# DeepRank/Deeprank-GNN

Measured on AMD Instinct MI355X. Metric: interface-graphs/sec (fwd+bwd) GINet batch=64 per GPU, higher is better.
Workload: dtype f32; 1 GPU; GINet train step (topology + body fwd + FC head/MSE + bwd + grad all-reduce + Adam) on SYN graphs: 200 nodes, ~1000 directed edges, 32 node feats, 50->16 clusters (BASELINE.json configs[1]); graphs_per_gpu=64, global_batch=64, parallelism=dp1, mode=native, step_layout=auto

## Files before the change

### deeprank-gnn_amd/_lib.py

```python
import ctypes
import os

import torch

_HERE = os.path.dirname(os.path.abspath(__file__))
LIB_PATH = os.environ.get("DRGNN_LIB") or os.path.join(_HERE, "csrc", "libdrgnn.so")

GINET, SGAT, FOUT = 0, 1, 2
MAX_BRANCH = 2
LDS_LIMIT = 160 * 1024
HEAD_MAX_HIDDEN = 512

TI = {name: i for i, name in enumerate([
    "NPTR", "EPTR", "ROWPTR0", "COL0", "EID0", "COLPTR0", "ROWIDX0", "TSLOT0", "CL0", "NC0",
    "MPTR0", "MEM0", "ROWPTR1", "COL1", "NE1", "COLPTR1", "ROWIDX1", "TSLOT1", "CL1", "NC1",
    "MPTR1", "MEM1", "CPTR0", "E1PTR", "CPTR1", "ERR", "GSTAT", "HORD", "HMP0", "HSPLIT", "IHORD"])}
TI_COUNT = len(TI)
TF = {"W0": 0, "W1": 1}
TF_COUNT = 2

FAULT_EXCHANGE = 1
STATUS_BITS = {1: "edge endpoint outside its graph's node range",
               2: "batch vector / edge list not grouped by graph",
               4: "cluster ids of one graph span too large a range",
               8: "len(cluster1) != number of depth-0 clusters"}

_c_i64 = ctypes.c_int64
_c_i32 = ctypes.c_int32
_vp = ctypes.c_void_p


class ConvParams(ctypes.Structure):
    _fields_ = [("w_nbr", _vp), ("nbr_sk", _c_i64), ("nbr_sh", _c_i64),
                ("w_self", _vp), ("self_sk", _c_i64), ("self_sh", _c_i64),
                ("bias", _vp)]


class ConvGrads(ctypes.Structure):
    _fields_ = [("w_nbr", _vp), ("w_self", _vp), ("bias", _vp)]


class NetDesc(ctypes.Structure):
    _fields_ = [("kind", _c_i32), ("n_branch", _c_i32), ("n_feat", _c_i32), ("reserved", _c_i32),
                ("conv1", ConvParams * MAX_BRANCH), ("conv2", ConvParams * MAX_BRANCH)]


class EnsMember(ctypes.Structure):
    _fields_ = [("net", NetDesc), ("w1", _vp), ("b1", _vp), ("w2", _vp), ("b2", _vp)]


class CohortMember(ctypes.Structure):
    _fields_ = EnsMember._fields_ + [
                ("flat_param", _vp), ("flat_grad", _vp), ("exp_avg", _vp), ("exp_avg_sq", _vp),
                ("step2", _vp), ("pred", _vp), ("readout", _vp), ("head_partials", _vp), ("partials", _vp), ("loss", _vp),
                ("lr", ctypes.c_double), ("beta1", ctypes.c_double), ("beta2", ctypes.c_double), ("eps", ctypes.c_double),
                ("seed", ctypes.c_uint32), ("reserved", _c_i32)]


class TopologyRequest(ctypes.Structure):
    _fields_ = [("edge_index", _vp), ("edge_attr", _vp), ("batch", _vp), ("cluster0", _vp), ("cluster1", _vp),
                ("node_ptr", _vp), ("edge_ptr", _vp), ("c1_ptr", _vp),
                ("n_nodes", _c_i64), ("n_edges", _c_i64), ("len_cluster1", _c_i64), ("n_graphs", _c_i64),
                ("max_nodes", _c_i32), ("max_edges", _c_i32),
                ("ws_i32", _vp), ("ws_f32", _vp), ("scratch_i32", _vp),
                ("set", _vp), ("ids", _vp), ("x_out", _vp), ("y_out", _vp),
                ("flags", _c_i32), ("reserved", _c_i32),
                ("x", _vp), ("tiles", _vp), ("n_feat", _c_i32), ("reserved2", _c_i32)]


TOPO_HIER = 1
TOPO_LEAN = 2
TOPO_TILES = 4
METRICS_COUNTS, METRICS_REGRESSION, METRICS_RANKING = 1, 2, 4


class GraphSet(ctypes.Structure):
    _fields_ = [("n_graphs", _c_i64), ("n_nodes", _c_i64), ("n_edges", _c_i64), ("len_cluster1", _c_i64),
                ("n_feat", _c_i32), ("y_bytes", _c_i32),
                ("node_ptr", _vp), ("edge_ptr", _vp), ("c1_ptr", _vp),
                ("x", _vp), ("edge_index", _vp), ("edge_attr", _vp),
                ("cluster0", _vp), ("cluster1", _vp), ("y", _vp)]


class EpochPlan(ctypes.Structure):
    _fields_ = [("set", _vp), ("host_node_ptr", _vp), ("host_edge_ptr", _vp), ("host_c1_ptr", _vp),
                ("ids", _vp), ("host_ids", _vp), ("n_ids", _c_i64),
                ("batch_size", _c_i32), ("need_weights", _c_i32), ("inference", _c_i32), ("reserved", _c_i32),
                ("net", _vp), ("head", _vp), ("g_conv1", _vp), ("g_conv2", _vp),
                ("head_offset", _c_i64),
                ("flat_param", _vp), ("flat_grad", _vp), ("exp_avg", _vp), ("exp_avg_sq", _vp), ("n_param", _c_i64),
                ("step2", _vp),
                ("lr", ctypes.c_double), ("beta1", ctypes.c_double), ("beta2", ctypes.c_double), ("eps", ctypes.c_double),
                ("cache", _vp), ("exchange", _vp), ("exchange_user", _vp), ("step_overrides", _vp), ("last_loss", _vp)]


class Optim(ctypes.Structure):
    _fields_ = [("lr", ctypes.c_double), ("beta1", ctypes.c_double), ("beta2", ctypes.c_double), ("eps", ctypes.c_double),
                ("weight_decay", ctypes.c_double), ("max_grad_norm", ctypes.c_double),
                ("lr_table", _vp), ("norm_words", _vp), ("norm_out", _vp),
                ("lr_n", _c_i32), ("decoupled", _c_i32), ("clip", _c_i32), ("norm_cap", _c_i32),
                ("n_dead", _c_i32), ("reserved", _c_i32),
                ("dead_off", _c_i64 * 8), ("dead_len", _c_i64 * 8)]


class IfaceRequest(ctypes.Structure):
    _fields_ = [("xyz", _vp), ("atom_ptr", _vp), ("res_ptr", _vp), ("res_split", _vp), ("res_type", _vp),
                ("host_atom_ptr", _vp), ("host_res_ptr", _vp), ("host_res_split", _vp),
                ("n_atoms", _c_i64), ("n_residues", _c_i64), ("n_complexes", _c_i64),
                ("contact_distance", ctypes.c_double), ("internal_contact_distance", ctypes.c_double),
                ("tile_atoms", _c_i32), ("reserved", _c_i32),
                ("workspace", _vp), ("workspace_bytes", _c_i64),
                ("node_ptr", _vp), ("edge_ptr", _vp), ("iedge_ptr", _vp)]


class ScoreRequest(ctypes.Structure):
    _fields_ = [("xyz", _vp), ("zone_atom", _vp), ("zone_ref", _vp), ("pair_res", _vp), ("atom_ptr", _vp),
                ("host_zone_atom", _vp), ("host_zone_ptr", _vp), ("host_pair_res", _vp), ("host_atom_ptr", _vp),
                ("n_poses", _c_i64), ("n_atoms", _c_i64), ("n_residues", _c_i64), ("n_pairs", _c_i64),
                ("n_ref_pairs", _c_i64), ("fnat_cutoff", ctypes.c_double),
                ("scores", _vp), ("classes", _vp), ("n_preserved", _vp)]


class BsaRequest(ctypes.Structure):
    _fields_ = [("xyz", _vp), ("atom_ptr", _vp), ("res_ptr", _vp), ("res_split", _vp), ("rad_complex", _vp),
                ("rad_unbound", _vp), ("target_res", _vp), ("target_complex", _vp),
                ("host_atom_ptr", _vp), ("host_res_ptr", _vp), ("host_res_split", _vp), ("host_target_res", _vp),
                ("host_target_complex", _vp),
                ("n_atoms", _c_i64), ("n_residues", _c_i64), ("n_complexes", _c_i64), ("n_targets", _c_i64),
                ("n_radii", _c_i64), ("probe", ctypes.c_double), ("n_slices", _c_i32), ("reserved", _c_i32),
                ("out", _vp), ("status", _vp)]


class HseRequest(ctypes.Structure):
    _fields_ = [("xyz", _vp), ("atom_ptr", _vp), ("res_ptr", _vp), ("bb", _vp), ("target_res", _vp), ("target_complex", _vp),
                ("tile_ptr", _vp),
                ("host_atom_ptr", _vp), ("host_res_ptr", _vp), ("host_bb", _vp), ("host_target_res", _vp),
                ("host_target_complex", _vp), ("host_tile_ptr", _vp),
                ("n_atoms", _c_i64), ("n_residues", _c_i64), ("n_complexes", _c_i64), ("n_targets", _c_i64),
                ("n_tiles", _c_i64), ("n_rows", _c_i64), ("radius", ctypes.c_double), ("connect_cutoff", ctypes.c_double),
                ("offset", _c_i32), ("connect_a", _c_i32), ("connect_b", _c_i32), ("direction", _c_i32),
                ("out", _vp), ("status", _vp)]


class PackRequest(ctypes.Structure):
    _fields_ = [("node_ptr", _vp), ("edge_ptr", _vp), ("iedge_ptr", _vp), ("node_residue", _vp), ("chain", _vp), ("type", _vp),
                ("pos", _vp), ("edge_index", _vp), ("dist", _vp), ("internal_edge_index", _vp), ("bsa", _vp), ("hse", _vp),
                ("res_feat", _vp), ("type_table", _vp), ("cols", _vp), ("host_cols", _vp),
                ("n_complexes", _c_i64), ("n_nodes", _c_i64), ("n_edges", _c_i64), ("n_iedges", _c_i64),
                ("n_residues", _c_i64), ("n_rows", _c_i64),
                ("res_width", _c_i32), ("type_width", _c_i32), ("n_cols", _c_i32), ("edge_mode", _c_i32),
                ("x", _vp), ("edge_index_out", _vp), ("edge_attr", _vp), ("internal_edge_index_out", _vp), ("batch", _vp)]


PACK_TYPE, PACK_POS, PACK_CHAIN, PACK_BSA, PACK_HSE, PACK_RES = range(6)


EXCHANGE_FN = ctypes.CFUNCTYPE(ctypes.c_int, ctypes.c_void_p, ctypes.c_int64, ctypes.c_int64, ctypes.c_void_p)


class StepPlan(ctypes.Structure):
    _fields_ = [("kind", _c_i32), ("n_feat", _c_i32), ("max_nodes", _c_i32), ("max_edges", _c_i32), ("max_c0", _c_i32),
                ("R", _c_i32), ("H", _c_i32), ("O", _c_i32),
                ("n_graphs", _c_i64), ("co_built_graphs", _c_i64),
                ("train", _c_i32), ("topo_flags", _c_i32),
                ("force_wgs", _c_i32), ("no_class", _c_i32), ("no_aggregate", _c_i32), ("no_split", _c_i32),
                ("no_paired", _c_i32),
                ("family", _c_i32), ("wgs_per_graph", _c_i32), ("slabs_per_graph", _c_i32), ("width", _c_i32),
                ("cls", _c_i32), ("lean_ok", _c_i32), ("builder_wgs_per_graph", _c_i32),
                ("lds_bytes", _c_i64), ("xchg_words", _c_i64),
                ("from_memory", _c_i32), ("reserved", _c_i32)]

    OVERRIDES = ("force_wgs", "no_class", "no_aggregate", "no_split", "no_paired")


STEP_FAMILY_NONE, STEP_FAMILY_PRODUCT, STEP_FAMILY_AGGREGATE = 0, 1, 2


def _plan_inputs(kind, n_feat, max_nodes, max_edges, max_c0, R, H, O, n_graphs, topo_flags):
    p = StepPlan()
    p.kind, p.n_feat, p.max_nodes, p.max_edges, p.max_c0 = int(kind), int(n_feat), int(max_nodes), int(max_edges), int(max_c0)
    p.R, p.H, p.O, p.n_graphs, p.topo_flags = int(R), int(H), int(O), int(n_graphs), int(topo_flags)
    return p


class StepHints(ctypes.Structure):
    _fields_ = [("host_node_ptr", _vp), ("host_edge_ptr", _vp), ("set_node_ptr", _vp), ("set_edge_ptr", _vp),
                ("host_ids", _vp), ("topo_flags", _c_i32), ("reserved", _c_i32), ("tiles", _vp), ("plan", _vp),
                ("next_ids", _vp), ("n_next", _c_i64)]


class TopologyCacheDesc(ctypes.Structure):
    _fields_ = [("n_graphs", _c_i64), ("n_nodes", _c_i64), ("n_edges", _c_i64),
                ("ws_i32", _vp), ("ws_f32", _vp), ("x", _vp), ("y", _vp), ("y_bytes", _c_i32), ("flags", _c_i32),
                ("tiles", _vp)]


class HeadDesc(ctypes.Structure):
    _fields_ = [("R", _c_i32), ("H", _c_i32), ("O", _c_i32), ("task", _c_i32), ("train", _c_i32),
                ("p_drop", ctypes.c_float), ("seed", ctypes.c_uint32), ("transform_sigmoid", _c_i32),
                ("w1", _vp), ("b1", _vp), ("w2", _vp), ("b2", _vp), ("class_w", _vp), ("drop_mask", _vp)]


TASK_REG, TASK_CLASS, TASK_GRAD = 0, 1, 2
ZERO_RANGES = 8


def _ptr(t):
    return None if t is None else t.data_ptr()


class DrgnnError(RuntimeError):
    pass


def _check(rc, what):
    if rc != 0:
        kind = {-1: "bad argument", -2: "workspace/capacity", -3: "unsupported width"}.get(
            rc, "hipError_t %d" % rc if rc > 0 else "error %d" % rc)
        raise DrgnnError("%s failed: %s" % (what, kind))


class Api(object):

    def __init__(self, path):
        self.path = path
# ... 576 lines not shown
```

### deeprank-gnn_amd/csrc/drgnn_capi.hip

```cpp
#define DRGNN_KERNELS_MAIN
#include "drgnn_kernels.h"

#include <vector>
#include <algorithm>
#include <memory>
#include <string.h>
#include <stdlib.h>
#ifdef DRGNN_EMU
#define DRGNN_LDS_LIMIT (160 * 1024)
#else
#define DRGNN_LDS_LIMIT (160 * 1024)
#define HIP_TRY(expr)                                   \
    do {                                                \
        hipError_t e_ = (expr);                         \
        if (e_ != hipSuccess) return (int)e_;           \
    } while (0)
#endif



extern "C" {

int drgnn_abi_version(void) { return DRGNN_ABI_VERSION; }

#if defined(DRGNN_PHASE_TIMING) && !defined(DRGNN_EMU)
int drgnn_debug_set_phase_buffer(void* dev_buf) {
    unsigned long long* p = (unsigned long long*)dev_buf;
    return (int)hipMemcpyToSymbol(HIP_SYMBOL(g_phase_buf), &p, sizeof(p));
}
#endif

int drgnn_topology_layout(int64_t n_nodes, int64_t n_edges, int64_t n_graphs, int64_t* off_i32,
                          int64_t* off_f32) {
    if (n_nodes < 0 || n_edges < 0 || n_graphs < 0 || !off_i32 || !off_f32) return DRGNN_E_ARG;
    TopoLayout L;
    topo_layout(n_nodes, n_edges, n_graphs, &L);
    for (int k = 0; k <= DRGNN_TI_COUNT; ++k) off_i32[k] = L.i32[k];
    for (int k = 0; k <= DRGNN_TF_COUNT; ++k) off_f32[k] = L.f32[k];
    return 0;
}

int64_t drgnn_topology_scratch_elems(int64_t n_nodes, int64_t n_edges, int64_t n_graphs) {
    return topo_gscratch_base(n_nodes, n_edges, n_graphs) + TOPO_GSCRATCH_CONST;
}

static int64_t topo_lds_bytes(int capN, int capE, int tile_f = 0) {
    const int64_t capT = (capN > capE ? capN : capE) + 1;
    return 4 * (topo_scratch_ints(capN, capE, capT, (int64_t)capN + capE + 2) + (tile_f > 0 ? (int64_t)capN * (((tile_f + 3) & ~3) + 4) : 0));
}
static bool topo_tiles_shape_ok(int capN, int capE, int F) {
    const int TF = (F + 3) & ~3;
    if (capN <= 0 || F <= 0 || F > 256 || (int64_t)capN * TF > 16 * DRGNN_BCAP) return false;
    return topo_lds_bytes(capN, capE > 0 ? capE : 1, F) <= DRGNN_LDS_LIMIT;
}

int64_t drgnn_topology_lds_bytes(int32_t max_nodes, int32_t max_edges) {
    if (max_nodes <= 0) return 0;
    return topo_lds_bytes(max_nodes, max_edges > 0 ? max_edges : 1);
}

int64_t drgnn_topology_tiles_elems(int64_t n_nodes, int32_t n_feat) {
    if (n_nodes < 0 || n_feat <= 0) return 0;
    const int64_t TF = ((int64_t)n_feat + 3) & ~(int64_t)3;
    return (n_feat & 3) ? drgnn_tiles_x_off(n_nodes, TF) + n_nodes * TF : n_nodes * (TF + 2);
}
int32_t drgnn_topology_tiles_ok(int32_t max_nodes, int32_t max_edges, int32_t n_feat) {
    return topo_tiles_shape_ok(max_nodes, max_edges, n_feat) ? 1 : 0;
}

}

#ifndef DRGNN_TOPO_SPLIT_MAX_GRAPHS
#define DRGNN_TOPO_SPLIT_MAX_GRAPHS 160
#endif
static int topo_prepare(TopoLaunch& L, int64_t* lds_out, const int64_t* edge_index, const float* edge_attr,
                        const int64_t* batch, const int64_t* cluster0, const int64_t* cluster1,
                        const int32_t* node_ptr, const int32_t* edge_ptr, const int32_t* c1_ptr,
                        int64_t n_nodes, int64_t n_edges, int64_t len_cluster1, int64_t n_graphs,
                        int32_t max_nodes, int32_t max_edges, int32_t* ws_i32, float* ws_f32,
                        int32_t* scratch_i32, int32_t flags = DRGNN_TOPO_HIER, const float* x_in = nullptr,
                        float* tiles = nullptr, int32_t tile_f = 0) {
    if (n_nodes < 0 || n_edges < 0 || n_graphs < 0 || !ws_i32) return DRGNN_E_ARG;
    if (!batch && !(node_ptr && edge_ptr)) return DRGNN_E_ARG;
    if (!cluster0 && cluster1) return DRGNN_E_ARG;
    if (n_edges > 0 && !edge_index) return DRGNN_E_ARG;
    if (edge_attr && !ws_f32) return DRGNN_E_ARG;
    if (n_nodes + n_graphs >= INT32_MAX || n_edges >= INT32_MAX) return DRGNN_E_CAPACITY;
    TopoLayout lay;
    topo_layout(n_nodes, n_edges, n_graphs, &lay);
    L.tv = topo_view(ws_i32, ws_f32, lay);
    L.args.edge_index = edge_index;
    L.args.edge_attr = edge_attr;
    L.args.cluster0 = cluster0;
    L.args.cluster1 = cluster1;
    L.args.c1_ptr = c1_ptr;
    L.args.n_edges = n_edges;
    L.args.len_cluster1 = len_cluster1;
    L.args.n_graphs = (int)n_graphs;
    L.args.set_ids = nullptr; L.args.set_node_ptr = L.args.set_edge_ptr = L.args.set_c1_ptr = nullptr;
    L.args.set_x = nullptr; L.args.set_y = nullptr; L.args.x_out = nullptr; L.args.y_out = nullptr;
    L.args.n_set = 0; L.args.n_feat = 0; L.args.y_bytes = 0;
    L.args.flags = flags;
    L.args.x_in = nullptr; L.args.tiles = nullptr; L.args.tile_nodes = n_nodes; L.args.tile_f = 0;
    if (flags & DRGNN_TOPO_TILES) {
        if (!(flags & DRGNN_TOPO_HIER) || !tiles || (x_in && !(tile_f & 3) && (((uintptr_t)x_in) & 15)) || (((uintptr_t)tiles) & 15)) return DRGNN_E_ARG;
        if (!topo_tiles_shape_ok(max_nodes, max_edges, tile_f)) return DRGNN_E_CAPACITY;
        L.args.x_in = x_in; L.args.tiles = tiles; L.args.tile_f = tile_f;
    }
    L.gscratch = scratch_i32;
    L.level1_only = 0;
    L.roles = 1;
    L.pf_ids = nullptr; L.pf_n = 0; L.pf_graphs = 0;
    L.user_nptr = (node_ptr && edge_ptr) ? node_ptr : nullptr;
    L.user_eptr = (node_ptr && edge_ptr) ? edge_ptr : nullptr;
    int64_t lds = 0;
    L.capN = 0; L.capE = 0;
    if (max_nodes > 0) {
        lds = topo_lds_bytes(max_nodes, max_edges > 0 ? max_edges : 1, L.args.tile_f);
        if (lds <= DRGNN_LDS_LIMIT) { L.capN = max_nodes; L.capE = max_edges > 0 ? max_edges : 1; }
        else lds = 0;
    }
    if (L.args.tile_f > 0 && L.capN == 0) return DRGNN_E_CAPACITY;
    if (L.capN > 0 && cluster0 != nullptr && L.user_nptr != nullptr && !(cluster1 != nullptr && c1_ptr == nullptr) &&
        n_graphs <= DRGNN_TOPO_SPLIT_MAX_GRAPHS)
        L.roles = 2;
    *lds_out = lds;
    return 0;
}

static int topo_prepare_req(TopoLaunch& T, int64_t* tlds, const drgnn_topology_request* r) {
    const drgnn_graph_set* gs = r->set;
    if (!gs)
        return topo_prepare(T, tlds, r->edge_index, r->edge_attr, r->batch, r->cluster0, r->cluster1, r->node_ptr,
                            r->edge_ptr, r->c1_ptr, r->n_nodes, r->n_edges, r->len_cluster1, r->n_graphs, r->max_nodes,
                            r->max_edges, r->ws_i32, r->ws_f32, r->scratch_i32, r->flags, r->x, r->tiles, r->n_feat);
    if (!r->ids || !r->node_ptr || !r->edge_ptr || !gs->node_ptr || !gs->edge_ptr || !gs->cluster0) return DRGNN_E_ARG;
    if (gs->cluster1 && (!gs->c1_ptr || !r->c1_ptr)) return DRGNN_E_ARG;
    if (r->x_out && (!gs->x || gs->n_feat <= 0)) return DRGNN_E_ARG;
    if (r->y_out && (!gs->y || (gs->y_bytes != 4 && gs->y_bytes != 8))) return DRGNN_E_ARG;
    const float* attr = (r->ws_f32 && gs->edge_attr) ? gs->edge_attr : nullptr;
    if ((r->flags & DRGNN_TOPO_TILES) && (!gs->x || gs->n_feat <= 0 || (!(gs->n_feat & 3) && (((uintptr_t)gs->x) & 15)))) return DRGNN_E_ARG;
    const int rc = topo_prepare(T, tlds, gs->edge_index, attr, nullptr, gs->cluster0, gs->cluster1, r->node_ptr,
                                r->edge_ptr, r->c1_ptr, r->n_nodes, r->n_edges, r->len_cluster1, r->n_graphs,
                                r->max_nodes, r->max_edges, r->ws_i32, r->ws_f32, r->scratch_i32, r->flags, nullptr, r->tiles,
                                gs->n_feat);
    if (rc) return rc;
    TopoArgs& a = T.args;
    a.n_edges = gs->n_edges;
    a.set_ids = r->ids; a.set_node_ptr = gs->node_ptr; a.set_edge_ptr = gs->edge_ptr; a.set_c1_ptr = gs->c1_ptr;
    a.set_x = gs->x; a.set_y = gs->y; a.x_out = r->x_out; a.y_out = r->y_out;
    a.n_set = gs->n_graphs; a.n_feat = gs->n_feat; a.y_bytes = gs->y_bytes;
    return 0;
}

static int topology_build_impl(const int64_t* edge_index, const float* edge_attr, const int64_t* batch,
                         const int64_t* cluster0, const int64_t* cluster1, const int32_t* node_ptr,
                         const int32_t* edge_ptr, const int32_t* c1_ptr, int64_t n_nodes,
                         int64_t n_edges, int64_t len_cluster1, int64_t n_graphs, int32_t max_nodes,
                         int32_t max_edges, int32_t* ws_i32, float* ws_f32, int32_t* scratch_i32,
                         int32_t flags, void* stream_, const float* x_in = nullptr, float* tiles = nullptr,
                         int32_t tile_f = 0) {
    drgnn_stream_t stream = (drgnn_stream_t)stream_;
    TopoLaunch L;
    int64_t lds = 0;
    int rc0 = topo_prepare(L, &lds, edge_index, edge_attr, batch, cluster0, cluster1, node_ptr, edge_ptr, c1_ptr,
                           n_nodes, n_edges, len_cluster1, n_graphs, max_nodes, max_edges, ws_i32, ws_f32,
                           scratch_i32, flags, x_in, tiles, tile_f);
    if (rc0) return rc0;
    if (L.capN == 0 && !scratch_i32) return DRGNN_E_CAPACITY;
    if (n_graphs == 0) return 0;
    PtrArgs pa;
    pa.batch = batch; pa.edge_row = edge_index; pa.n_nodes = n_nodes; pa.n_edges = n_edges;
    pa.n_graphs = (int)n_graphs; pa.nptr = L.tv.p[DRGNN_TI_NPTR]; pa.eptr = L.tv.p[DRGNN_TI_EPTR];
    pa.err = L.tv.p[DRGNN_TI_ERR];
    const bool need_ptrs = !(node_ptr && edge_ptr);
    const int64_t span = n_nodes > n_edges ? n_nodes : n_edges;
#ifdef DRGNN_EMU
    if (need_ptrs) {
        for (int k = 0; k < 4; ++k) pa.err[k] = 0;
        for (int64_t i = 0; i < (span > 0 ? span : 1); ++i) ptr_item(pa, i);
    }
    std::vector<int> lds_buf((size_t)(lds / 4) + 16);
    for (int pass = 0; pass < 2; ++pass) {
        if (pass == 1) { if (!(cluster1 && !c1_ptr)) break; L.level1_only = 1; L.roles = 1; }
        for (int gph = 0; gph < n_graphs * (pass == 0 ? L.roles : 1); ++gph) {
            if (L.capN > 0) topo_block<true>(L, gph, lds_buf.data());
            else topo_block<false>(L, gph, lds_buf.data());
        }
    }
    (void)stream;
#else
    if (need_ptrs) {
        const int n = (int)n_graphs + 1;
        hipLaunchKernelGGL(k_topo_begin, dim3((unsigned)((n + 255) / 256)), dim3(256), 0, stream,
                           (const int32_t*)nullptr, (const int32_t*)nullptr, pa.nptr, pa.eptr, pa.err, n);
        const int64_t items = span > 0 ? span : 1;
        hipLaunchKernelGGL(k_ptrs, dim3((unsigned)((items + 255) / 256)), dim3(256), 0, stream, pa);
    }
    if (lds > 64 * 1024)
        HIP_TRY(hipFuncSetAttribute((const void*)k_topo<true>, hipFuncAttributeMaxDynamicSharedMemorySize, (int)lds));
    for (int pass = 0; pass < 2; ++pass) {
        if (pass == 1) { if (!(cluster1 && !c1_ptr)) break; L.level1_only = 1; L.roles = 1; }
        if (L.capN > 0) hipLaunchKernelGGL(k_topo<true>, dim3((unsigned)(n_graphs * L.roles)), dim3(DRGNN_NTHREADS), (size_t)lds, stream, L);
        else hipLaunchKernelGGL(k_topo<false>, dim3((unsigned)n_graphs), dim3(DRGNN_NTHREADS), 0, stream, L);
    }
    HIP_TRY(hipGetLastError());
#endif
    return 0;
}

extern "C" {

int drgnn_topology_build(const int64_t* edge_index, const float* edge_attr, const int64_t* batch,
                         const int64_t* cluster0, const int64_t* cluster1, const int32_t* node_ptr,
                         const int32_t* edge_ptr, const int32_t* c1_ptr, int64_t n_nodes,
                         int64_t n_edges, int64_t len_cluster1, int64_t n_graphs, int32_t max_nodes,
                         int32_t max_edges, int32_t* ws_i32, float* ws_f32, int32_t* scratch_i32,
                         void* stream_) {
    return topology_build_impl(edge_index, edge_attr, batch, cluster0, cluster1, node_ptr, edge_ptr, c1_ptr, n_nodes, n_edges,
                               len_cluster1, n_graphs, max_nodes, max_edges, ws_i32, ws_f32, scratch_i32, DRGNN_TOPO_HIER,
                               stream_);
}

int drgnn_topology_build_request(const drgnn_topology_request* r, void* stream_) {
    if (!r) return DRGNN_E_ARG;
    if (!r->set)
        return topology_build_impl(r->edge_index, r->edge_attr, r->batch, r->cluster0, r->cluster1, r->node_ptr,
                                   r->edge_ptr, r->c1_ptr, r->n_nodes, r->n_edges, r->len_cluster1, r->n_graphs,
                                   r->max_nodes, r->max_edges, r->ws_i32, r->ws_f32, r->scratch_i32, r->flags, stream_,
                                   r->x, r->tiles, r->n_feat);
    TopoLaunch L;
    int64_t lds = 0;
    const int rc = topo_prepare_req(L, &lds, r);
    if (rc) return rc;
    if (L.capN == 0 && !r->scratch_i32) return DRGNN_E_CAPACITY;
    if (r->n_graphs == 0) return 0;
#ifdef DRGNN_EMU
    std::vector<int> lds_buf((size_t)(lds / 4) + 16);
    for (int gph = 0; gph < r->n_graphs * L.roles; ++gph) {
        if (L.capN > 0) topo_block<true>(L, gph, lds_buf.data());
        else topo_block<false>(L, gph, lds_buf.data());
    }
    (void)stream_;
#else
    hipStream_t stream = (hipStream_t)stream_;
    if (lds > 64 * 1024)
        HIP_TRY(hipFuncSetAttribute((const void*)k_topo<true>, hipFuncAttributeMaxDynamicSharedMemorySize, (int)lds));
    if (L.capN > 0) hipLaunchKernelGGL(k_topo<true>, dim3((unsigned)(r->n_graphs * L.roles)), dim3(DRGNN_NTHREADS), (size_t)lds, stream, L);
    else hipLaunchKernelGGL(k_topo<false>, dim3((unsigned)r->n_graphs), dim3(DRGNN_NTHREADS), 0, stream, L);
    HIP_TRY(hipGetLastError());
#endif
    return 0;
}

int drgnn_topology_tiles(const int32_t* ws_i32, const float* ws_f32, int64_t n_nodes, int64_t n_edges, int64_t n_graphs,
                         const float* x, int32_t n_feat, int32_t use_weights, float* tiles, void* stream_) {
    if (!ws_i32 || !x || !tiles || n_nodes < 0 || n_edges < 0 || n_graphs < 0 || n_feat <= 0) return DRGNN_E_ARG;
    if (use_weights && !ws_f32) return DRGNN_E_ARG;
    if (n_graphs == 0) return 0;
    TopoLayout lay;
    topo_layout(n_nodes, n_edges, n_graphs, &lay);
    TilesArgs a;
    a.tv = topo_view(const_cast<int32_t*>(ws_i32), const_cast<float*>(ws_f32), lay);
    a.x = x; a.tiles = tiles; a.n_nodes = n_nodes; a.n_feat = n_feat; a.use_weights = use_weights ? 1 : 0;
#ifdef DRGNN_EMU
    for (int64_t g = 0; g < n_graphs; ++g) tiles_block(a, (int)g);
    (void)stream_;
#else
    hipLaunchKernelGGL(k_tiles, dim3((unsigned)n_graphs), dim3(DRGNN_NTHREADS), 0, (hipStream_t)stream_, a);
    HIP_TRY(hipGetLastError());
#endif
    return 0;
}

int drgnn_batch_offsets(const drgnn_graph_set* set, const int32_t* ids, int64_t n_ids, int32_t batch_size,
                        int32_t* ptrs, void* stream_) {
    if (!set || !ids || !ptrs || n_ids < 0 || batch_size < 1 || !set->node_ptr || !set->edge_ptr) return DRGNN_E_ARG;
    if (batch_size > 4096) return DRGNN_E_CAPACITY;
    if (n_ids == 0) return 0;
    OffsetsArgs a;
    a.set = *set; a.ids = ids; a.n_ids = n_ids; a.batch_size = batch_size; a.ptrs = ptrs;
    const int64_t nb = (n_ids + batch_size - 1) / batch_size;
    const size_t words = (size_t)DRGNN_NTHREADS + 4 + 3 * ((size_t)batch_size + 1);
#ifdef DRGNN_EMU
    std::vector<int> buf(words);
    for (int64_t k = 0; k < nb; ++k) batch_offsets_block(a, (int)k, buf.data() + DRGNN_NTHREADS + 4, buf.data());
    (void)stream_;
#else
    hipLaunchKernelGGL(k_batch_offsets, dim3((unsigned)nb), dim3(DRGNN_NTHREADS), words * 4, (hipStream_t)stream_, a);
    HIP_TRY(hipGetLastError());
#endif
    return 0;
}

int drgnn_topology_finalize(int32_t* ws_i32, int64_t n_nodes, int64_t n_edges, int64_t n_graphs,
                            void* stream_) {
    if (!ws_i32 || n_graphs < 0) return DRGNN_E_ARG;
    TopoLayout lay;
    topo_layout(n_nodes, n_edges, n_graphs, &lay);
    ScanArgs a;
    a.tv = topo_view(ws_i32, nullptr, lay);
    a.n_graphs = (int)n_graphs;
#ifdef DRGNN_EMU
    int part[DRGNN_NTHREADS + 4];
    finalize_block(a, part);
    (void)stream_;
#else
    hipLaunchKernelGGL(k_finalize, dim3(1), dim3(DRGNN_NTHREADS), 0, (hipStream_t)stream_, a);
    HIP_TRY(hipGetLastError());
#endif
    return 0;
}

int drgnn_topology_status(const int32_t* ws_i32, int64_t n_nodes, int64_t n_edges, int64_t n_graphs,
                          int32_t* status4, void* stream_) {
    if (!ws_i32 || !status4) return DRGNN_E_ARG;
    TopoLayout lay;
    topo_layout(n_nodes, n_edges, n_graphs, &lay);
    const int32_t* err = ws_i32 + lay.i32[DRGNN_TI_ERR];
    const int32_t* gst = ws_i32 + lay.i32[DRGNN_TI_GSTAT];
    std::vector<int32_t> host((size_t)(2 * n_graphs) + 4);
#ifdef DRGNN_EMU
    for (int k = 0; k < 4; ++k) host[k] = err[k];
    for (int64_t g = 0; g < 2 * n_graphs; ++g) host[4 + g] = gst[g];
    (void)stream_;
#else
    HIP_TRY(hipMemcpyAsync(host.data(), err, 4 * sizeof(int32_t), hipMemcpyDeviceToHost, (hipStream_t)stream_));
    if (n_graphs > 0)
        HIP_TRY(hipMemcpyAsync(host.data() + 4, gst, 2 * n_graphs * sizeof(int32_t), hipMemcpyDeviceToHost, (hipStream_t)stream_));
    HIP_TRY(hipStreamSynchronize((hipStream_t)stream_));
#endif
    status4[0] = host[0]; status4[1] = -1; status4[2] = 0; status4[3] = 0;
    for (int64_t g = 0; g < n_graphs; ++g) {
        host[4 + g] |= host[4 + n_graphs + g];
        if (host[4 + g]) {
            status4[0] |= host[4 + g];
            if (status4[1] < 0) status4[1] = (int32_t)g;
            status4[2] += 1;
        }
    }
    return 0;
}

struct StepCaps { int N, E, C; };
static StepCaps step_caps(int32_t max_nodes, int32_t max_edges, int32_t max_c0) {
    return StepCaps{max_nodes, max_edges > 0 ? max_edges : 1, (max_c0 > 0 && max_c0 < max_nodes) ? max_c0 : max_nodes};
}

int64_t drgnn_net_lds_bytes(int32_t kind, int32_t n_feat, int32_t max_nodes, int32_t max_edges,
                            int32_t max_c0, int32_t backward) {
    if (max_nodes <= 0) return 0;
    const StepCaps c = step_caps(max_nodes, max_edges, max_c0);
    return 4 * net_scratch_words(kind, n_feat, c.N, c.E, c.C, backward);
}

int64_t drgnn_net_partial_elems(int32_t kind, int32_t n_feat) { (void)kind; return net_partial_floats(n_feat); }

int64_t drgnn_net_scratch_elems(int32_t kind, int32_t n_feat, int64_t n_nodes, int64_t n_edges,
                                int64_t n_graphs) {
    const int nb = (kind == DRGNN_GINET) ? 2 : 1;
    const int64_t f = net_gscratch_base(kind, n_feat, n_nodes, n_edges, n_graphs, 0);
    const int64_t b = net_gscratch_base(kind, n_feat, n_nodes, n_edges, n_graphs, 1);
    return nb * (f > b ? f : b) + 64;
}

}

static int net_check(const drgnn_net_desc* net) {
    if (!net) return DRGNN_E_ARG;
    if (net->kind < DRGNN_GINET || net->kind > DRGNN_FOUT) return DRGNN_E_ARG;
    if (net->n_branch < 1 || net->n_branch > DRGNN_MAX_BRANCH) return DRGNN_E_ARG;
    if (net->n_feat < 1) return DRGNN_E_WIDTH;
    for (int b = 0; b < net->n_branch; ++b) {
        if (!net->conv1[b].w_nbr || !net->conv2[b].w_nbr) return DRGNN_E_ARG;
        if (net->kind != DRGNN_GINET &&
            (!net->conv1[b].w_self || !net->conv2[b].w_self || !net->conv1[b].bias || !net->conv2[b].bias))
            return DRGNN_E_ARG;
    }
    return 0;
}

template <bool BWD>
static int net_launch(NetLaunch& L, int32_t max_nodes, int32_t max_edges, int32_t max_c0, float* scratch,
// ... 2302 lines not shown
```

### deeprank-gnn_amd/csrc/drgnn_kernels.h

```cpp
#pragma once
#include "drgnn_head.h"
#include "drgnn_step.h"
#include "drgnn_step2.h"
#include "drgnn_step3.h"
#include "drgnn_layers.h"
#include "drgnn_mcl.h"
#include "drgnn_louvain.h"
#include "drgnn_iface.h"
#include "drgnn_score.h"
#include "drgnn_bsa.h"
#include "drgnn_hse.h"
#include "drgnn_pack.h"
#include "drgnn_metrics.h"
#include "drgnn_collate.h"
#include "drgnn_p2p.h"

struct PtrArgs {
    const int64_t* batch;
    const int64_t* edge_row;
    int64_t n_nodes, n_edges;
    int n_graphs;
    int32_t* nptr;
    int32_t* eptr;
    int32_t* err;
};

DEV void ptr_item(const PtrArgs& a, int64_t i) {
    const int B = a.n_graphs;
    if (i < a.n_nodes) {
        long long b = a.batch[i];
        long long prev = (i > 0) ? (long long)a.batch[i - 1] : -1;
        if (b < prev || b < 0 || b >= B) { ATOMIC_OR(&a.err[0], DRGNN_S_UNSORTED); a.err[1] = 0; b = prev < 0 ? 0 : prev; }
        for (long long gph = prev + 1; gph <= b && gph <= B; ++gph) a.nptr[gph] = (int32_t)i;
        if (i == a.n_nodes - 1)
            for (long long gph = b + 1; gph <= B; ++gph) a.nptr[gph] = (int32_t)a.n_nodes;
    }
    if (i < a.n_edges) {
        auto graph_of = [&](int64_t e) -> long long {
            const long long r = a.edge_row[e];
            if (r < 0 || r >= a.n_nodes) return -2;
            return (long long)a.batch[r];
        };
        long long b = graph_of(i);
        long long prev = (i > 0) ? graph_of(i - 1) : -1;
        if (b == -2 || prev == -2) { ATOMIC_OR(&a.err[0], DRGNN_S_EDGE_RANGE); a.err[1] = 0; if (b == -2) b = prev < 0 ? 0 : prev; if (prev == -2) prev = b; }
        if (b < prev || b >= B) { ATOMIC_OR(&a.err[0], DRGNN_S_UNSORTED); a.err[1] = 0; b = prev; }
        for (long long gph = prev + 1; gph <= b && gph <= B; ++gph) a.eptr[gph] = (int32_t)i;
        if (i == a.n_edges - 1)
            for (long long gph = b + 1; gph <= B; ++gph) a.eptr[gph] = (int32_t)a.n_edges;
    }
    if (i == 0) {
        if (a.n_nodes == 0) for (int gph = 0; gph <= B; ++gph) a.nptr[gph] = 0;
        if (a.n_edges == 0) for (int gph = 0; gph <= B; ++gph) a.eptr[gph] = 0;
    }
}

struct TopoLaunch {
    TopoView tv;
    TopoArgs args;
    const int32_t* user_nptr;
    const int32_t* user_eptr;
    int32_t* gscratch;
    int capN, capE;
    int level1_only;
    int roles;
    const int32_t* pf_ids; int pf_n; int pf_graphs;
    const float* pf_tiles; const float* pf_x; int pf_f; int pf_coef;
    long long pf_tile_nodes;
    const void* pf_y; int pf_y_bytes;
};

#ifdef DRGNN_EMU
DEV void prefetch_block(const TopoLaunch&, int) {}
#else
DEV void prefetch_block(const TopoLaunch& L, int g) {
    if (g >= L.pf_n) return;
    const int32_t* const* P = L.tv.p;
    const int id = __builtin_amdgcn_readfirstlane(L.pf_ids[g]);
    if (id < 0 || id >= L.pf_graphs) return;
    const int n0 = P[DRGNN_TI_NPTR][id], n1 = P[DRGNN_TI_NPTR][id + 1];
    const int e0 = P[DRGNN_TI_EPTR][id], e1 = P[DRGNN_TI_EPTR][id + 1];
    const int N = n1 - n0, E = e1 - e0, rowbase = n0 + id, t = threadIdx.x;
    int acc = P[DRGNN_TI_NC0][id] ^ P[DRGNN_TI_NE1][id] ^ P[DRGNN_TI_NC1][id] ^ P[DRGNN_TI_GSTAT][id] ^ P[DRGNN_TI_HSPLIT][4 * id];
    if (L.pf_y) acc ^= (L.pf_y_bytes == 8) ? (int)((const long long*)L.pf_y)[id] : ((const int*)L.pf_y)[id];
    drgnn_f4 f = {0.f, 0.f, 0.f, 0.f};
    const int n4 = (N * L.pf_f) >> 2;
    const drgnn_f4* s4 = (const drgnn_f4*)(L.pf_tiles + (long long)n0 * L.pf_f);
    const drgnn_f4* x4 = L.pf_x ? (const drgnn_f4*)(L.pf_x + (long long)n0 * L.pf_f) : nullptr;
    for (int q = t; q < n4; q += DRGNN_NTHREADS) {
        const drgnn_f4 v = s4[q];
        f[0] += v[0]; f[1] += v[1]; f[2] += v[2]; f[3] += v[3];
        if (x4) { const drgnn_f4 u = x4[q]; f[0] += u[0]; f[1] += u[1]; f[2] += u[2]; f[3] += u[3]; }
    }
    for (int i = t; i <= N; i += DRGNN_NTHREADS) {
        acc ^= P[DRGNN_TI_HMP0][rowbase + i] ^ P[DRGNN_TI_MPTR1][rowbase + i] ^ P[DRGNN_TI_ROWPTR1][rowbase + i] ^
               P[DRGNN_TI_COLPTR1][rowbase + i];
        if (i < N) {
            acc ^= P[DRGNN_TI_IHORD][n0 + i] ^ P[DRGNN_TI_MEM1][n0 + i];
            if (L.pf_coef) {
                const float* td = L.pf_tiles + L.pf_tile_nodes * L.pf_f + n0;
                f[0] += td[i] + td[L.pf_tile_nodes + i];
            }
        }
    }
    for (int e = t; e < E; e += DRGNN_NTHREADS) {
        acc ^= P[DRGNN_TI_COL1][e0 + e] ^ P[DRGNN_TI_ROWIDX1][e0 + e];
        if (L.pf_coef && L.tv.w1) { acc ^= P[DRGNN_TI_TSLOT1][e0 + e]; f[1] += L.tv.w1[e0 + e]; }
    }
    if (acc == 0x7fc12345 && f[0] + f[1] + f[2] + f[3] == 12345.678f) { const_cast<int32_t*>(P[DRGNN_TI_ERR])[1] = acc; }
}
#endif

template <bool LDS, int WEIGHTS = -1>
DEV void topo_block(const TopoLaunch& L, int blk, int* lds) {
    TopoScratch s;
    if (L.pf_ids != nullptr) { prefetch_block(L, blk); return; }
#ifdef DRGNN_TOPO_EXIT0
    return;
#endif
    int g = blk, role = TOPO_ROLE_ALL;
    if (L.roles == 2) {
        const int full = (L.args.n_graphs >> 3) << 4;
        if (blk < full) { g = ((blk >> 4) << 3) + (blk & 7); role = ((blk >> 3) & 1) ? TOPO_ROLE_MEMBERS : TOPO_ROLE_EDGES; }
        else { const int t = blk - full; g = (full >> 1) + (t >> 1); role = (t & 1) ? TOPO_ROLE_MEMBERS : TOPO_ROLE_EDGES; }
    }
    const int sidx = (role == TOPO_ROLE_MEMBERS) ? L.args.n_graphs + g : g;
    const int32_t* NP = L.user_nptr ? L.user_nptr : L.tv.p[DRGNN_TI_NPTR];
    const int32_t* EP = L.user_eptr ? L.user_eptr : L.tv.p[DRGNN_TI_EPTR];
    const int n0 = NP[g], n1 = NP[g + 1], N = n1 - n0;
    const int e0 = EP[g], e1 = EP[g + 1], E = e1 - e0;
    if (LDS) {
        const int capT = imax(L.capN, L.capE) + 1;
        s = topo_carve(lds, L.capN, L.capE, capT, L.capN + L.capE + 2);
        if (L.args.tile_f > 0 && L.args.tiles != nullptr)
            s.xs = (float*)(lds + topo_scratch_ints(L.capN, L.capE, capT, (int64_t)L.capN + L.capE + 2));
    } else {
        s = topo_carve(L.gscratch + topo_gscratch_base(n0, e0, g), N, E, N + E + 1, N + E + 2);
    }
    const bool fits = !LDS || (N <= L.capN && E <= L.capE);
    if (!L.level1_only) {
        FOR_TID(i, 1) {
            L.tv.p[DRGNN_TI_GSTAT][sidx] = 0;
            if (role == TOPO_ROLE_ALL) L.tv.p[DRGNN_TI_GSTAT][L.args.n_graphs + g] = 0;
            if (L.user_nptr && role != TOPO_ROLE_MEMBERS) {
                L.tv.p[DRGNN_TI_NPTR][g] = n0; L.tv.p[DRGNN_TI_NPTR][g + 1] = n1;
                L.tv.p[DRGNN_TI_EPTR][g] = e0; L.tv.p[DRGNN_TI_EPTR][g + 1] = e1;
                if (g == 0) L.tv.p[DRGNN_TI_ERR][0] = 0;
            }
        }
        if (fits && (L.args.flags & DRGNN_TOPO_LEAN)) topo_lean_preclear(N, s, role != TOPO_ROLE_EDGES, role != TOPO_ROLE_MEMBERS);
        BARRIER();
    }
    if (!fits) {
        FOR_TID(i, 1) { topo_flag(L.tv, DRGNN_S_EDGE_RANGE, sidx); }
        return;
    }
    if (!L.level1_only) {
        topo_graph<WEIGHTS>(L.tv, L.args, g, n0, n1, e0, e1, s, role);
    } else {
        FOR_TID(i, 1) { s.part[0] = 0; }
        BARRIER();
        FOR_TID(t, DRGNN_NTHREADS) {
            int acc = 0;
            for (int q = t; q < g; q += DRGNN_NTHREADS) acc += L.tv.p[DRGNN_TI_NC0][q];
            if (acc) ATOMIC_ADD(&s.part[0], acc);
        }
        BARRIER();
        const int begin = s.part[0];
        const int C0 = L.tv.p[DRGNN_TI_NC0][g];
        BARRIER();
        int len = C0;
        if (g == L.args.n_graphs - 1 && (int64_t)begin + C0 != L.args.len_cluster1) len = -1;
        if ((int64_t)begin + C0 > L.args.len_cluster1) len = -1;
        topo_graph_level1(L.tv, L.args, g, n0, C0, L.args.cluster1 + begin, len, s, g, false,
                          (L.args.flags & DRGNN_TOPO_HIER) ? L.tv.p[DRGNN_TI_CL0] + n0 : nullptr, N);
    }
}

struct TilesArgs { TopoView tv; const float* x; float* tiles; int64_t n_nodes; int n_feat, use_weights; };
DEV void tiles_block(const TilesArgs& a, int g) {
    const int n0 = a.tv.p[DRGNN_TI_NPTR][g], N = a.tv.p[DRGNN_TI_NPTR][g + 1] - n0;
    const int e0 = a.tv.p[DRGNN_TI_EPTR][g];
    const int32_t* rp = a.tv.p[DRGNN_TI_ROWPTR0] + n0 + g;
    const int32_t* col = a.tv.p[DRGNN_TI_COL0] + e0;
    const float* w = (a.use_weights && a.tv.w0) ? a.tv.w0 + e0 : nullptr;
    const int F = a.n_feat, TF = (F + 3) & ~3;
    const float* x = a.x + (long long)n0 * F;
    float* ts = a.tiles + (long long)n0 * TF;
    float* td = a.tiles + a.n_nodes * TF + n0;
    float* tc = td + a.n_nodes;
    float* tx = (F & 3) ? a.tiles + drgnn_tiles_x_off(a.n_nodes, TF) + (long long)n0 * TF : nullptr;
    FOR_TID(pad, N * (TF - F)) {
        const int i = pad / (TF - F), f = F + pad % (TF - F);
        ts[(long long)i * TF + f] = 0.0f;
        tx[(long long)i * TF + f] = 0.0f;
    }
    FOR_TID(item, N * F) {
        const int i = item / F, f = item - i * F;
        if (tx) tx[(long long)i * TF + f] = x[(long long)i * F + f];
        const int lo = rp[i], hi = rp[i + 1], deg = hi - lo;
        float acc = 0.0f, asum = 0.0f;
        if (w != nullptr) {
            for (int k = lo; k < hi; k += 4)
                for (int j = 0; j < 4; ++j) {
                    const int kk = (k + j < hi) ? k + j : hi - 1;
                    const float cf = ((k + j < hi) ? 1.0f : 0.0f) * w[kk];
                    asum += cf;
                    acc = fmaf(cf, x[(long long)col[kk] * F + f], acc);
                }
        } else {
            for (int k = lo; k < hi; ++k) acc += x[(long long)col[k] * F + f];
        }
        ts[(long long)i * TF + f] = acc;
        if (f == 0) {
            float d, sc;
            if (w != nullptr) { d = 1.0f / (float)(deg > 0 ? deg : 1); sc = asum * d; }
            else { d = deg > 0 ? 1.0f / (float)deg : 0.0f; sc = 1.0f; }
            td[i] = d; tc[i] = sc;
        }
    }
}

struct ScanArgs { TopoView tv; int n_graphs; };
DEV void finalize_block(const ScanArgs& a, int* part) {
    const int B = a.n_graphs;
    const int src[3] = {DRGNN_TI_NC0, DRGNN_TI_NE1, DRGNN_TI_NC1};
    const int dst[3] = {DRGNN_TI_CPTR0, DRGNN_TI_E1PTR, DRGNN_TI_CPTR1};
    for (int w = 0; w < 3; ++w) {
        int32_t* out = a.tv.p[dst[w]];
        const int32_t* in = a.tv.p[src[w]];
        FOR_TID(i, B + 1) { out[i] = (i < B) ? in[i] : 0; }
        BARRIER();
        wg_exscan(out, B + 1, part);
    }
}

struct ReduceArgs {
    const float* partials;
    int n_graphs, n_branch, n_feat, n_partial;
    int kind;
    drgnn_conv_params lay1[DRGNN_MAX_BRANCH], lay2[DRGNN_MAX_BRANCH];
    drgnn_conv_grads g1[DRGNN_MAX_BRANCH], g2[DRGNN_MAX_BRANCH];
    float* grad_x; int64_t n_nodes;
};

DEV float* reduce_dst(const ReduceArgs& a, int br, int p) {
    const int F = a.n_feat;
    const int o_w1s = F * DRGNN_H1, o_b1 = 2 * F * DRGNN_H1, o_w2n = o_b1 + DRGNN_H1;
    const int o_w2s = o_w2n + DRGNN_H1 * DRGNN_H2, o_b2 = o_w2s + DRGNN_H1 * DRGNN_H2;
    if (p < o_w1s)
        return a.g1[br].w_nbr ? a.g1[br].w_nbr + (int64_t)(p / DRGNN_H1) * a.lay1[br].nbr_sk + (int64_t)(p % DRGNN_H1) * a.lay1[br].nbr_sh : nullptr;
    if (p < o_b1) {
        const int q = p - o_w1s;
        return a.g1[br].w_self ? a.g1[br].w_self + (int64_t)(q / DRGNN_H1) * a.lay1[br].self_sk + (int64_t)(q % DRGNN_H1) * a.lay1[br].self_sh : nullptr;
    }
    if (p < o_w2n) return a.g1[br].bias ? a.g1[br].bias + (p - o_b1) : nullptr;
    if (p < o_w2s) {
        const int q = p - o_w2n;
        return a.g2[br].w_nbr ? a.g2[br].w_nbr + (int64_t)(q / DRGNN_H2) * a.lay2[br].nbr_sk + (int64_t)(q % DRGNN_H2) * a.lay2[br].nbr_sh : nullptr;
    }
    if (p < o_b2) {
        const int q = p - o_w2s;
        return a.g2[br].w_self ? a.g2[br].w_self + (int64_t)(q / DRGNN_H2) * a.lay2[br].self_sk + (int64_t)(q % DRGNN_H2) * a.lay2[br].self_sh : nullptr;
    }
    return a.g2[br].bias ? a.g2[br].bias + (p - o_b2) : nullptr;
}
DEV void reduce_write(const ReduceArgs& a, int br, int p, float acc) {
    float* d = reduce_dst(a, br, p);
    if (d) *d = acc;
}

DEV bool reduce_live(const ReduceArgs& a, int p) {
    if (a.kind != DRGNN_GINET) return true;
    const int F = a.n_feat;
    const int o_w1s = F * DRGNN_H1, o_w2n = 2 * F * DRGNN_H1 + DRGNN_H1, o_w2s = o_w2n + DRGNN_H1 * DRGNN_H2;
    return p < o_w1s || (p >= o_w2n && p < o_w2s);
}

DEV float reduce_sum(const ReduceArgs& a, int br, int p, int first, int stride) {
    const float* src = a.partials + (int64_t)br * a.n_partial + p;
    const int64_t step = (int64_t)a.n_branch * a.n_partial;
    float acc = 0.0f;
    float v[16];
    int g = first;
    for (; g + 15 * stride < a.n_graphs; g += 16 * stride) {
#pragma unroll
        for (int k = 0; k < 16; ++k) v[k] = src[(int64_t)(g + k * stride) * step];
#pragma unroll
        for (int k = 0; k < 16; ++k) acc += v[k];
    }
    for (; g < a.n_graphs; g += stride) acc += src[(int64_t)g * step];
    return acc;
}

DEV float reduce_sum_w(const ReduceArgs& a, int br, int p, int first, int stride, const float* w, int wshift) {
    const float* src = a.partials + (int64_t)br * a.n_partial + p;
    const int64_t step = (int64_t)a.n_branch * a.n_partial;
    float acc = 0.0f;
    float v[16], c[16];
    int g = first;
    for (; g + 15 * stride < a.n_graphs; g += 16 * stride) {
#pragma unroll
        for (int k = 0; k < 16; ++k) { v[k] = src[(int64_t)(g + k * stride) * step]; c[k] = w[(g + k * stride) >> wshift]; }
#pragma unroll
        for (int k = 0; k < 16; ++k) acc = fmaf(c[k], v[k], acc);
    }
    for (; g < a.n_graphs; g += stride) acc = fmaf(w[g >> wshift], src[(int64_t)g * step], acc);
    return acc;
}

DEV void reduce_grad_x(const ReduceArgs& a, int64_t item) {
    if (a.grad_x != nullptr && a.n_branch > 1 && item < a.n_nodes * a.n_feat) {
        float acc = a.grad_x[item];
        for (int br = 1; br < a.n_branch; ++br) acc += a.grad_x[(int64_t)br * a.n_nodes * a.n_feat + item];
        a.grad_x[item] = acc;
    }
}

struct NetLaunch {
    NetArgs a;
    float* gscratch;
    int capN, capE, capC;
    int64_t n_edges;
};

struct CoLaunch {
    NetLaunch net;
    TopoLaunch topo;
    int n_net;
};

HD int64_t net_gscratch_base(int kind, int F, int64_t n0, int64_t e0, int64_t g, int bwd) {
    const int64_t c0 = net_scratch_words(kind, F, 0, 0, 0, bwd);
    return net_scratch_words(kind, F, n0, e0, n0, bwd) - c0 + c0 * g;
}

template <int KIND, bool BWD, bool LDS>
DEV void net_block(const NetLaunch& L, int blk, float* lds) {
    const int nb = L.a.net.n_branch;
    const int g = blk / nb, br = blk % nb;
    float* scratch;
    int capN, capE, capC;
    if (LDS) {
        scratch = lds; capN = L.capN; capE = L.capE; capC = L.capC;
        const int n0 = L.a.tv.p[DRGNN_TI_NPTR][g], e0 = L.a.tv.p[DRGNN_TI_EPTR][g];
        if (L.a.tv.p[DRGNN_TI_NPTR][g + 1] - n0 > capN || L.a.tv.p[DRGNN_TI_EPTR][g + 1] - e0 > capE ||
            L.a.tv.p[DRGNN_TI_NC0][g] > capC) {
            if (!BWD) {
                FOR_TID(c, DRGNN_H2) { L.a.readout[(long)g * DRGNN_H2 * nb + br * DRGNN_H2 + c] = DRGNN_NAN; }
            }
            return;
        }
    } else {
        const int n0 = L.a.tv.p[DRGNN_TI_NPTR][g], e0 = L.a.tv.p[DRGNN_TI_EPTR][g];
        capN = L.a.tv.p[DRGNN_TI_NPTR][g + 1] - n0;
        capE = L.a.tv.p[DRGNN_TI_EPTR][g + 1] - e0;
        capC = capN;
        const int F = L.a.net.n_feat;
        const int64_t per_branch = net_gscratch_base(KIND, F, L.a.n_nodes, L.n_edges, L.a.n_graphs, BWD);
        scratch = L.gscratch + (int64_t)br * per_branch + net_gscratch_base(KIND, F, n0, e0, g, BWD);
    }
    if (BWD) net_backward_graph<KIND>(L.a, g, g, br, scratch, capN, capE, capC);
    else net_forward_graph<KIND>(L.a, g, g, br, scratch, capN, capE, capC);
}

#define DRGNN_STEP_DIMS_MAX 64
struct StepDims {
    int count;
    int32_t n0[DRGNN_STEP_DIMS_MAX], n[DRGNN_STEP_DIMS_MAX], e0[DRGNN_STEP_DIMS_MAX], e[DRGNN_STEP_DIMS_MAX];
    int32_t gi[DRGNN_STEP_DIMS_MAX];
};
struct StepLaunch {
    StepArgs a;
    int capN, capE, capC;
    int64_t words;
    StepDims dims;
};
struct StepCoLaunch {
    StepLaunch step;
    TopoLaunch topo;
    int n_net;
};

#ifndef DRGNN_EMU
template <int KIND, int XF, bool GATHER, int CLS, int SPLIT, bool TRAIN, int XG = 0>
DEV void step2_block(const StepLaunch& L, const StepArgs& A, int blk, float* lds) {
    int g, half;
    if (SPLIT == 2) { g = ((blk >> 4) << 3) + (blk & 7); half = (blk >> 3) & 1; }
    else { g = blk; half = 0; }
    if (g >= A.n_graphs) return;
    if (L.dims.count > 0) {
        const int gi = GATHER ? L.dims.gi[g] : g;
        GraphDims d;
        d.n0 = L.dims.n0[g]; d.N = L.dims.n[g]; d.e0 = L.dims.e0[g]; d.E = L.dims.e[g];
        d.rowbase = d.n0 + gi;
        d.C = 0; d.E1 = 0; d.C1 = 0;
        const int cnt_c = A.tv.p[DRGNN_TI_NC0][gi], cnt_e1 = A.tv.p[DRGNN_TI_NE1][gi], cnt_c1 = A.tv.p[DRGNN_TI_NC1][gi];
        const int32_t* hs = A.tv.p[DRGNN_TI_HSPLIT] + 4 * gi;
        const int hk = (SPLIT == 2) ? hs[0] : 0, hq = (SPLIT == 2) ? hs[1] : 0, hn = (SPLIT == 2) ? hs[2] : 0;
        net_step2_graph<KIND, XF, GATHER, CLS, SPLIT, TRAIN, XG>(A, d, g, gi, half, lds, L.capN, L.capE, L.capC, true, cnt_c, cnt_e1,
                                                             cnt_c1, hk, hq, hn);
        return;
    }
    const int gi = GATHER ? WG_UNIFORM(A.gather_ids[g]) : g;
    const GraphDims d = net_dims(A.tv, gi);
    const int32_t* hs = A.tv.p[DRGNN_TI_HSPLIT] + 4 * gi;
    const int hk = (SPLIT == 2) ? WG_UNIFORM(hs[0]) : 0, hq = (SPLIT == 2) ? WG_UNIFORM(hs[1]) : 0, hn = (SPLIT == 2) ? WG_UNIFORM(hs[2]) : 0;
    if (d.N > L.capN || d.E > L.capE || d.C > L.capC) {
        if (half == 0) {
            FOR_TID(c, A.hf.R) { const_cast<float*>(A.hf.readout)[(long)g * A.hf.R + c] = DRGNN_NAN; }
            if (TRAIN) {
                float* hp = A.hf.partials + (long)g * head_compact_floats(A.hf.R, A.hf.H, A.hf.O);
                FOR_TID(i, (int)head_compact_floats(A.hf.R, A.hf.H, A.hf.O)) { hp[i] = DRGNN_NAN; }
            }
            FOR_TID(o, A.hf.O) { A.hf.pred[(long)g * A.hf.O + o] = DRGNN_NAN; }
        }
        return;
    }
    net_step2_graph<KIND, XF, GATHER, CLS, SPLIT, TRAIN, XG>(A, d, g, gi, half, lds, L.capN, L.capE, L.capC, false, 0, 0, 0, hk, hq, hn);
}
#endif

#ifndef DRGNN_EMU
template <int XF, bool GATHER, int CLS, bool TRAIN>
DEV void step3_block(const StepLaunch& L, int blk, float* lds) {
    const int g = ((blk >> 4) << 3) + (blk & 7), br = (blk >> 3) & 1;
    if (g >= L.a.n_graphs) return;
    if (L.dims.count > 0) {
        const int gi = GATHER ? L.dims.gi[g] : g;
        GraphDims d;
        d.n0 = L.dims.n0[g]; d.N = L.dims.n[g]; d.e0 = L.dims.e0[g]; d.E = L.dims.e[g];
        d.rowbase = d.n0 + gi;
        d.C = 0; d.E1 = 0; d.C1 = 0;
        const int cnt_c = L.a.tv.p[DRGNN_TI_NC0][gi], cnt_e1 = L.a.tv.p[DRGNN_TI_NE1][gi], cnt_c1 = L.a.tv.p[DRGNN_TI_NC1][gi];
        net_step3_graph<XF, GATHER, CLS, TRAIN>(L.a, d, g, gi, br, lds, L.capN, L.capE, L.capC, true, cnt_c, cnt_e1, cnt_c1);
        return;
    }
    const int gi = GATHER ? WG_UNIFORM(L.a.gather_ids[g]) : g;
    const GraphDims d = net_dims(L.a.tv, gi);
    if (d.N > L.capN || d.E > L.capE || d.C > L.capC) {
        const uint32_t tag = (uint32_t)L.a.step2[0] + 1u;
        FOR_TID(c, DRGNN_H2) { const_cast<float*>(L.a.hf.readout)[(long)g * L.a.hf.R + br * DRGNN_H2 + c] = DRGNN_NAN; }
        FOR_TID(h, L.a.hf.H) { xchg_publish(L.a.xchg + ((long)g * 2 + br) * L.a.hf.H + h, tag, DRGNN_NAN); }
        if (br == 0) {
            if (TRAIN) {
                float* hp = L.a.hf.partials + (long)g * head_compact_floats(L.a.hf.R, L.a.hf.H, L.a.hf.O);
                FOR_TID(i, (int)head_compact_floats(L.a.hf.R, L.a.hf.H, L.a.hf.O)) { hp[i] = DRGNN_NAN; }
            }
            FOR_TID(o, L.a.hf.O) { L.a.hf.pred[(long)g * L.a.hf.O + o] = DRGNN_NAN; }
        }
        return;
    }
    net_step3_graph<XF, GATHER, CLS, TRAIN>(L.a, d, g, gi, br, lds, L.capN, L.capE, L.capC, false, 0, 0, 0);
}
#endif

#ifndef DRGNN_EMU
template <int XF, bool GATHER, int CLS, bool TRAIN, bool SG = false>
DEV void step3b_block(const StepLaunch& L, const StepArgs& A, int g, float* lds) {
    constexpr bool DUAL = !SG && STEP3B_DUAL(XF, CLS, TRAIN);
    if (g >= A.n_graphs) return;
    if (L.dims.count > 0) {
        const int gi = GATHER ? L.dims.gi[g] : g;
        GraphDims d;
        d.n0 = L.dims.n0[g]; d.N = L.dims.n[g]; d.e0 = L.dims.e0[g]; d.E = L.dims.e[g];
        d.rowbase = d.n0 + gi;
        d.C = 0; d.E1 = 0; d.C1 = 0;
        const int cnt_c = A.tv.p[DRGNN_TI_NC0][gi], cnt_e1 = A.tv.p[DRGNN_TI_NE1][gi], cnt_c1 = A.tv.p[DRGNN_TI_NC1][gi];
        net_step3_graph_both<XF, GATHER, CLS, TRAIN, DUAL, SG>(A, d, g, gi, lds, L.capN, L.capE, L.capC, true, cnt_c, cnt_e1, cnt_c1);
        return;
    }
    const int gi = GATHER ? WG_UNIFORM(A.gather_ids[g]) : g;
    const GraphDims d = net_dims(A.tv, gi);
    if (d.N > L.capN || d.E > L.capE || d.C > L.capC) {
        FOR_TID(c, A.hf.R) { const_cast<float*>(A.hf.readout)[(long)g * A.hf.R + c] = DRGNN_NAN; }
        if (TRAIN) {
            float* hp = A.hf.partials + (long)g * head_compact_floats(A.hf.R, A.hf.H, A.hf.O);
            FOR_TID(i, (int)head_compact_floats(A.hf.R, A.hf.H, A.hf.O)) { hp[i] = DRGNN_NAN; }
        }
        FOR_TID(o, A.hf.O) { A.hf.pred[(long)g * A.hf.O + o] = DRGNN_NAN; }
        return;
    }
    net_step3_graph_both<XF, GATHER, CLS, TRAIN, DUAL, SG>(A, d, g, gi, lds, L.capN, L.capE, L.capC, false, 0, 0, 0);
}
#endif

struct UpdateArgs {
    ReduceArgs r;
    HeadReduceArgs h;
    AdamArgs ad;
    int conv_blocks;
    int blocks_per_branch;
    int apply_adam;
    const float* readout;
    int hR, hH;
    int32_t* step2;
    float* loss2;
};

DEV void update_store(const UpdateArgs& u, float* dst, float g) {
    *dst = g;
    if (u.apply_adam) adam_item(u.ad, (int64_t)(dst - u.ad.grad));
}

DEV int update_head_items(const UpdateArgs& u) { return (u.readout ? u.hH * u.hR : 0) + u.h.P - 1; }
DEV float update_head_sum(const UpdateArgs& u, int item, int first, int stride) {
    float acc = 0.0f;
    if (u.readout) {
        const int HR = u.hH * u.hR;
        if (item < HR) {
            const int h = item / u.hR, r = item - h * u.hR;
            const float* dh = u.h.partials + h;
            const float* xr = u.readout + r;
            float va[16], vb[16];
            int w = first;
            for (; w + 15 * stride < u.h.n_wg; w += 16 * stride) {
#pragma unroll
                for (int k = 0; k < 16; ++k) { va[k] = dh[(long)(w + k * stride) * u.h.P]; vb[k] = xr[(long)(w + k * stride) * u.hR]; }
#pragma unroll
                for (int k = 0; k < 16; ++k) acc = fmaf(va[k], vb[k], acc);
            }
            for (; w < u.h.n_wg; w += stride) acc = fmaf(dh[(long)w * u.h.P], xr[(long)w * u.hR], acc);
            return acc;
        }
        item -= HR;
    }
    const float* src = u.h.partials + item;
    float v[16];
    int w = first;
    for (; w + 15 * stride < u.h.n_wg; w += 16 * stride) {
#pragma unroll
        for (int k = 0; k < 16; ++k) v[k] = src[(long)(w + k * stride) * u.h.P];
#pragma unroll
        for (int k = 0; k < 16; ++k) acc += v[k];
    }
    for (; w < u.h.n_wg; w += stride) acc += src[(long)w * u.h.P];
    return acc;
}
DEV float update_head_sum_w(const UpdateArgs& u, int item, int first, int stride, const float* gw) {
    float acc = 0.0f;
    if (u.readout) {
        const int HR = u.hH * u.hR;
        if (item < HR) {
            const int h = item / u.hR, r = item - h * u.hR;
            const float* dh = u.h.partials + h;
            const float* xr = u.readout + r;
            float va[16], vb[16], vc[16];
            int w = first;
            for (; w + 15 * stride < u.h.n_wg; w += 16 * stride) {
#pragma unroll
                for (int k = 0; k < 16; ++k) {
                    va[k] = dh[(long)(w + k * stride) * u.h.P]; vb[k] = xr[(long)(w + k * stride) * u.hR]; vc[k] = gw[w + k * stride];
                }
#pragma unroll
                for (int k = 0; k < 16; ++k) acc = fmaf(vc[k] * va[k], vb[k], acc);
            }
            for (; w < u.h.n_wg; w += stride) acc = fmaf(gw[w] * dh[(long)w * u.h.P], xr[(long)w * u.hR], acc);
            return acc;
        }
        item -= HR;
    }
    const float* src = u.h.partials + item;
    float v[16], c[16];
    int w = first;
    for (; w + 15 * stride < u.h.n_wg; w += 16 * stride) {
#pragma unroll
        for (int k = 0; k < 16; ++k) { v[k] = src[(long)(w + k * stride) * u.h.P]; c[k] = gw[w + k * stride]; }
#pragma unroll
        for (int k = 0; k < 16; ++k) acc = fmaf(c[k], v[k], acc);
    }
    for (; w < u.h.n_wg; w += stride) acc = fmaf(gw[w], src[(long)w * u.h.P], acc);
    return acc;
}
struct GradArgs {
    UpdateArgs u;
    const float* graph_weight;
    int wshift;
    int n_zero;
    float* zero_ptr[DRGNN_ZERO_RANGES];
    int64_t zero_len[DRGNN_ZERO_RANGES];
};
DEV void update_head_store(const UpdateArgs& u, int item, float acc) {
    const int n_grad = update_head_items(u) - 1;
    if (item < n_grad) update_store(u, u.h.grad + item, acc);
    else if (item == n_grad && u.h.loss) { u.h.loss[0] = acc; if (u.loss2) u.loss2[0] = acc; }
}

struct CohortStep {
    const drgnn_cohort_member* members;
    const int32_t* ids;
    const int32_t* counts;
    int K;
    int64_t stride;
};
#ifndef DRGNN_EMU
#ifdef DRGNN_KERNELS_MAIN
__global__ void __launch_bounds__(256) k_ptrs(PtrArgs a) {
    const int64_t i = (int64_t)blockIdx.x * blockDim.x + threadIdx.x;
    ptr_item(a, i);
}
#endif
template <int N>
DEV void kernarg_touch_lines(int off0) {
    static_assert(N >= 1 && N <= 12, "lines per call");
    const char* base = (const char*)__builtin_amdgcn_kernarg_segment_ptr() + (off0 & ~63);
    int t;
#define DRGNN_KA_OFF(k) "i"(64 * ((k) < N ? (k) : N - 1))
    asm volatile("s_load_dword %0, %1, %2\n s_load_dword %0, %1, %3\n s_load_dword %0, %1, %4\n s_load_dword %0, %1, %5\n"
                 "s_load_dword %0, %1, %6\n s_load_dword %0, %1, %7\n s_load_dword %0, %1, %8\n s_load_dword %0, %1, %9\n"
                 "s_load_dword %0, %1, %10\n s_load_dword %0, %1, %11\n s_load_dword %0, %1, %12\n s_load_dword %0, %1, %13\n"
                 "s_waitcnt lgkmcnt(0)"
                 : "=&s"(t)
                 : "s"(base), DRGNN_KA_OFF(0), DRGNN_KA_OFF(1), DRGNN_KA_OFF(2), DRGNN_KA_OFF(3), DRGNN_KA_OFF(4), DRGNN_KA_OFF(5),
                   DRGNN_KA_OFF(6), DRGNN_KA_OFF(7), DRGNN_KA_OFF(8), DRGNN_KA_OFF(9), DRGNN_KA_OFF(10), DRGNN_KA_OFF(11)
                 : "memory");
#undef DRGNN_KA_OFF
}
#define DRGNN_KA_LINES(first_byte, end_byte) ((((end_byte) - 1) >> 6) - ((first_byte) >> 6) + 1)
template <bool LDS>
__global__ void __launch_bounds__(DRGNN_NTHREADS) k_topo(TopoLaunch L) {
    extern __shared__ __attribute__((aligned(16))) int smem_i[];
    PHASE_BEGIN();
    kernarg_touch_lines<DRGNN_KA_LINES(0, (int)sizeof(TopoLaunch))>(0);
    topo_block<LDS>(L, blockIdx.x, smem_i);
}
#ifdef DRGNN_KERNELS_MAIN
__global__ void __launch_bounds__(DRGNN_NTHREADS) k_tiles(TilesArgs a) { tiles_block(a, blockIdx.x); }
__global__ void __launch_bounds__(DRGNN_NTHREADS) k_finalize(ScanArgs a) {
    __shared__ int part[DRGNN_NTHREADS + 4];
    finalize_block(a, part);
}
__global__ void __launch_bounds__(256) k_reduce(ReduceArgs a, int64_t n_items) {
    __shared__ float quarter[4][64];
    const int lane = threadIdx.x & 63, q = threadIdx.x >> 6;
    const int bpb = (a.n_partial + 63) / 64;
    int br = 0, blk = (int)blockIdx.x;
    while (blk >= bpb && br + 1 < a.n_branch) { blk -= bpb; ++br; }
    const int p_raw = blk * 64 + lane;
    const bool live = p_raw < a.n_partial && reduce_live(a, p_raw);
    const int p = live ? p_raw : 0;
    quarter[q][lane] = live ? reduce_sum(a, br, p, q, 4) : 0.0f;
    __syncthreads();
    if (q == 0) {
        if (live) reduce_write(a, br, p, (quarter[0][lane] + quarter[1][lane]) + (quarter[2][lane] + quarter[3][lane]));
    } else {
        for (int64_t e = (int64_t)blockIdx.x * 192 + (threadIdx.x - 64); e < a.n_nodes * a.n_feat && a.grad_x; e += (int64_t)gridDim.x * 192)
            reduce_grad_x(a, e);
    }
}
#endif
template <int KIND, bool BWD, bool LDS>
__global__ void __launch_bounds__(DRGNN_NTHREADS) k_net(NetLaunch L) {
    extern __shared__ __attribute__((aligned(16))) float smem_f[];
    PHASE_BEGIN();
    net_block<KIND, BWD, LDS>(L, blockIdx.x, smem_f);
}
template <int KIND, bool BWD>
__global__ void __launch_bounds__(DRGNN_NTHREADS) k_net_co_topo(CoLaunch C) {
    extern __shared__ __attribute__((aligned(16))) float smem_c[];
    PHASE_BEGIN();
    if ((int)blockIdx.x < C.n_net) net_block<KIND, BWD, true>(C.net, blockIdx.x, smem_c);
    else topo_block<true>(C.topo, (int)blockIdx.x - C.n_net, (int*)smem_c);
}
DEV const StepCoLaunch& step_kernarg() {
    return *reinterpret_cast<const StepCoLaunch*>((const char*)__builtin_amdgcn_kernarg_segment_ptr());
}
DEV void co_kernarg_touch() {
    constexpr int first = (int)offsetof(StepCoLaunch, topo), end = (int)sizeof(StepCoLaunch);
    constexpr int N0 = 13, N1 = DRGNN_KA_LINES(first, end);
    static_assert(offsetof(StepLaunch, dims) + sizeof(int) >= 0x2c0 && sizeof(StepLaunch) >= 0x340, "the touched lines lie inside the step arguments");
    static_assert(N1 >= 1 && N1 <= 13, "one asm statement covers 13 lines per part");
    const char* b0 = (const char*)__builtin_amdgcn_kernarg_segment_ptr();
    const char* b1 = b0 + (first & ~63);
    int t;
#define DRGNN_KA_OFF(k, N) "i"(64 * ((k) < N ? (k) : N - 1))
#define DRGNN_KA_13(b) "s_load_dword %0, " b ", %3\n s_load_dword %0, " b ", %4\n s_load_dword %0, " b ", %5\n s_load_dword %0, " b ", %6\n" \
                       "s_load_dword %0, " b ", %7\n s_load_dword %0, " b ", %8\n s_load_dword %0, " b ", %9\n s_load_dword %0, " b ", %10\n" \
                       "s_load_dword %0, " b ", %11\n s_load_dword %0, " b ", %12\n s_load_dword %0, " b ", %13\n s_load_dword %0, " b ", %14\n" \
                       "s_load_dword %0, " b ", %15\n"
    asm volatile(DRGNN_KA_13("%1")
                 "s_load_dword %0, %2, %16\n s_load_dword %0, %2, %17\n s_load_dword %0, %2, %18\n s_load_dword %0, %2, %19\n"
                 "s_load_dword %0, %2, %20\n s_load_dword %0, %2, %21\n s_load_dword %0, %2, %22\n s_load_dword %0, %2, %23\n"
                 "s_load_dword %0, %2, %24\n s_load_dword %0, %2, %25\n s_load_dword %0, %2, %26\n s_load_dword %0, %2, %27\n"
                 "s_load_dword %0, %2, %28\n s_waitcnt lgkmcnt(0)"
                 : "=&s"(t)
                 : "s"(b0), "s"(b1),
                   DRGNN_KA_OFF(0, N0), DRGNN_KA_OFF(1, N0), DRGNN_KA_OFF(2, N0), DRGNN_KA_OFF(3, N0), DRGNN_KA_OFF(4, N0), DRGNN_KA_OFF(5, N0),
                   DRGNN_KA_OFF(6, N0), DRGNN_KA_OFF(7, N0), DRGNN_KA_OFF(8, N0), DRGNN_KA_OFF(9, N0), DRGNN_KA_OFF(10, N0), DRGNN_KA_OFF(11, N0),
                   DRGNN_KA_OFF(12, N0),
                   DRGNN_KA_OFF(0, N1), DRGNN_KA_OFF(1, N1), DRGNN_KA_OFF(2, N1), DRGNN_KA_OFF(3, N1), DRGNN_KA_OFF(4, N1), DRGNN_KA_OFF(5, N1),
                   DRGNN_KA_OFF(6, N1), DRGNN_KA_OFF(7, N1), DRGNN_KA_OFF(8, N1), DRGNN_KA_OFF(9, N1), DRGNN_KA_OFF(10, N1), DRGNN_KA_OFF(11, N1),
                   DRGNN_KA_OFF(12, N1)
                 : "memory");
#undef DRGNN_KA_13
#undef DRGNN_KA_OFF
}
#ifdef DRGNN_TOPO_FIRST
#define STEP_CO_ROLES(C)                                                       \
    const int co_extra_ = (int)gridDim.x - (C).n_net;                          \
    const bool co_is_step_ = (int)blockIdx.x >= co_extra_;                     \
    const int co_step_blk_ = (int)blockIdx.x - co_extra_, co_topo_blk_ = (int)blockIdx.x
#else
#define STEP_CO_ROLES(C)                                                       \
    const bool co_is_step_ = (int)blockIdx.x < (C).n_net;                      \
    const int co_step_blk_ = (int)blockIdx.x, co_topo_blk_ = (int)blockIdx.x - (C).n_net
#endif
template <int KIND, int XF, bool GATHER, int CLS, int SPLIT, bool TRAIN, int XG = 0>
__global__ void __launch_bounds__(DRGNN_NTHREADS) k_step2_co_topo(StepCoLaunch C_by_value) {
    extern __shared__ __attribute__((aligned(16))) float smem_s2[];
    PHASE_BEGIN();
    const StepCoLaunch& C = step_kernarg();
    co_kernarg_touch();
    STEP_CO_ROLES(C);
    if (co_is_step_) step2_block<KIND, XF, GATHER, CLS, SPLIT, TRAIN, XG>(C.step, C.step.a, co_step_blk_, smem_s2);
    else topo_block<true, (KIND == DRGNN_SGAT) ? -1 : 0>(C.topo, co_topo_blk_, (int*)smem_s2);
}
template <int XF, bool GATHER, int CLS, bool TRAIN>
__global__ void __launch_bounds__(DRGNN_NTHREADS) k_step3_co_topo(StepCoLaunch C_by_value) {
    extern __shared__ __attribute__((aligned(16))) float smem_s3[];
    PHASE_BEGIN();
    const StepCoLaunch& C = step_kernarg();
    co_kernarg_touch();
    STEP_CO_ROLES(C);
    if (co_is_step_) step3_block<XF, GATHER, CLS, TRAIN>(C.step, co_step_blk_, smem_s3);
    else topo_block<true, 0>(C.topo, co_topo_blk_, (int*)smem_s3);
}
template <int XF, bool GATHER, int CLS, bool TRAIN, bool SG = false>
__global__ void __launch_bounds__(DRGNN_NTHREADS) k_step3b_co_topo(StepCoLaunch C_by_value) {
    extern __shared__ __attribute__((aligned(16))) float smem_s3b[];
    PHASE_BEGIN();
    const StepCoLaunch& C = step_kernarg();
    co_kernarg_touch();
    STEP_CO_ROLES(C);
    if (co_is_step_) step3b_block<XF, GATHER, CLS, TRAIN, SG>(C.step, C.step.a, co_step_blk_, smem_s3b);
    else topo_block<true, 0>(C.topo, co_topo_blk_, (int*)smem_s3b);
}
DEV bool ens_slot(int blk, int K, int n_graphs, int& g, int& m) {
    const int q = blk >> 3;
    m = q % K;
    g = (q / K) * 8 + (blk & 7);
    return g < n_graphs;
}
DEV void ens_args(StepArgs& a, const drgnn_ens_member* models, int m) {
    const drgnn_ens_member& mm = models[m];
    a.net = mm.net;
    a.hf.w1 = mm.w1; a.hf.b1 = mm.b1; a.hf.w2 = mm.w2; a.hf.b2 = mm.b2;
    a.hf.pred = a.hf.pred + (long)m * a.hf.B * a.hf.O;
    a.hf.readout = a.hf.readout + (long)m * a.hf.B * a.hf.R;
}
typedef void (*drgnn_ens_kernel_t)(StepCoLaunch, const drgnn_ens_member*, int);
template <int XF, int CLS, bool SG>
__global__ void __launch_bounds__(DRGNN_NTHREADS) k_step3b_ens(StepCoLaunch C_by_value, const drgnn_ens_member* models, int K) {
    extern __shared__ __attribute__((aligned(16))) float smem_e3[];
    PHASE_BEGIN();
    const StepCoLaunch& C = step_kernarg();
    co_kernarg_touch();
    int g, m;
    if (!ens_slot((int)blockIdx.x, K, C.step.a.n_graphs, g, m)) return;
    StepArgs a = C.step.a;
    ens_args(a, models, m);
    step3b_block<XF, true, CLS, false, SG>(C.step, a, g, smem_e3);
}
template <int KIND, int XF, int CLS, int XG>
__global__ void __launch_bounds__(DRGNN_NTHREADS) k_step2_ens(StepCoLaunch C_by_value, const drgnn_ens_member* models, int K) {
    extern __shared__ __attribute__((aligned(16))) float smem_e2[];
    PHASE_BEGIN();
    const StepCoLaunch& C = step_kernarg();
    co_kernarg_touch();
    int g, m;
    if (!ens_slot((int)blockIdx.x, K, C.step.a.n_graphs, g, m)) return;
    StepArgs a = C.step.a;
    ens_args(a, models, m);
    step2_block<KIND, XF, true, CLS, 1, false, XG>(C.step, a, g, smem_e2);
}
template <class T> DEV T wg_uniform_words(const T& v) {
    static_assert(sizeof(T) % 4 == 0, "whole words");
    union { T t; int w[sizeof(T) / 4]; } in, out;
    in.t = v;
#pragma unroll
    for (int i = 0; i < (int)(sizeof(T) / 4); ++i) out.w[i] = __builtin_amdgcn_readfirstlane(in.w[i]);
    return out.t;
}
DEV bool cohort_args(StepArgs& a, const CohortStep& c, int m, int g) {
    const int B = WG_UNIFORM(c.counts[m]);
    if (g >= B) return false;
    const drgnn_cohort_member mm = wg_uniform_words(c.members[m]);
    a.net = mm.net;
    a.n_graphs = B;
    a.gather_ids = c.ids + (int64_t)m * c.stride;
    a.partials = mm.partials;
    a.step2 = mm.step2;
    a.hf.B = B; a.hf.seed = mm.seed; a.hf.step = mm.step2;
    a.hf.w1 = mm.w1; a.hf.b1 = mm.b1; a.hf.w2 = mm.w2; a.hf.b2 = mm.b2;
    a.hf.pred = mm.pred; a.hf.readout = mm.readout; a.hf.partials = mm.head_partials;
    return true;
}
typedef void (*drgnn_cohort_kernel_t)(StepCoLaunch, CohortStep);
template <int XF, int CLS, bool SG>
__global__ void __launch_bounds__(DRGNN_NTHREADS) k_step3b_cohort(StepCoLaunch C_by_value, CohortStep coh) {
    extern __shared__ __attribute__((aligned(16))) float smem_c3[];
    PHASE_BEGIN();
    const StepCoLaunch& C = step_kernarg();
    co_kernarg_touch();
    int g, m;
    if (!ens_slot((int)blockIdx.x, coh.K, C.step.a.n_graphs, g, m)) return;
    StepArgs a = C.step.a;
    if (!cohort_args(a, coh, m, g)) return;
    step3b_block<XF, true, CLS, true, SG>(C.step, a, g, smem_c3);
}
template <int KIND, int XF, int CLS, int XG>
__global__ void __launch_bounds__(DRGNN_NTHREADS) k_step2_cohort(StepCoLaunch C_by_value, CohortStep coh) {
    extern __shared__ __attribute__((aligned(16))) float smem_c2[];
    PHASE_BEGIN();
    const StepCoLaunch& C = step_kernarg();
    co_kernarg_touch();
    int g, m;
    if (!ens_slot((int)blockIdx.x, coh.K, C.step.a.n_graphs, g, m)) return;
    StepArgs a = C.step.a;
    if (!cohort_args(a, coh, m, g)) return;
    step2_block<KIND, XF, true, CLS, 1, true, XG>(C.step, a, g, smem_c2);
}
#ifdef DRGNN_KERNELS_MAIN
__global__ void __launch_bounds__(DRGNN_NTHREADS) k_conv_gemm(ConvLayerArgs a) { conv_gemm_block(a, blockIdx.x); }
__global__ void __launch_bounds__(256) k_conv_aggregate(ConvLayerArgs a) {
    conv_aggregate_item(a, (int64_t)blockIdx.x * blockDim.x + threadIdx.x);
}
__global__ void __launch_bounds__(256) k_conv_bwd_du(ConvLayerArgs a) {
    conv_bwd_du_item(a, (int64_t)blockIdx.x * blockDim.x + threadIdx.x);
}
__global__ void __launch_bounds__(DRGNN_NTHREADS) k_conv_bwd_dw(ConvLayerArgs a) { conv_bwd_dw_block(a, blockIdx.x); }
__global__ void __launch_bounds__(256) k_conv_reduce(ConvReduceArgs a) {
    conv_reduce_item(a, blockIdx.x * blockDim.x + threadIdx.x);
}
__global__ void __launch_bounds__(256) k_conv_bwd_dx(ConvLayerArgs a) {
    conv_bwd_dx_item(a, (int64_t)blockIdx.x * blockDim.x + threadIdx.x);
}
__global__ void __launch_bounds__(DRGNN_NTHREADS) k_segpool_fwd(SegPoolArgs a) { segpool_fwd_block(a, blockIdx.x); }
__global__ void __launch_bounds__(256) k_segmax_bwd(SegPoolArgs a, int64_t n_items, int64_t n_nodes) {
    segmax_bwd_item(a, (int64_t)blockIdx.x * blockDim.x + threadIdx.x, n_items, n_nodes);
}
__global__ void __launch_bounds__(DRGNN_NTHREADS) k_edge_export(EdgeExportArgs a) { edge_export_block(a, blockIdx.x); }
__global__ void __launch_bounds__(DRGNN_NTHREADS) k_cluster_max(ClusterOffsetArgs a) {
    __shared__ long long mm[2];
    cluster_max_block(a, blockIdx.x, mm);
}
__global__ void k_cluster_scan(ClusterOffsetArgs a) { cluster_scan_single(a); }
__global__ void __launch_bounds__(DRGNN_NTHREADS) k_cluster_add(ClusterOffsetArgs a) { cluster_add_block(a, blockIdx.x); }
__global__ void __launch_bounds__(DRGNN_NTHREADS) k_mcl(MclArgs a) {
// ... 331 lines not shown
```

### deeprank-gnn_amd/csrc/drgnn_topology.h

```cpp
#pragma once
#include "drgnn_rt.h"
#include "../../include/drgnn.h"

HD long long drgnn_tiles_x_off(long long n, int TF) { return n * TF + ((2 * n + 3) & ~3LL); }

#ifdef DRGNN_EMU
#define LAMBDA_DEV
#else
#define LAMBDA_DEV __device__
#endif

struct TopoLayout {
    int64_t i32[DRGNN_TI_COUNT + 1];
    int64_t f32[DRGNN_TF_COUNT + 1];
};

static inline void topo_layout(int64_t N, int64_t E, int64_t B, TopoLayout* L) {
    int64_t o = 0;
    auto take = [&](int which, int64_t n) { L->i32[which] = o; o += (n + 3) & ~(int64_t)3; };
    take(DRGNN_TI_NPTR, B + 1);
    take(DRGNN_TI_EPTR, B + 1);
    take(DRGNN_TI_ROWPTR0, N + B);
    take(DRGNN_TI_COL0, E);
    take(DRGNN_TI_EID0, E);
// ... 211 lines not shown
#else
    long long lo = LLONG_MAX, hi = LLONG_MIN;
    for (int i = threadIdx.x; i < n; i += DRGNN_NTHREADS) {
        const long long v = (long long)ids[i];
        lo = v < lo ? v : lo;
        hi = v > hi ? v : hi;
        low[i] = (int)(unsigned int)((unsigned long long)v & 0xffffffffull);
    }
    if ((int)(threadIdx.x & ~(DRGNN_WAVE - 1)) < n) {
        wave_minmax_i64(lo, hi);
        if ((threadIdx.x & (DRGNN_WAVE - 1)) == 0) {
            slots[2 * (threadIdx.x / DRGNN_WAVE)] = lo;
            slots[2 * (threadIdx.x / DRGNN_WAVE) + 1] = hi;
        }
    }
#endif
}
DEV void wg_rank_prepare(const int64_t* ids, int n, TopoScratch& s) { wg_rank_prepare_to(ids, n, s.pp, s.mm + 2); }
#ifndef DRGNN_EMU
DEV void wg_rank_prepare_val(long long v, int n, int* low, long long* slots) {
    long long lo = LLONG_MAX, hi = LLONG_MIN;
    if ((int)threadIdx.x < n) {
        lo = v; hi = v;
        low[threadIdx.x] = (int)(unsigned int)((unsigned long long)v & 0xffffffffull);
    }
    if ((int)(threadIdx.x & ~(DRGNN_WAVE - 1)) < n) {
        wave_minmax_i64(lo, hi);
        if ((threadIdx.x & (DRGNN_WAVE - 1)) == 0) {
            slots[2 * (threadIdx.x / DRGNN_WAVE)] = lo;
            slots[2 * (threadIdx.x / DRGNN_WAVE) + 1] = hi;
        }
    }
}
#endif
DEV void wg_prepared_minmax(const long long* slots, int n, long long& mn, long long& mx) {
    mn = LLONG_MAX; mx = LLONG_MIN;
    const int nw = imin(DRGNN_NTHREADS / DRGNN_WAVE, (n + DRGNN_WAVE - 1) / DRGNN_WAVE);
    if (nw == 1) { mn = slots[0]; mx = slots[1]; return; }
    for (int w = 0; w < nw; ++w) {
        const long long l = slots[2 * w], h = slots[2 * w + 1];
        mn = l < mn ? l : mn;
        mx = h > mx ? h : mx;
    }
}

DEV int wg_cluster_rank(const TopoView& tv, int graph, const int64_t* ids, int n, TopoScratch& s,
                        bool prepared = false, bool with_members = true, int* inv = nullptr) {
    long long mn, mx;
    if (prepared) {
        mn = LLONG_MAX; mx = LLONG_MIN;
        const int nw = imin(DRGNN_NTHREADS / DRGNN_WAVE, (n + DRGNN_WAVE - 1) / DRGNN_WAVE);
        for (int w = 0; w < nw; ++w) {
            const long long l = s.mm[2 + 2 * w], h = s.mm[3 + 2 * w];
            mn = l < mn ? l : mn;
            mx = h > mx ? h : mx;
        }
    } else {
        wg_minmax64(ids, n, s.mm, false);
        mn = s.mm[0]; mx = s.mm[1];
    }
    const long long span = (n > 0) ? (mx - mn + 1) : 0;
    int C;
    if (span >= 0 && span <= (long long)(s.capF - 1)) {
        const int range = (int)span;
        if (!prepared) {
            FOR_TID(v, range + 1) { s.fl[v] = 0; }
            BARRIER();
        }
        const unsigned int mn_lo = (unsigned int)((unsigned long long)mn & 0xffffffffull);
        if (prepared) { FOR_TID(i, n) { s.fl[(int)((unsigned int)s.pp[i] - mn_lo)] = 1; } }
        else { FOR_TID(i, n) { s.fl[(int)((long long)ids[i] - mn)] = 1; } }
        BARRIER();
        C = wg_exscan(s.fl, range + 1, s.part);
        if (prepared) { FOR_TID(i, n) { s.cl[i] = s.fl[(int)((unsigned int)s.pp[i] - mn_lo)]; } }
        else { FOR_TID(i, n) { s.cl[i] = s.fl[(int)((long long)ids[i] - mn)]; } }
        FOR_TID(b, n + 1) { s.mp[b] = 0; s.cur[b] = 0; }
        BARRIER();
    } else {
        FOR_TID(i, n) {
            const long long me = (long long)ids[i];
            int r = 0;
            for (int j = 0; j < n; ++j) {
                const long long o = (long long)ids[j];
                r += (o < me || (o == me && j < i)) ? 1 : 0;
            }
            s.t1[r] = i;
        }
        BARRIER();
        FOR_TID(p, n + 1) {
            int head = 0;
            if (p < n) head = (p == 0 || ids[s.t1[p]] != ids[s.t1[p - 1]]) ? 1 : 0;
            s.t2[p] = head;
        }
        BARRIER();
        C = wg_exscan(s.t2, n + 1, s.part);
        FOR_TID(p, n) {
            const bool head = (p == 0 || ids[s.t1[p]] != ids[s.t1[p - 1]]);
            s.cl[s.t1[p]] = s.t2[p] - (head ? 0 : 1);
        }
        FOR_TID(b, n + 1) { s.mp[b] = 0; s.cur[b] = 0; }
        BARRIER();
    }
    if (with_members) {
        const int* cl = s.cl;
        wg_bucket_sort(n, C, [cl] LAMBDA_DEV(int i) { return cl[i]; }, s.mp, s.cur, s.t1, s.t2, s.mem,
                       s.part, true, inv);
    }
    return C;
}

DEV void wg_csc_build(int n, int m, const int* col, const int* slot_row, TopoScratch& s,
                      int32_t* g_colptr, int32_t* g_rowidx, int32_t* g_tslot, bool prezeroed = false) {
    wg_bucket_sort(m, n, [col] LAMBDA_DEV(int k) { return col[k]; }, s.cp, s.cur, s.t1, s.t2, s.t3,
                   s.part, prezeroed);
    FOR_TID(j, m) {
        const int k = s.t3[j];
        g_tslot[j] = k;
        g_rowidx[j] = slot_row[k];
    }
    FOR_TID(i, n + 1) { g_colptr[i] = s.cp[i]; }
    BARRIER();
}

struct TopoArgs {
    const int64_t* edge_index;
    const float* edge_attr;
    const int64_t* cluster0;
    const int64_t* cluster1;
    const int32_t* c1_ptr;
    int64_t n_edges;
    int64_t len_cluster1;
    int n_graphs;
    const int32_t* set_ids;
    const int64_t* set_node_ptr;
    const int64_t* set_edge_ptr;
    const int64_t* set_c1_ptr;
    const float* set_x;
    const void* set_y;
    float* x_out;
    void* y_out;
    int64_t n_set;
    int n_feat, y_bytes;
    int flags;
    const float* x_in;
    float* tiles;
    int64_t tile_nodes;
    int tile_f;
};

struct TopoSrc {
    const int64_t* row; const int64_t* col; const float* attr; const int64_t* cl0; const int64_t* cl1;
    long long shift; long long x_row;
};
DEV TopoSrc topo_src(const TopoArgs& a, int g, int n0, int e0) {
    TopoSrc t;
    if (a.set_ids == nullptr) {
        t.row = a.edge_index + e0;
        t.col = a.edge_index + a.n_edges + e0;
        t.attr = a.edge_attr ? a.edge_attr + e0 : nullptr;
        t.cl0 = a.cluster0 ? a.cluster0 + n0 : nullptr;
        t.cl1 = (a.cluster1 && a.c1_ptr) ? a.cluster1 + a.c1_ptr[g] : nullptr;
        t.shift = n0;
        t.x_row = n0;
    } else {
        long long id = a.set_ids[g];
        if (id < 0 || id >= a.n_set) id = 0;
        const long long se = a.set_edge_ptr[id], sn = a.set_node_ptr[id];
        t.row = a.edge_index + se;
        t.col = a.edge_index + a.n_edges + se;
        t.attr = a.edge_attr ? a.edge_attr + se : nullptr;
        t.cl0 = a.cluster0 ? a.cluster0 + sn : nullptr;
        t.cl1 = (a.cluster1 && a.set_c1_ptr) ? a.cluster1 + a.set_c1_ptr[id] : nullptr;
        t.shift = 0;
        t.x_row = sn;
    }
    return t;
}
DEV void topo_gather_rows(const TopoArgs& a, const TopoSrc& src, int g, int n0, int N) {
    if (a.set_ids == nullptr || a.x_out == nullptr) return;
    const int F = a.n_feat;
    const float* xs = a.set_x + src.x_row * F;
    float* xd = a.x_out + (long long)n0 * F;
#ifndef DRGNN_EMU
    if ((F & 3) == 0) {
        const drgnn_f4* xs4 = (const drgnn_f4*)xs;
        drgnn_f4* xd4 = (drgnn_f4*)xd;
        FOR_TID(i, N * (F >> 2)) { xd4[i] = xs4[i]; }
    } else
#endif
    {
        FOR_TID(i, N * F) { xd[i] = xs[i]; }
    }
    if (a.y_out && a.set_y) {
        long long id = a.set_ids[g];
        if (id < 0 || id >= a.n_set) id = 0;
        FOR_TID(i, 1) {
            if (a.y_bytes == 8) ((int64_t*)a.y_out)[g] = ((const int64_t*)a.set_y)[id];
            else ((int32_t*)a.y_out)[g] = ((const int32_t*)a.set_y)[id];
        }
    }
}

DEV void topo_hier_init(int C, TopoScratch& s) {
    FOR_TID(c, C + 1) { s.t4[c] = (C > 0) ? C - 1 : 0; s.rp1[c] = 0; s.nb[c] = 0; }
}
DEV void topo_hier(const TopoView& tv, int g, int n0, int N, int C, int C1, const int* cl0, TopoScratch& s) {
    const int rowbase = n0 + g;
    const int* qpos = s.t4;
    int* ptr = s.rp1;
    int* cur = s.nb;
    int* tmp = s.t1;
    int* slot_bucket = s.t2;
    long long* best = (long long*)s.fl;
    FOR_TID(i, N) { ATOMIC_ADD(&ptr[qpos[cl0[i]]], 1); }
    FOR_TID(i, 1) { best[0] = LLONG_MAX; }
    BARRIER();
    wg_exscan(ptr, C + 1, s.part);
    int32_t* g_hord = tv.p[DRGNN_TI_HORD] + n0;
    int32_t* g_ihord = tv.p[DRGNN_TI_IHORD] + n0;
    int32_t* g_hmp = tv.p[DRGNN_TI_HMP0] + rowbase;
    FOR_TID(i, N) {
        const int b = qpos[cl0[i]];
        const int pos = ptr[b] + ATOMIC_ADD(&cur[b], 1);
        tmp[pos] = i;
        slot_bucket[pos] = b;
    }
    FOR_TID(q, C + 1) { g_hmp[q] = ptr[q]; }
    FOR_TID(k, C1 + 1) {
        const int pos = ptr[imin(s.mp[k], C)];
        int d = 2 * pos - N;
        d = d < 0 ? -d : d;
        ATOMIC_MIN64(&best[0], ((long long)d << 32) | (long long)k);
    }
    BARRIER();
    FOR_TID(p, N) {
        const int b = slot_bucket[p];
        const int me = tmp[p];
        const int lo = ptr[b], hi = ptr[b + 1];
        int rank = 0;
        for (int q = lo; q < hi; ++q) rank += (tmp[q] < me) ? 1 : 0;
        g_hord[lo + rank] = me;
        g_ihord[me] = lo + rank;
    }
    FOR_TID(i, 1) {
        const int k = (int)(best[0] & 0xffffffffLL);
        const int q = imin(s.mp[k], C);
        int32_t* hs = tv.p[DRGNN_TI_HSPLIT] + 4 * g;
        hs[0] = k; hs[1] = q; hs[2] = ptr[q]; hs[3] = C1;
    }
}

DEV void topo_graph_level1(const TopoView& tv, const TopoArgs& a, int g, int n0, int C0, const int64_t* ids1,
                           int c1_len, TopoScratch& s, int sidx, bool prepared = false, const int* cl0 = nullptr,
                           int N = 0, bool hier_ready = false) {
    const int rowbase = n0 + g;
    if (c1_len != C0) {
        FOR_TID(i, 1) { topo_flag(tv, DRGNN_S_CLUSTER1_LEN, sidx); }
    }
    const int n = imin(C0, imax(c1_len, 0));
    if (cl0 != nullptr && !hier_ready) { topo_hier_init(C0, s); BARRIER(); }
    const int C1 = wg_cluster_rank(tv, sidx, ids1, n, s, prepared, true, cl0 != nullptr ? s.t4 : nullptr);
    int32_t* g_cl1 = tv.p[DRGNN_TI_CL1] + n0;
    int32_t* g_mptr1 = tv.p[DRGNN_TI_MPTR1] + rowbase;
    int32_t* g_mem1 = tv.p[DRGNN_TI_MEM1] + n0;
    FOR_TID(i, n) { g_cl1[i] = s.cl[i]; g_mem1[i] = s.mem[i]; }
    FOR_TID(c, C1 + 1) { g_mptr1[c] = s.mp[c]; }
    FOR_TID(i, 1) { tv.p[DRGNN_TI_NC1][g] = C1; }
    BARRIER();
    if (cl0 != nullptr) topo_hier(tv, g, n0, N, C0, C1, cl0, s);
}

#define TOPO_ROLE_ALL 0
#define TOPO_ROLE_EDGES 1
#define TOPO_ROLE_MEMBERS 2

DEV void topo_stage_edges(const TopoView& tv, const TopoSrc& src, int g, int N, int E, bool has_w, TopoScratch& s) {
    const int64_t* src_row = src.row;
    const int64_t* src_col = src.col;
    const long long shift = src.shift;
    const int Nm1 = N - 1;
    FOR_TID(e, E) {
        long long r = (long long)src_row[e] - shift, c = (long long)src_col[e] - shift;
        if (r < 0 || r > Nm1 || c < 0 || c > Nm1) {
            topo_flag(tv, DRGNN_S_EDGE_RANGE, g);
            r = (r < 0 || r > Nm1) ? 0 : r;
            c = (c < 0 || c > Nm1) ? 0 : c;
        }
        s.er[e] = (int)r;
        s.ec[e] = (int)c;
        if (has_w) s.w0[e] = src.attr[e];
    }
}

DEV void topo_csr0(const TopoView& tv, int g, int n0, int e0, int N, int E, bool has_w, TopoScratch& s) {
    const int rowbase = n0 + g;
    int32_t* g_rowptr0 = tv.p[DRGNN_TI_ROWPTR0] + rowbase;
    int32_t* g_col0 = tv.p[DRGNN_TI_COL0] + e0;
    int32_t* g_eid0 = tv.p[DRGNN_TI_EID0] + e0;
    float* g_w0 = tv.w0 ? tv.w0 + e0 : nullptr;
    int* rp = s.rp;
    int* cp = s.rp + (N + 1);
    int* cur_r = s.cur;
    int* cur_c = s.nb;
    FOR_TID(e, E) {
        ATOMIC_ADD(&rp[s.er[e]], 1);
        ATOMIC_ADD(&cp[s.ec[e]], 1);
    }
    BARRIER();
    wg_exscan(rp, 2 * N + 2, s.part);
    FOR_TID(e, E) {
        const int r = s.er[e], c = s.ec[e];
        s.t1[rp[r] + ATOMIC_ADD(&cur_r[r], 1)] = e;
        s.t2[cp[c] - E + ATOMIC_ADD(&cur_c[c], 1)] = e;
    }
    BARRIER();
    FOR_TID(p, E) {
        {
            const int e = s.t1[p];
            const int lo = rp[s.er[e]], hi = rp[s.er[e] + 1];
            int rank = 0;
            for (int q = lo; q < hi; ++q) rank += (s.t1[q] < e) ? 1 : 0;
            s.t3[lo + rank] = e;
        }
        {
            const int e = s.t2[p];
            const int lo = cp[s.ec[e]] - E, hi = cp[s.ec[e] + 1] - E;
            int rank = 0;
            for (int q = lo; q < hi; ++q) rank += (s.t2[q] < e) ? 1 : 0;
            s.t4[lo + rank] = e;
        }
    }
    BARRIER();
    FOR_TID(k, E) {
        const int e = s.t3[k];
        s.t5[e] = k;
        s.col[k] = s.ec[e];
        if (has_w) ((float*)s.seg)[k] = s.w0[e];
        g_col0[k] = s.ec[e];
        g_eid0[k] = e;
        if (has_w) g_w0[k] = s.w0[e];
    }
    {
        int32_t* g_colptr0 = tv.p[DRGNN_TI_COLPTR0] + rowbase;
        FOR_TID(i, N + 1) { g_rowptr0[i] = rp[i]; g_colptr0[i] = cp[i] - E; }
    }
    BARRIER();
    {
        int32_t* g_rowidx0 = tv.p[DRGNN_TI_ROWIDX0] + e0;
        int32_t* g_tslot0 = tv.p[DRGNN_TI_TSLOT0] + e0;
        FOR_TID(j, E) {
            const int e = s.t4[j];
            g_rowidx0[j] = s.er[e];
            g_tslot0[j] = s.t5[e];
        }
    }
    BARRIER();
}

DEV void topo_pool(const TopoView& tv, int g, int n0, int e0, int E, int C, bool has_w, TopoScratch& s) {
    const int rowbase = n0 + g;
    float* g_w1 = tv.w1 ? tv.w1 + e0 : nullptr;
    const int BW = (C + 31) >> 5;
    const bool bitmap = !has_w && (long)C * BW + 1 <= (long)s.capT;
    int E1;
    int32_t* g_rowptr1 = tv.p[DRGNN_TI_ROWPTR1] + rowbase;
    int32_t* g_col1 = tv.p[DRGNN_TI_COL1] + e0;
    if (bitmap) {
        int* bm = s.t1;
        int* pre = s.t2;
        FOR_TID(q, C * BW) { bm[q] = 0; }
        BARRIER();
        FOR_TID(e, E) {
            const int r = s.cl[s.er[e]], cc = s.cl[s.ec[e]];
            if (cc != r) ATOMIC_OR(&bm[r * BW + (cc >> 5)], (int)(1u << (cc & 31)));
        }
        BARRIER();
        FOR_TID(q, C * BW + 1) { pre[q] = (q < C * BW) ? __builtin_popcount((unsigned)bm[q]) : 0; }
        BARRIER();
        E1 = wg_exscan(pre, C * BW + 1, s.part);
        FOR_TID(q, C * BW) {
            unsigned bits = (unsigned)bm[q];
            const int r = q / BW, base_col = (q - r * BW) << 5;
            int slot = pre[q];
            while (bits) {
                const int b = __builtin_ctz(bits);
                bits &= bits - 1;
                s.col1[slot] = base_col + b;
                s.seg[slot] = r;
                g_col1[slot] = base_col + b;
                ++slot;
            }
        }
        FOR_TID(r, C + 1) {
            const int v = pre[r * BW];
            s.rp1[r] = v;
            g_rowptr1[r] = v;
            s.cp[r] = 0;
            s.cur[r] = 0;
        }
        FOR_TID(i, 1) { tv.p[DRGNN_TI_NE1][g] = E1; }
        BARRIER();
    } else {
        FOR_TID(r, C + 1) { s.pp[r] = 0; s.cur[r] = 0; }
        FOR_TID(i, 1) { TOPO_WMAX(s)[0] = 0; }
        BARRIER();
        {
            int mine = 0;
            FOR_TID(e, E) {
                ATOMIC_ADD(&s.pp[s.cl[s.er[e]]], 1);
                if (has_w) { const int b = topo_f2i(fabsf(s.w0[e])) & 0x7fffffff; mine = b > mine ? b : mine; }
            }
#ifdef DRGNN_EMU
            if (has_w) ATOMIC_MAX(TOPO_WMAX(s), mine);
#else
            if (has_w && (int)(threadIdx.x & ~(DRGNN_WAVE - 1)) < E) {
#pragma unroll
                for (int m = 1; m < DRGNN_WAVE; m <<= 1) { const int o = __shfl_xor(mine, m, DRGNN_WAVE); mine = o > mine ? o : mine; }
                if ((threadIdx.x & (DRGNN_WAVE - 1)) == 0) ATOMIC_MAX(TOPO_WMAX(s), mine);
            }
#endif
        }
        BARRIER();
        wg_exscan(s.pp, C + 1, s.part);
        constexpr int DROPPED = 0x7FFF;
        const bool packed = (E <= 0x10000) && (C <= DROPPED);
        FOR_TID(e, E) {
            const int r = s.cl[s.er[e]];
            const int cc = s.cl[s.ec[e]];
            const int j = s.pp[r] + ATOMIC_ADD(&s.cur[r], 1);
            if (packed) {
                s.t1[j] = (((cc == r) ? DROPPED : cc) << 16) | e;
            } else {
                s.t1[j] = (cc == r) ? INT_MAX : cc;
                s.t2[j] = e;
            }
            s.t3[j] = r;
        }
        BARRIER();
        FOR_TID(j, E) {
            const int r = s.t3[j];
            const int mine = s.t1[j];
            const int lo = s.pp[r], hi = s.pp[r + 1];
            if (packed) {
                const int rank = rank_below(s.t1, lo, hi, mine);
                const int key = mine >> 16;
                s.t4[lo + rank] = (key == DROPPED) ? INT_MAX : key;
                s.t5[lo + rank] = mine & 0xFFFF;
            } else {
                const int id = s.t2[j];
                int rank = 0;
                for (int q = lo; q < hi; ++q) {
                    const int kq = s.t1[q];
                    rank += (kq < mine || (kq == mine && s.t2[q] < id)) ? 1 : 0;
                }
                s.t4[lo + rank] = mine;
                s.t5[lo + rank] = id;
            }
        }
        BARRIER();
        float* const wv = reinterpret_cast<float*>(s.t2);
        FOR_TID(j, E + 1) {
            int head = 0;
            if (j < E) {
                const int key = s.t4[j];
                head = (key != INT_MAX && (j == s.pp[s.t3[j]] || s.t4[j - 1] != key)) ? 1 : 0;
                if (has_w) wv[j] = s.w0[s.t5[j]];
            }
            s.t1[j] = head;
        }
        BARRIER();
        E1 = wg_exscan(s.t1, E + 1, s.part);
        double winv = 1.0;
        const double wsc = has_w ? topo_wscale(TOPO_WMAX(s)[0], &winv) : 1.0;
        FOR_TID(j, E) {
            const int key = s.t4[j];
            const int r = s.t3[j];
            if (key != INT_MAX && (j == s.pp[r] || s.t4[j - 1] != key)) {
                const int slot = s.t1[j];
                s.col1[slot] = key;
                s.seg[slot] = r;
                g_col1[slot] = key;
                if (has_w) {
                    const int hi = s.pp[r + 1];
                    long long w = 0;
                    int q = j;
                    for (; q + 3 < hi; q += 4) {
                        const int k0 = s.t4[q], k1 = s.t4[q + 1], k2 = s.t4[q + 2], k3 = s.t4[q + 3];
                        const float v0 = wv[q], v1 = wv[q + 1], v2 = wv[q + 2], v3 = wv[q + 3];
                        const bool e0 = k0 == key, e1 = e0 && k1 == key, e2 = e1 && k2 == key, e3 = e2 && k3 == key;
                        if (e0) w += topo_wfix(v0, wsc);
                        if (e1) w += topo_wfix(v1, wsc);
                        if (e2) w += topo_wfix(v2, wsc);
                        if (e3) w += topo_wfix(v3, wsc);
                        if (!e3) { q = hi; break; }
                    }
                    for (; q < hi && s.t4[q] == key; ++q) w += topo_wfix(wv[q], wsc);
                    g_w1[slot] = (float)((double)w * winv);
                }
            }
        }
        FOR_TID(r, C + 1) {
            const int v = s.t1[s.pp[r]];
            s.rp1[r] = v;
            g_rowptr1[r] = v;
            s.cp[r] = 0;
            s.cur[r] = 0;
        }
        FOR_TID(i, 1) { tv.p[DRGNN_TI_NE1][g] = E1; }
        BARRIER();
    }
    wg_csc_build(C, E1, s.col1, s.seg, s, tv.p[DRGNN_TI_COLPTR1] + rowbase,
                 tv.p[DRGNN_TI_ROWIDX1] + e0, tv.p[DRGNN_TI_TSLOT1] + e0, true);
}

DEV int topo_clusters0(const TopoView& tv, int g, int n0, int N, const TopoSrc& src, TopoScratch& s, int sidx,
                       bool with_members, bool ranks_out = false) {
    const int rowbase = n0 + g;
    const int C = wg_cluster_rank(tv, sidx, src.cl0, N, s, true, with_members);
    if (!with_members && ranks_out) {
        int32_t* g_cl0 = tv.p[DRGNN_TI_CL0] + n0;
        FOR_TID(i, N) { g_cl0[i] = s.cl[i]; }
        FOR_TID(i, 1) { tv.p[DRGNN_TI_NC0][g] = C; }
    }
    if (with_members) {
        int32_t* g_cl0 = tv.p[DRGNN_TI_CL0] + n0;
        int32_t* g_mptr0 = tv.p[DRGNN_TI_MPTR0] + rowbase;
        int32_t* g_mem0 = tv.p[DRGNN_TI_MEM0] + n0;
        FOR_TID(i, N) { g_cl0[i] = s.cl[i]; g_mem0[i] = s.mem[i]; }
        FOR_TID(c, C + 1) { g_mptr0[c] = s.mp[c]; }
        FOR_TID(i, 1) { tv.p[DRGNN_TI_NC0][g] = C; }
    }
    return C;
}
DEV void topo_clusters1(const TopoView& tv, const TopoArgs& a, int g, int n0, int N, int C, const TopoSrc& src, TopoScratch& s,
                        int sidx) {
    if (a.cluster1 == nullptr || a.c1_ptr == nullptr) return;
    const bool hier = (a.flags & DRGNN_TOPO_HIER) != 0;
    FOR_TID(v, s.capF) { s.fl[v] = 0; }
    if (hier) {
        FOR_TID(i, N) { s.t5[i] = s.cl[i]; }
        topo_hier_init(C, s);
    }
    const int b = a.c1_ptr[g];
    const int c1_len = a.c1_ptr[g + 1] - b;
    wg_rank_prepare(src.cl1, imin(C, imax(c1_len, 0)), s);
    BARRIER();
    topo_graph_level1(tv, a, g, n0, C, src.cl1, c1_len, s, sidx, true, hier ? s.t5 : nullptr, N, true);
}

struct TopoTile { const float* x; float* ts; float* td; float* tc; float* tx; float* xs; int F, TF; };
#ifdef DRGNN_EMU
struct TopoTouch { int dummy; };
DEV void topo_touch_load(TopoTouch&, const float*, int) {}
DEV void topo_touch_done(const TopoTouch&) {}
#else
struct TopoTouch { drgnn_f4 v[4]; };
DEV void topo_touch_load(TopoTouch& t, const float* p, int words) {
#ifdef DRGNN_NO_TOUCH
    const int n4 = 0;
#else
    const int n4 = p ? (words >> 2) : 0;
#endif
#pragma unroll
    for (int j = 0; j < 4; ++j) {
        const int q = threadIdx.x + j * DRGNN_NTHREADS;
        t.v[j] = drgnn_f4{0.f, 0.f, 0.f, 0.f};
        if (q < n4) t.v[j] = ((const drgnn_f4*)p)[q];
    }
}
DEV void topo_touch_done(const TopoTouch& t) {
#pragma unroll
    for (int j = 0; j < 4; ++j) asm volatile("" :: "v"(t.v[j]));
}
#endif
DEV TopoTile topo_tile_of(const TopoArgs& a, const TopoSrc& src, int n0, float* xs) {
    TopoTile t;
    t.F = (a.tiles != nullptr) ? a.tile_f : 0;
    const float* xsrc = a.set_ids ? a.set_x : a.x_in;
    if (xsrc == nullptr || xs == nullptr) t.F = 0;
    t.x = (t.F > 0) ? xsrc + src.x_row * t.F : nullptr;
    t.TF = (t.F + 3) & ~3;
    t.ts = (t.F > 0) ? a.tiles + (long long)n0 * t.TF : nullptr;
    t.td = (t.F > 0) ? a.tiles + a.tile_nodes * t.TF + n0 : nullptr;
    t.tc = (t.F > 0) ? t.td + a.tile_nodes : nullptr;
    t.tx = (t.F > 0 && (t.F & 3)) ? a.tiles + drgnn_tiles_x_off(a.tile_nodes, t.TF) + (long long)n0 * t.TF : nullptr;
    t.xs = xs;
    return t;
}
#ifdef DRGNN_EMU
struct TopoTileRegs { int dummy; };
DEV void topo_tile_load(TopoTileRegs&, const TopoTile&, int) {}
DEV void topo_tile_store(const TopoTileRegs&, const TopoTile& t, int N) {
    for (int i = 0; i < N && t.F > 0; ++i)
        for (int f = 0; f < t.TF; ++f) t.xs[i * (t.TF + 4) + f] = (f < t.F) ? t.x[(long long)i * t.F + f] : 0.0f;
}
#else
struct TopoTileRegs { BurstX<4> bx; };
DEV void topo_tile_load(TopoTileRegs& r, const TopoTile& t, int N) { if (t.F > 0 && !(t.F & 3)) burst_load_x(r.bx, t.x, N, t.F); }
DEV void topo_tile_store(const TopoTileRegs& r, const TopoTile& t, int N) {
    if (t.F <= 0) return;
    if (!(t.F & 3)) { burst_store_x4(r.bx, t.xs, t.F + 4); return; }
    const FastDiv fd = fastdiv_make(t.TF);
    FOR_TID(e, N * t.TF) {
        const int i = fastdiv(fd, e), f = fastmod(fd, e, i);
        t.xs[i * (t.TF + 4) + f] = (f < t.F) ? t.x[(long long)i * t.F + f] : 0.0f;
    }
}
#endif
DEV void topo_tiles_rows(const TopoTile& t, int N, const int* rp, const int* col_s, const float* w_s) {
    if (t.F <= 0) return;
    const int F = t.TF, G4 = F >> 2, XLD = F + 4;
    const FastDiv fd = fastdiv_make(G4);
    FOR_TID(item, N * G4) {
        const int i = fastdiv(fd, item), c = fastmod(fd, item, i) * 4;
        const int lo = rp[i], hi = rp[i + 1], deg = hi - lo;
        float a0 = 0.f, a1 = 0.f, a2 = 0.f, a3 = 0.f, asum = 0.f;
        if (w_s != nullptr) {
            for (int k = lo; k < hi; k += 4) {
                int kk[4];
                float cf[4];
                for (int j = 0; j < 4; ++j) { kk[j] = (k + j < hi) ? k + j : hi - 1; cf[j] = (k + j < hi) ? 1.0f : 0.0f; }
                for (int j = 0; j < 4; ++j) { cf[j] *= w_s[kk[j]]; asum += cf[j]; }
                const float* xj[4];
                for (int j = 0; j < 4; ++j) xj[j] = t.xs + ROW24(col_s[kk[j]], XLD) + c;
                for (int j = 0; j < 4; ++j) {
                    a0 = fmaf(cf[j], xj[j][0], a0); a1 = fmaf(cf[j], xj[j][1], a1);
                    a2 = fmaf(cf[j], xj[j][2], a2); a3 = fmaf(cf[j], xj[j][3], a3);
                }
            }
        } else {
#ifndef DRGNN_EMU
#pragma unroll 4
#endif
            for (int k = lo; k < hi; ++k) {
                const float* xj = t.xs + ROW24(col_s[k], XLD) + c;
                a0 += xj[0]; a1 += xj[1]; a2 += xj[2]; a3 += xj[3];
            }
        }
        out_store16(t.ts, i * F + c, N * F, a0, a1, a2, a3);
        if (t.tx != nullptr) {
            const float* xi = t.xs + ROW24(i, XLD) + c;
            out_store16(t.tx, i * F + c, N * F, xi[0], xi[1], xi[2], xi[3]);
        }
        if (c == 0) {
            float d, sc;
            if (w_s != nullptr) { d = 1.0f / (float)(deg > 0 ? deg : 1); sc = asum * d; }
            else { d = deg > 0 ? 1.0f / (float)deg : 0.0f; sc = 1.0f; }
            out_store(&t.td[i], d); out_store(&t.tc[i], sc);
        }
    }
}

#ifdef DRGNN_EMU
#define TOPO_LANES(G) 1
template <int G> DEV int topo_group_sum(int v) { return v; }
#else
#define TOPO_LANES(G) (G)
template <int CTRL> DEV int dpp_take_int(int v) { return __builtin_amdgcn_update_dpp(0, v, CTRL, 0xF, 0xF, false); }
template <int G> DEV int topo_group_sum(int v) {
    if (G >= 2) v += dpp_take_int<0xB1>(v);
    if (G >= 4) v += dpp_take_int<0x4E>(v);
    if (G >= 8) v += dpp_take_int<0x141>(v);
    if (G >= 16) v += dpp_take_int<0x140>(v);
    return v;
}
#endif
template <int G> DEV int topo_count_below(const int* keys, int n, int me, int sub) {
    constexpr int L = TOPO_LANES(G);
    int cnt = 0;
    for (int j = sub; j < n; j += 4 * L) {
        const int j1 = j + L, j2 = j + 2 * L, j3 = j + 3 * L;
        const int k0 = keys[j], k1 = keys[j1 < n ? j1 : j], k2 = keys[j2 < n ? j2 : j], k3 = keys[j3 < n ? j3 : j];
        cnt += ((k0 < me) ? 1 : 0) + ((j1 < n && k1 < me) ? 1 : 0) + ((j2 < n && k2 < me) ? 1 : 0) + ((j3 < n && k3 < me) ? 1 : 0);
    }
    return topo_group_sum<L>(cnt);
}

DEV void topo_lean_preclear(int N, TopoScratch& s, bool rows, bool clusters) {
    if (rows) { FOR_TID(i, N + 1) { s.rp[i] = 0; s.cur[i] = 0; } }
    if (clusters) {
        FOR_TID(v, imin(2 * N + 2, s.capF)) { s.fl[v] = 0; }
        FOR_TID(i, 1) { TOPO_OVF(s)[0] = (2 * N + 2 > s.capF) ? 1 : 0; TOPO_WMAX(s)[0] = 0; }
    }
}
DEV void topo_lean_flag(long long v, int i, int* Z, int N, int* key, TopoScratch& s) {
    if ((unsigned long long)v < (unsigned long long)N) { Z[(int)v] = 1; key[i] = (int)v; }
    else { TOPO_OVF(s)[0] = 1; key[i] = 0; }
}
DEV void topo_lean_prepare(const TopoSrc& src, int N, int E, int n1, bool rows, bool clusters, TopoScratch& s, bool pre = false,
                           long long v0 = 0, long long v1 = 0) {
    if (rows) { FOR_TID(e, E) { ATOMIC_ADD(&s.rp[s.er[e]], 1); } }
    if (clusters && 2 * N + 2 <= s.capF) {
        const int R = N + 1;
        FOR_TID(i, N + 1) { s.cp[i] = 0; }
#ifndef DRGNN_EMU
        if (pre) {
            if ((int)threadIdx.x < N) topo_lean_flag(v0, threadIdx.x, s.fl, N, s.pp, s);
// ... 137 lines not shown
        constexpr int G = TOPO_LANES(8);
        FOR_TID(item, (C + 1) * G) {
            const int q = item / G, sub = item % G;
            int acc = 0;
            for (int c = sub; c < C; c += G) acc += (qpos[c] < q) ? csize[c] : 0;
            acc = topo_group_sum<G>(acc);
            if (sub == 0) { hmp[q] = acc; out_store(&g_hmp[q], acc); }
        }
    }
    if (rows && tile.F > 0) topo_tiles_rows(tile, N, s.rp, s.col, has_w ? (const float*)s.wr : nullptr);
    auto emit_pooled = [&](const int* Y, const int E1) {
        int32_t* g_col1 = tv.p[DRGNN_TI_COL1] + e0;
        int32_t* g_rowidx1 = tv.p[DRGNN_TI_ROWIDX1] + e0;
        int32_t* g_tslot1 = tv.p[DRGNN_TI_TSLOT1] + e0;
        FOR_TID_FROM(q, 2 * CB, 512) {
            const bool tr = q >= CB;
            const int qq = tr ? q - CB : q;
            unsigned bits = (unsigned)(tr ? bmT[qq] : bm[qq]);
            const int r = qq / BW, base = (qq - r * BW) << 5;
            int slot = Y[q] - (tr ? E1 : 0);
            int32_t* dst = tr ? g_rowidx1 : g_col1;
            while (bits) {
                const int b = __builtin_ctz(bits);
                bits &= bits - 1;
                out_store(&dst[slot], base + b);
                if (tr && has_w) {
                    const int row = base + b, w_ = row * BW + (r >> 5);
                    out_store(&g_tslot1[slot], Y[w_] + __builtin_popcount((unsigned)bm[w_] & ((1u << (r & 31)) - 1u)));
                }
                ++slot;
            }
        }
        if (has_w) {
            double inv_unused;
            const double scale = topo_wscale(wmax_bits[0], &inv_unused);
            long long* acc = (long long*)s.seg;
            FOR_TID(e, E) {
                const int r = s.cl[s.er[e]], cc = s.cl[s.ec[e]];
                if (cc != r) {
                    const int w_ = r * BW + (cc >> 5);
                    const int slot = Y[w_] + __builtin_popcount((unsigned)bm[w_] & ((1u << (cc & 31)) - 1u));
                    ATOMIC_ADD64(&acc[slot], topo_wfix(s.w0[e], scale));
                }
            }
        }
        int32_t* g_rowptr1 = tv.p[DRGNN_TI_ROWPTR1] + rowbase;
        int32_t* g_colptr1 = tv.p[DRGNN_TI_COLPTR1] + rowbase;
        FOR_TID(r, C + 1) { out_store(&g_rowptr1[r], Y[r * BW]); out_store(&g_colptr1[r], Y[CB + r * BW] - E1); }
        FOR_TID(i, 1) { out_store(&tv.p[DRGNN_TI_NE1][g], E1); }
    };
    auto node_claim = [&]() {
    FOR_TID_FROM(i, N, 768) {
        const int c = s.cl[i], b = qpos[c];
        const int pos = hmp[b] + ATOMIC_ADD(&s.cur[c], 1);
        s.t5[pos] = i;
        s.nb[pos] = b;
    }
    };
    auto hier_tail = [&]() {
    {
        int32_t* g_hord = tv.p[DRGNN_TI_HORD] + n0;
        int32_t* g_ihord = tv.p[DRGNN_TI_IHORD] + n0;
        FOR_TID(p, N) {
            const int me = s.t5[p], b = s.nb[p];
            const int lo = hmp[b], hi = hmp[b + 1];
            int rank = 0;
            for (int q = lo; q < hi; ++q) rank += (s.t5[q] < me) ? 1 : 0;
            out_store(&g_hord[lo + rank], me);
            out_store(&g_ihord[me], lo + rank);
        }
    }
    {
        int32_t* hs = tv.p[DRGNN_TI_HSPLIT] + 4 * g;
#ifdef DRGNN_EMU
        long long best = LLONG_MAX;
        for (int k = 0; k <= C1; ++k) {
            int d = 2 * hmp[imin(mp1[k], C)] - N;
            d = d < 0 ? -d : d;
            const long long v = ((long long)d << 32) | (long long)k;
            best = v < best ? v : best;
        }
        const int kb = (int)(best & 0xffffffffLL);
        const int qb = imin(mp1[kb], C);
        out_store(&hs[0], kb); out_store(&hs[1], qb); out_store(&hs[2], hmp[qb]); out_store(&hs[3], C1);
#else
        if (threadIdx.x < DRGNN_WAVE) {
            long long best = LLONG_MAX, other = LLONG_MIN;
            for (int k = threadIdx.x; k <= C1; k += DRGNN_WAVE) {
                int d = 2 * hmp[imin(mp1[k], C)] - N;
                d = d < 0 ? -d : d;
                const long long v = ((long long)d << 32) | (long long)k;
                best = v < best ? v : best;
            }
            wave_minmax_i64(best, other);
            if (threadIdx.x == 0) {
                const int kb = (int)(best & 0xffffffffLL);
                const int qb = imin(mp1[kb], C);
                out_store(&hs[0], kb); out_store(&hs[1], qb); out_store(&hs[2], hmp[qb]); out_store(&hs[3], C1);
            }
        }
#endif
    }
    };
#ifndef DRGNN_EMU
    if (with_pool && !has_w && 2 * CB + 1 <= DRGNN_NTHREADS) {
        int* Y = s.t4;
        const int t = threadIdx.x, ny = 2 * CB + 1;
        const int lane = t & (DRGNN_WAVE - 1), wave = t >> 6, nw = (ny + DRGNN_WAVE - 1) / DRGNN_WAVE;
        int v = 0, inc = 0;
        if (wave < nw) {
            v = (t < CB) ? __builtin_popcount((unsigned)bm[t]) : (t < 2 * CB) ? __builtin_popcount((unsigned)bmT[t - CB]) : 0;
            inc = wave_incl_scan(v);
            if (lane == DRGNN_WAVE - 1) s.part[wave] = inc;
        }
        BARRIER();
        int base = 0, total = 0;
        for (int w = 0; w < nw; ++w) {
            const int tw = s.part[w];
            base += (w < wave) ? tw : 0;
            total += tw;
        }
        if (t < ny) Y[t] = base + inc - v;
        node_claim();
        BARRIER();
        emit_pooled(Y, total >> 1);
        hier_tail();
        return 0;
    }
#endif
    if (with_pool) {
        int* Y = s.t4;
        FOR_TID(q, 2 * CB + 1) { Y[q] = (q < CB) ? __builtin_popcount((unsigned)bm[q]) : (q < 2 * CB) ? __builtin_popcount((unsigned)bmT[q - CB]) : 0; }
        if (2 * CB + 1 > DRGNN_NTHREADS) BARRIER();
        const int E1 = wg_exscan(Y, 2 * CB + 1, s.part) >> 1;
        emit_pooled(Y, E1);
    } else {
        BARRIER();
    }
    node_claim();
    BARRIER();
    if (with_pool && has_w) {
        double inv;
        (void)topo_wscale(wmax_bits[0], &inv);
        const long long* acc = (const long long*)s.seg;
        float* g_w1 = tv.w1 + e0;
        const int E1 = s.t4[CB];
        FOR_TID(q, E1) { out_store(&g_w1[q], (float)((double)acc[q] * inv)); }
    }
    hier_tail();
    return 0;
}

template <int WEIGHTS = -1>
DEV void topo_graph(const TopoView& tv, const TopoArgs& a, int g, int n0, int n1, int e0, int e1,
                    TopoScratch& s, int role = TOPO_ROLE_ALL) {
    const int N = n1 - n0;
    int E = e1 - e0;
    const int sidx = (role == TOPO_ROLE_MEMBERS) ? a.n_graphs + g : g;
    if (N <= 0 && E > 0) {
        FOR_TID(i, 1) { topo_flag(tv, DRGNN_S_EDGE_RANGE, sidx); }
        E = 0;
    }
    PHASE_MARK();
    const TopoSrc src = topo_src(a, g, n0, e0);
    const bool has_w = (WEIGHTS != 0) && (a.edge_attr != nullptr) && (tv.w0 != nullptr);
    const bool structure = (role != TOPO_ROLE_EDGES);
    const bool pool = (role != TOPO_ROLE_MEMBERS);
    if (structure) topo_gather_rows(a, src, g, n0, N);

    const bool lean = (a.flags & DRGNN_TOPO_LEAN) != 0 && (a.flags & DRGNN_TOPO_HIER) != 0 && a.cluster0 != nullptr &&
                      a.cluster1 != nullptr && a.c1_ptr != nullptr;
    const int c1_len = lean ? a.c1_ptr[g + 1] - a.c1_ptr[g] : 0;
    const int nc1 = imin(N, imax(c1_len, 0));
    const bool run_rows = lean && structure;
    const bool run_clusters = lean && pool;
    const TopoTile tile = topo_tile_of(a, src, n0, structure ? s.xs : nullptr);
    TopoTileRegs treg;
    topo_tile_load(treg, tile, N);
    TopoTouch touch;
    topo_touch_load(touch, (run_rows || (structure && !lean)) ? tile.ts : nullptr, N * tile.TF);
    long long pre0 = 0, pre1 = 0;
    bool pre = false;
#ifndef DRGNN_EMU
    if (run_clusters && N <= DRGNN_NTHREADS) {
        pre = true;
        if ((int)threadIdx.x < N) pre0 = (long long)src.cl0[threadIdx.x];
        if ((int)threadIdx.x < nc1) pre1 = (long long)src.cl1[threadIdx.x];
    }
#endif
    topo_stage_edges(tv, src, sidx, N, E, has_w, s);
    topo_tile_store(treg, tile, N);
    topo_touch_done(touch);
    bool rows_done = false, need_c1 = false;
    if (run_rows || run_clusters) {
        topo_lean_prepare(src, N, E, nc1, run_rows, run_clusters, s, pre, pre0, pre1);
        BARRIER();
        if (run_rows && !run_clusters) {
            topo_lean_rows(tv, g, n0, e0, N, E, has_w, s, tile);
            return;
        }
        const int rc = topo_lean_clusters(tv, g, n0, e0, N, E, c1_len, true, has_w, s, sidx, run_rows, tile);
        if (rc == 0) return;
        if (run_rows) {
            if (rc == 1) topo_lean_rows(tv, g, n0, e0, N, E, has_w, s, tile);
            else topo_lean_rows_tail(tv, g, n0, e0, N, E, has_w, s, tile);
            rows_done = true;
        }
        need_c1 = true;
        BARRIER();
    }
    if (structure && !rows_done) {
        FOR_TID(i, 2 * N + 2) { s.rp[i] = 0; }
        FOR_TID(i, N + 1) { s.cur[i] = 0; }
        FOR_TID(i, N) { s.nb[i] = 0; }
    }
    FOR_TID(v, s.capF) { s.fl[v] = 0; }
    if (a.cluster0 != nullptr) wg_rank_prepare(src.cl0, N, s);
    BARRIER();

    if (structure && !rows_done) {
        topo_csr0(tv, g, n0, e0, N, E, has_w, s);
        topo_tiles_rows(tile, N, s.rp, s.col, has_w ? (const float*)s.seg : nullptr);
    }
    if (a.cluster0 == nullptr) {
        FOR_TID(i, 1) { tv.p[DRGNN_TI_NC0][g] = 0; tv.p[DRGNN_TI_NE1][g] = 0; tv.p[DRGNN_TI_NC1][g] = 0; }
        BARRIER();
        return;
    }
    if (role == TOPO_ROLE_MEMBERS) {
        const int C = topo_clusters0(tv, g, n0, N, src, s, sidx, false);
        topo_clusters1(tv, a, g, n0, N, C, src, s, sidx);
        return;
    }
    const bool members0 = !(lean && role == TOPO_ROLE_EDGES);
    const int C = topo_clusters0(tv, g, n0, N, src, s, sidx, members0, true);
    BARRIER();
    topo_pool(tv, g, n0, e0, E, C, has_w, s);
    if (role == TOPO_ROLE_ALL || need_c1) topo_clusters1(tv, a, g, n0, N, C, src, s, sidx);
}
```

### deeprank-gnn_amd/data.py

```python
import copy

import torch

__all__ = ["Data", "Batch", "DataLoader"]


def _is_index_key(key):
    return ("index" in key) or ("face" in key)


class Data(object):

    def __init__(self, x=None, edge_index=None, edge_attr=None, y=None, pos=None, **extra):
        store = self.__dict__
        store["x"] = x
        store["edge_index"] = edge_index
        store["edge_attr"] = edge_attr
        store["y"] = y
        store["pos"] = pos
        store.update(extra)

    def keys(self):
        return [k for k, v in self.__dict__.items() if v is not None and not k.startswith("_")]

    def __getitem__(self, key):
        return self.__dict__.get(key)

    def __setitem__(self, key, value):
        self.__dict__[key] = value

    def __contains__(self, key):
        return self.__dict__.get(key) is not None

    def __iter__(self):
        for k in self.keys():
            yield k, self.__dict__[k]

    @property
    def num_nodes(self):
        for key in ("x", "pos", "batch", "cluster0"):
            v = self.__dict__.get(key)
            if torch.is_tensor(v):
                return v.size(0)
        ei = self.__dict__.get("edge_index")
        if torch.is_tensor(ei) and ei.numel():
            return int(ei.max()) + 1
        return 0

    @property
    def num_edges(self):
        ei = self.__dict__.get("edge_index")
        return 0 if ei is None else ei.size(-1)

    @property
    def num_features(self):
        x = self.__dict__.get("x")
        if x is None:
            return 0
        return 1 if x.dim() == 1 else x.size(1)

    num_node_features = num_features

    def apply(self, fn):
        for k, v in self.__dict__.items():
            if torch.is_tensor(v):
                self.__dict__[k] = fn(v)
        return self

    def to(self, device, non_blocking=False):
        return self.apply(lambda t: t.to(device, non_blocking=non_blocking))

    def cpu(self):
        return self.to("cpu")

    def cuda(self, device=None):
        return self.to("cuda" if device is None else device)

    def clone(self):
        twin = self.__class__.__new__(self.__class__)
        for k, v in self.__dict__.items():
            twin.__dict__[k] = v.clone() if torch.is_tensor(v) else copy.deepcopy(v)
        return twin

    def __repr__(self):
        parts = []
        for k, v in self:
            parts.append("%s=%s" % (k, list(v.shape) if torch.is_tensor(v) else type(v).__name__))
        return "%s(%s)" % (self.__class__.__name__, ", ".join(parts))


class Batch(Data):

    def __init__(self, batch=None, **kw):
        super().__init__(**kw)
        self.__dict__["batch"] = batch

    @property
    def num_graphs(self):
        ng = self.__dict__.get("_num_graphs")
        if ng is None:
            b = self.__dict__.get("batch")
            ng = 0 if b is None or b.numel() == 0 else int(b.max()) + 1
            self.__dict__["_num_graphs"] = ng
        return ng

    @classmethod
    def from_data_list(cls, graphs):
        if len(graphs) == 0:
            raise ValueError("cannot batch an empty list of graphs")
        names = list(graphs[0].keys())
        pieces = {k: [] for k in names}
        owner = []
        shift = 0
        for gid, g in enumerate(graphs):
            n = g.num_nodes
            for k in names:
                v = g[k]
                if torch.is_tensor(v) and _is_index_key(k) and shift:
                    v = v + shift
                pieces[k].append(v)
            owner.append(torch.full((n,), gid, dtype=torch.long))
            shift += n
        out = cls()
        for k in names:
            first = pieces[k][0]
            if torch.is_tensor(first):
                vals = [v.reshape(1) if v.dim() == 0 else v for v in pieces[k]]
                out[k] = torch.cat(vals, dim=-1 if _is_index_key(k) else 0)
            elif isinstance(first, (int, float, bool)):
                out[k] = torch.tensor(pieces[k])
            else:
                out[k] = pieces[k]
        out["batch"] = torch.cat(owner, dim=0)
        out.__dict__["_num_graphs"] = len(graphs)
        out._record_layout(graphs)
        return out

    def _record_layout(self, graphs):
        nodes = [g.num_nodes for g in graphs]
        edges = [g.num_edges for g in graphs]

        def ptr(counts):
            t = torch.zeros(len(counts) + 1, dtype=torch.int32)
            if counts:
                t[1:] = torch.tensor(counts, dtype=torch.int64).cumsum(0).to(torch.int32)
            return t
        d = self.__dict__
        d["_node_ptr"] = ptr(nodes)
        d["_edge_ptr"] = ptr(edges)
        d["_host_node_ptr"] = d["_node_ptr"].numpy().copy()
        d["_host_edge_ptr"] = d["_edge_ptr"].numpy().copy()
        d["_max_nodes"] = max(nodes) if nodes else 0
        d["_max_edges"] = max(edges) if edges else 0
        c1 = [g["cluster1"] for g in graphs]
        if all(torch.is_tensor(c) for c in c1):
            lens = [int(c.numel()) for c in c1]
            d["_c1_ptr"] = ptr(lens)
            d["_max_c0"] = max(lens) if lens else 0


class DataLoader(torch.utils.data.DataLoader):

    def __init__(self, dataset, batch_size=1, shuffle=False, **kw):
        kw.pop("collate_fn", None)
        super().__init__(dataset, batch_size=batch_size, shuffle=shuffle,
                         collate_fn=Batch.from_data_list, **kw)
```

### deeprank-gnn_amd/topology.py

```python
import torch

from . import _lib

__all__ = ["Topology"]


def _contig(t, dtype):
    if t is None:
        return None
    if t.dtype != dtype:
        t = t.to(dtype)
    return t.contiguous()


class Topology(object):
    def __init__(self, api, n_nodes, n_edges, n_graphs, device, has_weights):
        self.api = api
        self.n_nodes, self.n_edges, self.n_graphs = int(n_nodes), int(n_edges), int(n_graphs)
        self.off_i32, self.off_f32 = api.topology_layout(self.n_nodes, self.n_edges, self.n_graphs)
        self.ws_i32 = torch.empty(max(self.off_i32[-1], 4), dtype=torch.int32, device=device)
        self.ws_f32 = (torch.empty(max(self.off_f32[-1], 4), dtype=torch.float32, device=device)
                       if has_weights else None)
        self.max_nodes = 0
        self.max_edges = 0
        self.max_c0 = 0
        self.host_node_ptr = self.host_edge_ptr = None
        self.has_level1 = False
        self.flags = _lib.TOPO_HIER
        self.x = None
        self.tiles = None
        self._tiles_x_version = None
        self.n_feat = 0
        self._finalized = False

    @classmethod
    def from_batch(cls, data, api=None, with_level1=True, check=False, need_weights=True, graph_only=False,
                   build=True, flags=None, with_tiles=True, host_tables=True):
        api = api or _lib.get()
        edge_index = _contig(data.edge_index, torch.int64)
        batch = _contig(data.batch, torch.int64)
        if api is _lib._API:
            _lib.require_device(edge_index, batch)
        device = batch.device
        n_nodes = batch.numel()
        n_edges = edge_index.size(1) if edge_index.dim() == 2 else 0
        edge_attr = getattr(data, "edge_attr", None) if need_weights else None
        if edge_attr is not None:
            if edge_attr.dim() == 2 and edge_attr.size(1) != 1:
                raise ValueError("only one edge feature is supported (the reference's layers "
                                 "broadcast edge_attr [E,1] over the channels, sGAT.py:76)")
            edge_attr = _contig(edge_attr.reshape(-1), torch.float32)
        cluster0 = _contig(getattr(data, "cluster0", None), torch.int64)
        if cluster0 is None and not graph_only:
            raise ValueError("the batch has no cluster0 (pre-computed communities, DataSet.py:342-357)")
        if graph_only:
            cluster0 = None
            with_level1 = False
        cluster1 = _contig(getattr(data, "cluster1", None), torch.int64) if with_level1 else None
        d = getattr(data, "__dict__", {})
        n_graphs = d.get("_num_graphs")
        if n_graphs is None:
            n_graphs = getattr(data, "num_graphs", None)
        if n_graphs is None:
            n_graphs = int(batch.max()) + 1 if n_nodes else 0
        node_ptr = _contig(d.get("_node_ptr"), torch.int32)
        edge_ptr = _contig(d.get("_edge_ptr"), torch.int32)
        c1_ptr = _contig(d.get("_c1_ptr"), torch.int32) if cluster1 is not None else None
        for t in (node_ptr, edge_ptr, c1_ptr):
            if t is not None and t.device != device:
                node_ptr = edge_ptr = c1_ptr = None
                break
        topo = cls(api, n_nodes, n_edges, n_graphs, device, edge_attr is not None)
        max_nodes = int(d.get("_max_nodes", 0))
        max_edges = int(d.get("_max_edges", 0))
        max_c0 = int(d.get("_max_c0", 0))
        if max_nodes == 0 and n_nodes and n_graphs:
            cn = torch.bincount(batch, minlength=n_graphs)
            be = batch[edge_index[0]] if n_edges else None
            ce = torch.bincount(be, minlength=n_graphs) if n_edges else torch.zeros_like(cn)
            cc = torch.zeros_like(cn)
            if cluster0 is not None:
                lo = cluster0.min()
                span = cluster0.max() - lo + 1
                keys = torch.unique(batch * span + (cluster0 - lo))
                cc = torch.bincount(torch.div(keys, span, rounding_mode="floor"), minlength=n_graphs)
            grouped = (batch[1:] >= batch[:-1]).all() if n_nodes > 1 else torch.ones((), dtype=torch.bool, device=device)
            if n_edges > 1:
                grouped = grouped & (be[1:] >= be[:-1]).all()
            flag = grouped.to(cn.dtype).reshape(1).expand(n_graphs)
            counts = torch.stack([cn[:n_graphs], ce[:n_graphs], cc[:n_graphs], flag]).cpu()
            max_nodes, max_edges = int(counts[0].max()), int(counts[1].max())
            if cluster0 is not None:
                max_c0 = int(counts[2].max())
            if host_tables and node_ptr is None and bool(counts[3, 0]) and int(counts[0].sum()) == n_nodes and \
                    int(counts[1].sum()) == n_edges and cn.numel() == n_graphs:
                ptr = torch.zeros((3, n_graphs + 1), dtype=torch.int32)
                ptr[:, 1:] = torch.cumsum(counts[:3], dim=1).to(torch.int32)
                dev_ptr = ptr.to(device)
                node_ptr, edge_ptr = dev_ptr[0], dev_ptr[1]
                if cluster1 is not None and int(counts[2].sum()) == cluster1.numel():
                    c1_ptr = dev_ptr[2]
                topo.host_node_ptr, topo.host_edge_ptr = ptr[0].numpy(), ptr[1].numpy()
        topo.max_nodes, topo.max_edges = max_nodes, max_edges
        topo.max_c0 = max_c0
        scratch = None
        lds_limit = 160 * 1024
        need = api.topology_lds_bytes(max_nodes, max_edges)
        if max_nodes == 0 or need > lds_limit:
            scratch = torch.empty(api.topology_scratch_elems(n_nodes, n_edges, n_graphs),
                                  dtype=torch.int32, device=device)
        topo.has_level1 = cluster1 is not None
        topo._inputs = (edge_index, edge_attr, batch, cluster0, cluster1, node_ptr, edge_ptr, c1_ptr, scratch)
        x = getattr(data, "x", None) if (with_tiles and cluster1 is not None) else None
        if x is not None and x.dim() == 2 and x.dtype == torch.float32 and x.device == device and scratch is None:
            x = x.contiguous()
            F = int(x.shape[1])
            if x.shape[0] == n_nodes and F > 0 and (F % 4 != 0 or x.data_ptr() % 16 == 0) and \
                    (api.topology_tiles_ok(max_nodes, max_edges, F) or (F <= 64 and max_nodes < 1024 and max_edges <= 2048)):
                topo.x, topo.n_feat = x, F
                topo.tiles = torch.empty(max(api.topology_tiles_elems(n_nodes, F), 4), dtype=torch.float32, device=device)
                topo._tiles_separately = not api.topology_tiles_ok(max_nodes, max_edges, F)
        if build:
            topo.rebuild(flags)
            if check:
                topo.check()
        return topo

    def request(self, flags=None):
        edge_index, edge_attr, batch, cluster0, cluster1, node_ptr, edge_ptr, c1_ptr, scratch = self._inputs
        r = _lib.TopologyRequest()
        p = _lib._ptr
        r.edge_index, r.edge_attr, r.batch, r.cluster0, r.cluster1 = p(edge_index), p(edge_attr), p(batch), p(cluster0), p(cluster1)
        r.node_ptr, r.edge_ptr, r.c1_ptr = p(node_ptr), p(edge_ptr), p(c1_ptr)
        r.n_nodes, r.n_edges, r.n_graphs = self.n_nodes, self.n_edges, self.n_graphs
        r.len_cluster1 = 0 if cluster1 is None else cluster1.numel()
        r.max_nodes, r.max_edges = self.max_nodes, self.max_edges
        r.ws_i32, r.ws_f32, r.scratch_i32 = p(self.ws_i32), p(self.ws_f32), p(scratch)
        r.flags = self.full_flags() if flags is None else int(flags)
        self._tiles_pending = False
        if (r.flags & _lib.TOPO_TILES) and getattr(self, "_tiles_separately", False):
            r.flags &= ~_lib.TOPO_TILES
            self._tiles_pending = True
        if r.flags & _lib.TOPO_TILES:
            if self.tiles is None:
                raise ValueError("this topology has no aggregation tiles (no float32 x the builder's LDS holds a tile of)")
            r.x, r.tiles, r.n_feat = p(self.x), p(self.tiles), self.n_feat
            self._tiles_x_version = self.x._version
        self.flags = int(r.flags)
        self._finalized = False
        return r

    def full_flags(self):
        own = self.tiles is not None and not getattr(self, "_tiles_separately", False)
        return _lib.TOPO_HIER | (_lib.TOPO_TILES if own else 0)

    def rebuild(self, flags=None):
        edge_index, edge_attr, batch, cluster0, cluster1, node_ptr, edge_ptr, c1_ptr, scratch = self._inputs
        if flags is None:
            flags = self.full_flags()
        if int(flags) != _lib.TOPO_HIER:
            stream = _lib.current_stream(batch)
            self.api.topology_build_request(self.request(flags), stream)
            if getattr(self, "_tiles_pending", False):
                self.api.topology_tiles(self.ws_i32, self.ws_f32, self.n_nodes, self.n_edges, self.n_graphs, self.x, self.n_feat,
                                        self.ws_f32 is not None, self.tiles, stream)
                self._tiles_x_version = self.x._version
                self.flags |= _lib.TOPO_TILES
                self._tiles_pending = False
            return self
        self.flags = _lib.TOPO_HIER
        self.api.topology_build(edge_index, edge_attr, batch, cluster0, cluster1, node_ptr, edge_ptr, c1_ptr,
                                self.n_nodes, self.n_edges, 0 if cluster1 is None else cluster1.numel(),
                                self.n_graphs, self.max_nodes, self.max_edges, self.ws_i32, self.ws_f32,
                                scratch, _lib.current_stream(batch))
        self._finalized = False
        return self

    @classmethod
    def single_graph(cls, edge_index, edge_attr, n_nodes, api=None, cluster=None):
        import types
        dev = edge_index.device if edge_index is not None else cluster.device
        if edge_index is None:
            edge_index = torch.zeros((2, 0), dtype=torch.int64, device=dev)
        shadow = types.SimpleNamespace(
            edge_index=edge_index, edge_attr=edge_attr,
            batch=torch.zeros(n_nodes, dtype=torch.int64, device=dev), cluster0=cluster, cluster1=None)
        shadow.__dict__["_num_graphs"] = 1 if n_nodes > 0 else 0
        shadow.__dict__["_node_ptr"] = torch.tensor([0, n_nodes], dtype=torch.int32, device=dev)
        shadow.__dict__["_edge_ptr"] = torch.tensor([0, edge_index.size(1)], dtype=torch.int32, device=dev)
        shadow.__dict__["_max_nodes"] = n_nodes
        shadow.__dict__["_max_edges"] = int(edge_index.size(1))
        return cls.from_batch(shadow, api=api, with_level1=False, graph_only=cluster is None)

    def totals(self):
        self.finalize()
        B = self.n_graphs
        vals = torch.stack([self.array("CPTR0")[B], self.array("E1PTR")[B], self.array("CPTR1")[B]]).tolist()
        return int(vals[0]), int(vals[1]), int(vals[2])

    def array(self, name):
        k = _lib.TI[name]
        return self.ws_i32[self.off_i32[k]:self.off_i32[k + 1]]

    def tile_arrays(self):
        n, F = self.n_nodes, self.n_feat
        TF = (F + 3) // 4 * 4
        t = self.tiles
        return t[:n * TF].view(n, TF)[:, :F], t[n * TF:n * TF + n], t[n * TF + n:n * TF + 2 * n]

    def weights(self, name):
        k = _lib.TF[name]
        return self.ws_f32[self.off_f32[k]:self.off_f32[k + 1]]

    def status(self):
        return self.api.topology_status(self.ws_i32, self.n_nodes, self.n_edges, self.n_graphs,
                                        _lib.current_stream(self.ws_i32))

    def check(self):
        st = self.status()
        if st[0]:
            msgs = [m for bit, m in _lib.STATUS_BITS.items() if st[0] & bit]
            raise _lib.DrgnnError("malformed batch (graph %d): %s" % (st[1], "; ".join(msgs)))

    def finalize(self):
        if not self._finalized:
            self.api.topology_finalize(self.ws_i32, self.n_nodes, self.n_edges, self.n_graphs,
                                       _lib.current_stream(self.ws_i32))
            self._finalized = True
        return self
```

### include/drgnn.h

```cpp
#ifndef DRGNN_H
#define DRGNN_H

#include <stdint.h>

#ifdef __cplusplus
extern "C" {
#endif

#define DRGNN_ABI_VERSION 5

#define DRGNN_E_ARG      (-1)
#define DRGNN_E_CAPACITY (-2)
#define DRGNN_E_WIDTH    (-3)

#define DRGNN_S_EDGE_RANGE    1
#define DRGNN_S_UNSORTED      2
#define DRGNN_S_CLUSTER_RANGE 4
#define DRGNN_S_CLUSTER1_LEN  8
#define DRGNN_FAULT_EXCHANGE  1
#define DRGNN_FAULT_SPLIT     2

#define DRGNN_GINET 0
#define DRGNN_SGAT  1
#define DRGNN_FOUT  2
// ... 11 lines not shown
    DRGNN_TI_NC0,
    DRGNN_TI_MPTR0,
    DRGNN_TI_MEM0,
    DRGNN_TI_ROWPTR1,
    DRGNN_TI_COL1,
    DRGNN_TI_NE1,
    DRGNN_TI_COLPTR1,
    DRGNN_TI_ROWIDX1,
    DRGNN_TI_TSLOT1,
    DRGNN_TI_CL1,
    DRGNN_TI_NC1,
    DRGNN_TI_MPTR1,
    DRGNN_TI_MEM1,
    DRGNN_TI_CPTR0,
    DRGNN_TI_E1PTR,
    DRGNN_TI_CPTR1,
    DRGNN_TI_ERR,
    DRGNN_TI_GSTAT,
    DRGNN_TI_HORD,
    DRGNN_TI_HMP0,
    DRGNN_TI_HSPLIT,
    DRGNN_TI_IHORD,
    DRGNN_TI_COUNT
};
enum drgnn_topo_f32 {
    DRGNN_TF_W0 = 0,
    DRGNN_TF_W1,
    DRGNN_TF_COUNT
};

int drgnn_topology_layout(int64_t n_nodes, int64_t n_edges, int64_t n_graphs,
                          int64_t* off_i32, int64_t* off_f32);

int64_t drgnn_topology_scratch_elems(int64_t n_nodes, int64_t n_edges, int64_t n_graphs);
int64_t drgnn_topology_lds_bytes(int32_t max_nodes, int32_t max_edges);
int drgnn_topology_build(const int64_t* edge_index, const float* edge_attr,
                         const int64_t* batch, const int64_t* cluster0, const int64_t* cluster1,
                         const int32_t* node_ptr, const int32_t* edge_ptr, const int32_t* c1_ptr,
                         int64_t n_nodes, int64_t n_edges, int64_t len_cluster1, int64_t n_graphs,
                         int32_t max_nodes, int32_t max_edges,
                         int32_t* ws_i32, float* ws_f32, int32_t* scratch_i32, void* stream);

int drgnn_topology_finalize(int32_t* ws_i32, int64_t n_nodes, int64_t n_edges,
                            int64_t n_graphs, void* stream);

int drgnn_topology_status(const int32_t* ws_i32, int64_t n_nodes, int64_t n_edges,
                          int64_t n_graphs, int32_t* status4, void* stream);

typedef struct drgnn_conv_params {
    const float* w_nbr;  int64_t nbr_sk, nbr_sh;
    const float* w_self; int64_t self_sk, self_sh;
    const float* bias;
} drgnn_conv_params;

typedef struct drgnn_conv_grads {
    float* w_nbr;
    float* w_self;
    float* bias;
} drgnn_conv_grads;

#define DRGNN_MAX_BRANCH 2

typedef struct drgnn_net_desc {
    int32_t kind;
    int32_t n_branch;
    int32_t n_feat;
    int32_t reserved;
    drgnn_conv_params conv1[DRGNN_MAX_BRANCH];
    drgnn_conv_params conv2[DRGNN_MAX_BRANCH];
} drgnn_net_desc;

int64_t drgnn_net_lds_bytes(int32_t kind, int32_t n_feat, int32_t max_nodes, int32_t max_edges,
                            int32_t max_c0, int32_t backward);

int drgnn_net_forward(const drgnn_net_desc* net, const float* x,
                      const int32_t* ws_i32, const float* ws_f32,
                      int64_t n_nodes, int64_t n_edges, int64_t n_graphs,
                      int32_t max_nodes, int32_t max_edges, int32_t max_c0,
                      float* xp, int32_t* arg0, int32_t* arg1, float* readout,
                      float* scratch_f32, int32_t* step_inc ,
                      void* stream);

int64_t drgnn_net_partial_elems(int32_t kind, int32_t n_feat);
int64_t drgnn_net_scratch_elems(int32_t kind, int32_t n_feat, int64_t n_nodes, int64_t n_edges,
                                int64_t n_graphs);
int drgnn_net_backward(const drgnn_net_desc* net, const float* x, const float* grad_readout,
                       const int32_t* ws_i32, const float* ws_f32,
                       int64_t n_nodes, int64_t n_edges, int64_t n_graphs,
                       int32_t max_nodes, int32_t max_edges, int32_t max_c0,
                       const float* xp, const int32_t* arg0, const int32_t* arg1,
                       float* grad_x, float* partials, float* scratch_f32,
                       int32_t* step_inc , void* stream);

int drgnn_net_reduce_grads(const drgnn_net_desc* net, const float* partials, int64_t n_nodes,
                           int64_t n_graphs, drgnn_conv_grads* g_conv1, drgnn_conv_grads* g_conv2,
                           float* grad_x, void* stream);

int64_t drgnn_conv_layer_slabs(int64_t n_nodes);
int64_t drgnn_conv_layer_partial_elems(int32_t kind, int32_t F, int32_t H);
int drgnn_conv_layer_forward(int32_t kind, const float* x, int64_t n_nodes, int32_t F, int32_t H,
                             const drgnn_conv_params* p, const int32_t* ws_i32, const float* ws_f32,
                             int64_t n_edges, float* u, float* out, void* stream);
int drgnn_conv_layer_backward(int32_t kind, const float* x, int64_t n_nodes, int32_t F, int32_t H,
                              const drgnn_conv_params* p, const int32_t* ws_i32, const float* ws_f32,
                              int64_t n_edges, const float* grad_out, float* du, float* partials,
                              const drgnn_conv_grads* g, float* grad_x, void* stream);
int drgnn_segpool_forward(const int32_t* ws_i32, int64_t n_nodes, int64_t n_edges, int64_t n_graphs,
                          const float* x, int32_t H, int32_t op, float* out, int64_t* arg, void* stream);
int drgnn_segmax_backward(const float* grad_out, const int64_t* arg, int64_t n_clusters, int32_t H,
                          int64_t n_nodes, float* grad_x , void* stream);
int drgnn_pooled_edges_export(const int32_t* ws_i32, const float* ws_f32, int64_t n_nodes, int64_t n_edges,
                              int64_t n_graphs, int64_t e1_total, int64_t* edge_index, float* edge_attr,
                              void* stream);
int drgnn_cluster_offset(int64_t* cluster, const int32_t* node_ptr, int64_t n_graphs, int64_t* scratch,
                         void* stream);

#define DRGNN_TASK_REG   0
#define DRGNN_TASK_CLASS 1
#define DRGNN_TASK_GRAD  2
typedef struct drgnn_head_desc {
    int32_t R, H, O;
    int32_t task;
    int32_t train;
    float   p_drop;
    uint32_t seed;
    int32_t transform_sigmoid;
    const float* w1; const float* b1; const float* w2; const float* b2;
    const float* class_w;
    const float* drop_mask;
} drgnn_head_desc;

typedef struct drgnn_graph_set {
    int64_t n_graphs, n_nodes, n_edges, len_cluster1;
    int32_t n_feat, y_bytes;
    const int64_t* node_ptr; const int64_t* edge_ptr; const int64_t* c1_ptr;
    const float* x; const int64_t* edge_index; const float* edge_attr;
    const int64_t* cluster0; const int64_t* cluster1; const void* y;
} drgnn_graph_set;
typedef struct drgnn_topology_request {
    const int64_t* edge_index; const float* edge_attr; const int64_t* batch;
    const int64_t* cluster0; const int64_t* cluster1;
    const int32_t* node_ptr; const int32_t* edge_ptr; const int32_t* c1_ptr;
    int64_t n_nodes, n_edges, len_cluster1, n_graphs;
    int32_t max_nodes, max_edges;
    int32_t* ws_i32; float* ws_f32; int32_t* scratch_i32;
    const drgnn_graph_set* set; const int32_t* ids; float* x_out; void* y_out;
    int32_t flags, reserved;
    const float* x; float* tiles;
    int32_t n_feat, reserved2;
} drgnn_topology_request;
#define DRGNN_TOPO_HIER 1
#define DRGNN_TOPO_LEAN 2
#define DRGNN_TOPO_TILES 4
int64_t drgnn_topology_tiles_elems(int64_t n_nodes, int32_t n_feat);
int32_t drgnn_topology_tiles_ok(int32_t max_nodes, int32_t max_edges, int32_t n_feat);
int drgnn_topology_tiles(const int32_t* ws_i32, const float* ws_f32, int64_t n_nodes, int64_t n_edges, int64_t n_graphs,
                         const float* x, int32_t n_feat, int32_t use_weights, float* tiles, void* stream);
int drgnn_topology_build_request(const drgnn_topology_request* request, void* stream);
int drgnn_batch_offsets(const drgnn_graph_set* set, const int32_t* ids, int64_t n_ids, int32_t batch_size,
                        int32_t* ptrs, void* stream);

int64_t drgnn_net_head_stage_bytes(int32_t R, int32_t H, int32_t O);
int drgnn_net_backward_fused_head(const drgnn_net_desc* net, const drgnn_head_desc* head, const float* x,
                                  const float* readout, const void* target, const int32_t* step,
                                  const int32_t* ws_i32, const float* ws_f32, int64_t n_nodes,
                                  int64_t n_edges, int64_t n_graphs, int32_t max_nodes, int32_t max_edges,
                                  int32_t max_c0, const float* xp, const int32_t* arg0, const int32_t* arg1,
                                  float* pred, float* head_partials, float* grad_x, float* partials,
                                  float* scratch_f32,
                                  const drgnn_topology_request* next_topology ,
                                  void* stream);

int64_t drgnn_head_partial_elems(int32_t R, int32_t H, int32_t O);
int64_t drgnn_head_num_slabs(int64_t n_graphs);
int32_t drgnn_head_pass_units(int32_t R, int32_t H, int32_t O, int64_t n_graphs);
int drgnn_head_step(const drgnn_head_desc* head, const float* readout, const void* target,
                    int64_t n_graphs, const int32_t* step, float* pred, float* grad_readout,
                    float* partials, void* stream);
int drgnn_head_reduce(const float* partials, int64_t n_graphs, int32_t R, int32_t H, int32_t O,
                      float* grad_block, float* loss, int32_t* step, void* stream);
int drgnn_adam_step(float* param, const float* grad, float* exp_avg, float* exp_avg_sq,
                    const int32_t* step, int64_t n, double lr, double beta1, double beta2, double eps,
                    double weight_decay, void* stream);

int drgnn_train_update(const drgnn_net_desc* net, const float* conv_partials, int64_t n_graphs,
                       drgnn_conv_grads* g_conv1, drgnn_conv_grads* g_conv2,
                       const float* head_partials, int64_t head_slabs ,
                       int32_t R, int32_t H, int32_t O, int64_t head_offset, float* flat_param, float* flat_grad, float* exp_avg,
                       float* exp_avg_sq, int64_t n_param, const int32_t* step, float* loss,
                       double lr, double beta1, double beta2, double eps, int32_t apply_adam, void* stream);

#define DRGNN_STEP_FAMILY_NONE 0
#define DRGNN_STEP_FAMILY_PRODUCT 1
#define DRGNN_STEP_FAMILY_AGGREGATE 2
typedef struct drgnn_step_plan {
    int32_t kind, n_feat, max_nodes, max_edges, max_c0, R, H, O;
    int64_t n_graphs;
    int64_t co_built_graphs;
    int32_t train;
    int32_t topo_flags;
    int32_t force_wgs, no_class, no_aggregate, no_split, no_paired;
    int32_t family, wgs_per_graph, slabs_per_graph, width, cls, lean_ok, builder_wgs_per_graph;
    int64_t lds_bytes, xchg_words;
    int32_t from_memory, reserved;
} drgnn_step_plan;
int32_t drgnn_net_step_plan(drgnn_step_plan* plan);

typedef struct drgnn_step_hints {
    const int32_t* host_node_ptr; const int32_t* host_edge_ptr;
    const int64_t* set_node_ptr; const int64_t* set_edge_ptr; const int32_t* host_ids;
    int32_t topo_flags, reserved;
    const float* tiles;
    const drgnn_step_plan* plan;
    const int32_t* next_ids; int64_t n_next;
} drgnn_step_hints;
int64_t drgnn_net_step_xchg_elems(int32_t kind, int32_t max_nodes, int32_t max_c0, int32_t H);
int64_t drgnn_net_step_lds_bytes(int32_t kind, int32_t n_feat, int32_t max_nodes, int32_t max_edges,
                                 int32_t max_c0, int32_t R, int32_t H, int32_t O);
int64_t drgnn_head_compact_elems(int32_t R, int32_t H, int32_t O);
int32_t drgnn_net_step_variant(int32_t kind, const float* x, int32_t n_feat, int32_t max_nodes, int32_t max_edges,
                               int32_t max_c0, int32_t H, int32_t O);
int drgnn_net_train_step(const drgnn_net_desc* net, const drgnn_head_desc* head, const float* x,
                         const void* target, int32_t* step2, const int32_t* ws_i32, const float* ws_f32,
                         int64_t n_nodes, int64_t n_edges, int64_t n_graphs, int32_t max_nodes,
                         int32_t max_edges, int32_t max_c0, float* pred, float* readout,
                         float* head_partials, float* partials, uint64_t* xchg,
                         const drgnn_topology_request* next_topology ,
                         const drgnn_step_hints* hints , void* stream);
int drgnn_step_update(const drgnn_net_desc* net, const float* conv_partials, int64_t n_graphs,
                      drgnn_conv_grads* g_conv1, drgnn_conv_grads* g_conv2, const float* head_partials,
                      const float* readout, int32_t R, int32_t H, int32_t O, int64_t head_offset,
                      float* flat_param, float* flat_grad, float* exp_avg, float* exp_avg_sq, int64_t n_param,
                      int32_t* step2, float* loss, double lr, double beta1, double beta2, double eps,
                      int32_t apply_adam, int32_t slabs_per_graph, void* stream);

#define DRGNN_ZERO_RANGES 8
int drgnn_step_gradients(const drgnn_net_desc* net, const float* conv_partials, int64_t n_graphs,
                         drgnn_conv_grads* g_conv1, drgnn_conv_grads* g_conv2, const float* head_partials,
                         const float* readout, int32_t R, int32_t H, int32_t O, float* head_grad,
                         const float* graph_weight, float* const* zero_ptr, const int64_t* zero_len, int32_t n_zero,
                         int32_t* step2, int32_t slabs_per_graph, void* stream);

int drgnn_graclus(const int32_t* ws_i32, int64_t n_nodes, int64_t n_edges, int64_t n_graphs, int32_t max_nodes,
                  int32_t max_edges, const float* weight, const int64_t* perm, int64_t* cluster, void* stream);

int drgnn_mcl(const int64_t* edge_index, int64_t n_edges, const int32_t* node_ptr, const int32_t* edge_ptr,
              const int64_t* mat_ptr, int64_t n_graphs, double* mat_scratch, int32_t* int_scratch,
              int64_t* labels, int32_t* info, void* stream);

int drgnn_louvain(const int64_t* edge_index, int64_t n_edges, const int32_t* node_ptr, const int32_t* edge_ptr,
                  int64_t n_graphs, int32_t max_nodes, int32_t max_edges, int64_t* labels, int32_t* info,
                  double* modularity, void* stream);

#define DRGNN_METRICS_COUNTS     1
#define DRGNN_METRICS_REGRESSION 2
#define DRGNN_METRICS_RANKING    4
int64_t drgnn_metrics_workspace_bytes(int64_t n);
int drgnn_metrics(const double* pred, const double* y, int64_t n, int32_t what, int32_t direction, double threshold,
                  int32_t label_lo, int32_t n_labels, void* workspace, int64_t workspace_bytes, int64_t* counts,
                  double* scores, int32_t* order, int64_t* hits, void* stream);

typedef struct drgnn_iface_request {
    const float* xyz;
    const int32_t* atom_ptr;
    const int32_t* res_ptr;
    const int32_t* res_split;
    const int32_t* res_type;
    const int32_t* host_atom_ptr;
    const int32_t* host_res_ptr;
    const int32_t* host_res_split;
    int64_t n_atoms, n_residues, n_complexes;
    double contact_distance, internal_contact_distance;
    int32_t tile_atoms, reserved;
    void* workspace;
    int64_t workspace_bytes;
    int32_t* node_ptr;
    int32_t* edge_ptr;
    int32_t* iedge_ptr;
} drgnn_iface_request;

int64_t drgnn_iface_workspace_bytes(int64_t n_complexes, int64_t max_res_a, int64_t max_res_b, int64_t n_residues);

int drgnn_iface_count(const drgnn_iface_request* req, void* stream);

int drgnn_iface_fill(const drgnn_iface_request* req, int64_t n_nodes, int64_t n_edges, int64_t n_iedges,
                     int32_t* node_residue, float* pos, int32_t* chain, int32_t* type, int64_t* edge_index, float* dist,
                     int64_t* internal_edge_index, float* internal_dist, void* stream);

typedef struct drgnn_score_request {
    const float* xyz;
    const int32_t* zone_atom;
    const double* zone_ref;
    const int32_t* pair_res;
    const int32_t* atom_ptr;
    const int32_t* host_zone_atom;
    const int32_t* host_zone_ptr;
    const int32_t* host_pair_res;
    const int32_t* host_atom_ptr;
    int64_t n_poses, n_atoms, n_residues, n_pairs, n_ref_pairs;
    double fnat_cutoff;
    double* scores;
    int32_t* classes;
    int32_t* n_preserved;
} drgnn_score_request;

int drgnn_dock_scores(const drgnn_score_request* req, void* stream);
// ... 201 lines not shown
```

Measured before the change: 3.776 million graphs/s.

## Pass per-graph offset tables via kernel arguments and prefetch edges into registers

```diff
diff --git a/deeprank-gnn_amd/_lib.py b/deeprank-gnn_amd/_lib.py
--- a/deeprank-gnn_amd/_lib.py
+++ b/deeprank-gnn_amd/_lib.py
@@ -65,12 +65,23 @@
                 ("ws_i32", _vp), ("ws_f32", _vp), ("scratch_i32", _vp),
                 ("set", _vp), ("ids", _vp), ("x_out", _vp), ("y_out", _vp),
                 ("flags", _c_i32), ("reserved", _c_i32),
-                ("x", _vp), ("tiles", _vp), ("n_feat", _c_i32), ("reserved2", _c_i32)]
+                ("x", _vp), ("tiles", _vp), ("n_feat", _c_i32), ("reserved2", _c_i32),
+                ("host_node_ptr", _vp), ("host_edge_ptr", _vp), ("host_c1_ptr", _vp)]
+
+    def set_host_tables(self, node_ptr, edge_ptr, c1_ptr=None):
+        import numpy as np
+        keep = [None if t is None else np.ascontiguousarray(t, dtype=np.int32) for t in (node_ptr, edge_ptr, c1_ptr)]
+        self._host_keep = keep
+        self.host_node_ptr, self.host_edge_ptr, self.host_c1_ptr = [None if t is None else t.ctypes.data for t in keep]
+        self.flags |= TOPO_HOST_TABLES
+        return self
 
 
 TOPO_HIER = 1
 TOPO_LEAN = 2
 TOPO_TILES = 4
+TOPO_HOST_TABLES = 8
+TOPO_TABLES_MAX = 64
 METRICS_COUNTS, METRICS_REGRESSION, METRICS_RANKING = 1, 2, 4
 
 
diff --git a/deeprank-gnn_amd/csrc/drgnn_capi.hip b/deeprank-gnn_amd/csrc/drgnn_capi.hip
--- a/deeprank-gnn_amd/csrc/drgnn_capi.hip
+++ b/deeprank-gnn_amd/csrc/drgnn_capi.hip
@@ -100,7 +100,8 @@
     L.args.set_ids = nullptr; L.args.set_node_ptr = L.args.set_edge_ptr = L.args.set_c1_ptr = nullptr;
     L.args.set_x = nullptr; L.args.set_y = nullptr; L.args.x_out = nullptr; L.args.y_out = nullptr;
     L.args.n_set = 0; L.args.n_feat = 0; L.args.y_bytes = 0;
-    L.args.flags = flags;
+    L.args.flags = flags & ~DRGNN_TOPO_HOST_TABLES;
+    L.dims.count = 0;
     L.args.x_in = nullptr; L.args.tiles = nullptr; L.args.tile_nodes = n_nodes; L.args.tile_f = 0;
     if (flags & DRGNN_TOPO_TILES) {
         if (!(flags & DRGNN_TOPO_HIER) || !tiles || (x_in && !(tile_f & 3) && (((uintptr_t)x_in) & 15)) || (((uintptr_t)tiles) & 15)) return DRGNN_E_ARG;
@@ -128,7 +129,33 @@
     return 0;
 }
 
-static int topo_prepare_req(TopoLaunch& T, int64_t* tlds, const drgnn_topology_request* r) {
+static int topo_host_dims(TopoLaunch& L, const drgnn_topology_request* r) {
+    L.dims.count = 0;
+    if (!(r->flags & DRGNN_TOPO_HOST_TABLES)) return 0;
+    const drgnn_topology_request_tables* t = reinterpret_cast<const drgnn_topology_request_tables*>(r);
+    const int64_t B = r->n_graphs;
+    const bool want_c1 = L.args.cluster1 != nullptr && L.args.c1_ptr != nullptr;
+    if (!t->host_node_ptr || !t->host_edge_ptr || (want_c1 && !t->host_c1_ptr)) return 0;
+    if (B < 1 || B > DRGNN_TOPO_TABLES_MAX || !L.user_nptr || !L.user_eptr) return 0;
+    const int32_t* tab[3] = {t->host_node_ptr, t->host_edge_ptr, want_c1 ? t->host_c1_ptr : nullptr};
+    const int64_t total[3] = {r->n_nodes, r->n_edges, r->len_cluster1};
+    const int64_t bound[3] = {r->max_nodes > 0 ? (int64_t)r->max_nodes : INT64_MAX, r->max_nodes > 0 ? (int64_t)(r->max_edges > 0 ? r->max_edges : 1) : INT64_MAX,
+                              INT64_MAX};
+    int32_t* dst[3] = {L.dims.n, L.dims.e, L.dims.c1};
+    for (int k = 0; k < 3; ++k) {
+        for (int64_t g = 0; g <= B; ++g) dst[k][g] = tab[k] ? tab[k][g] : 0;
+        if (!tab[k]) continue;
+        if (tab[k][0] != 0 || (int64_t)tab[k][B] != total[k]) return DRGNN_E_ARG;
+        for (int64_t g = 0; g < B; ++g) {
+            const int64_t len = (int64_t)tab[k][g + 1] - tab[k][g];
+            if (len < 0 || len > bound[k]) return DRGNN_E_ARG;
+        }
+    }
+    L.dims.count = (int)B;
+    return 0;
+}
+
+static int topo_prepare_req_(TopoLaunch& T, int64_t* tlds, const drgnn_topology_request* r) {
     const drgnn_graph_set* gs = r->set;
     if (!gs)
         return topo_prepare(T, tlds, r->edge_index, r->edge_attr, r->batch, r->cluster0, r->cluster1, r->node_ptr,
@@ -152,6 +179,10 @@
     a.n_set = gs->n_graphs; a.n_feat = gs->n_feat; a.y_bytes = gs->y_bytes;
     return 0;
 }
+static int topo_prepare_req(TopoLaunch& T, int64_t* tlds, const drgnn_topology_request* r) {
+    const int rc = topo_prepare_req_(T, tlds, r);
+    return rc ? rc : topo_host_dims(T, r);
+}
 
 static int topology_build_impl(const int64_t* edge_index, const float* edge_attr, const int64_t* batch,
                          const int64_t* cluster0, const int64_t* cluster1, const int32_t* node_ptr,
@@ -159,7 +190,7 @@
                          int64_t n_edges, int64_t len_cluster1, int64_t n_graphs, int32_t max_nodes,
                          int32_t max_edges, int32_t* ws_i32, float* ws_f32, int32_t* scratch_i32,
                          int32_t flags, void* stream_, const float* x_in = nullptr, float* tiles = nullptr,
-                         int32_t tile_f = 0) {
+                         int32_t tile_f = 0, const drgnn_topology_request* req = nullptr) {
     drgnn_stream_t stream = (drgnn_stream_t)stream_;
     TopoLaunch L;
     int64_t lds = 0;
@@ -167,6 +198,7 @@
                            n_nodes, n_edges, len_cluster1, n_graphs, max_nodes, max_edges, ws_i32, ws_f32,
                            scratch_i32, flags, x_in, tiles, tile_f);
     if (rc0) return rc0;
+    if (req && (rc0 = topo_host_dims(L, req))) return rc0;
     if (L.capN == 0 && !scratch_i32) return DRGNN_E_CAPACITY;
     if (n_graphs == 0) return 0;
     PtrArgs pa;
@@ -228,7 +260,7 @@
         return topology_build_impl(r->edge_index, r->edge_attr, r->batch, r->cluster0, r->cluster1, r->node_ptr,
                                    r->edge_ptr, r->c1_ptr, r->n_nodes, r->n_edges, r->len_cluster1, r->n_graphs,
                                    r->max_nodes, r->max_edges, r->ws_i32, r->ws_f32, r->scratch_i32, r->flags, stream_,
-                                   r->x, r->tiles, r->n_feat);
+                                   r->x, r->tiles, r->n_feat, r);
     TopoLaunch L;
     int64_t lds = 0;
     const int rc = topo_prepare_req(L, &lds, r);
diff --git a/deeprank-gnn_amd/csrc/drgnn_kernels.h b/deeprank-gnn_amd/csrc/drgnn_kernels.h
--- a/deeprank-gnn_amd/csrc/drgnn_kernels.h
+++ b/deeprank-gnn_amd/csrc/drgnn_kernels.h
@@ -55,6 +55,10 @@
     }
 }
 
+struct TopoDims {
+    int count;
+    int32_t n[DRGNN_TOPO_TABLES_MAX + 1], e[DRGNN_TOPO_TABLES_MAX + 1], c1[DRGNN_TOPO_TABLES_MAX + 1];
+};
 struct TopoLaunch {
     TopoView tv;
     TopoArgs args;
@@ -68,6 +72,7 @@
     const float* pf_tiles; const float* pf_x; int pf_f; int pf_coef;
     long long pf_tile_nodes;
     const void* pf_y; int pf_y_bytes;
+    TopoDims dims;
 };
 
 #ifdef DRGNN_EMU
@@ -114,6 +119,7 @@
 template <bool LDS, int WEIGHTS = -1>
 DEV void topo_block(const TopoLaunch& L, int blk, int* lds) {
     TopoScratch s;
+    PHASE_MARK();
     if (L.pf_ids != nullptr) { prefetch_block(L, blk); return; }
 #ifdef DRGNN_TOPO_EXIT0
     return;
@@ -125,10 +131,22 @@
         else { const int t = blk - full; g = (full >> 1) + (t >> 1); role = (t & 1) ? TOPO_ROLE_MEMBERS : TOPO_ROLE_EDGES; }
     }
     const int sidx = (role == TOPO_ROLE_MEMBERS) ? L.args.n_graphs + g : g;
-    const int32_t* NP = L.user_nptr ? L.user_nptr : L.tv.p[DRGNN_TI_NPTR];
-    const int32_t* EP = L.user_eptr ? L.user_eptr : L.tv.p[DRGNN_TI_EPTR];
-    const int n0 = NP[g], n1 = NP[g + 1], N = n1 - n0;
-    const int e0 = EP[g], e1 = EP[g + 1], E = e1 - e0;
+    int n0, n1, e0, e1, c1b = 0, c1e = 0;
+    if (L.dims.count > 0) {
+        n0 = L.dims.n[g]; n1 = L.dims.n[g + 1];
+        e0 = L.dims.e[g]; e1 = L.dims.e[g + 1];
+        c1b = L.dims.c1[g]; c1e = L.dims.c1[g + 1];
+    } else {
+        const int32_t* NP = L.user_nptr ? L.user_nptr : L.tv.p[DRGNN_TI_NPTR];
+        const int32_t* EP = L.user_eptr ? L.user_eptr : L.tv.p[DRGNN_TI_EPTR];
+        const bool has_c1 = L.args.c1_ptr != nullptr;
+        const int32_t* CP = has_c1 ? L.args.c1_ptr : NP;
+        n0 = NP[g]; n1 = NP[g + 1];
+        e0 = EP[g]; e1 = EP[g + 1];
+        const int cb = CP[g], ce = CP[g + 1];
+        c1b = has_c1 ? cb : 0; c1e = has_c1 ? ce : 0;
+    }
+    const int N = n1 - n0, E = e1 - e0;
     if (LDS) {
         const int capT = imax(L.capN, L.capE) + 1;
         s = topo_carve(lds, L.capN, L.capE, capT, L.capN + L.capE + 2);
@@ -148,15 +166,14 @@
                 if (g == 0) L.tv.p[DRGNN_TI_ERR][0] = 0;
             }
         }
-        if (fits && (L.args.flags & DRGNN_TOPO_LEAN)) topo_lean_preclear(N, s, role != TOPO_ROLE_EDGES, role != TOPO_ROLE_MEMBERS);
-        BARRIER();
     }
     if (!fits) {
+        if (!L.level1_only) BARRIER();
         FOR_TID(i, 1) { topo_flag(L.tv, DRGNN_S_EDGE_RANGE, sidx); }
         return;
     }
     if (!L.level1_only) {
-        topo_graph<WEIGHTS>(L.tv, L.args, g, n0, n1, e0, e1, s, role);
+        topo_graph<WEIGHTS>(L.tv, L.args, g, n0, n1, e0, e1, c1b, c1e, s, role, (L.args.flags & DRGNN_TOPO_LEAN) != 0);
     } else {
         FOR_TID(i, 1) { s.part[0] = 0; }
         BARRIER();
@@ -378,8 +395,8 @@
 };
 struct StepCoLaunch {
     StepLaunch step;
+    int n_net;
     TopoLaunch topo;
-    int n_net;
 };
 
 #ifndef DRGNN_EMU
@@ -617,11 +634,27 @@
 #undef DRGNN_KA_OFF
 }
 #define DRGNN_KA_LINES(first_byte, end_byte) ((((end_byte) - 1) >> 6) - ((first_byte) >> 6) + 1)
+#define DRGNN_KA_13L(b) "s_load_dword %0, " b ", 0x0\n s_load_dword %0, " b ", 0x40\n s_load_dword %0, " b ", 0x80\n s_load_dword %0, " b ", 0xc0\n" \
+                        "s_load_dword %0, " b ", 0x100\n s_load_dword %0, " b ", 0x140\n s_load_dword %0, " b ", 0x180\n s_load_dword %0, " b ", 0x1c0\n" \
+                        "s_load_dword %0, " b ", 0x200\n s_load_dword %0, " b ", 0x240\n s_load_dword %0, " b ", 0x280\n s_load_dword %0, " b ", 0x2c0\n" \
+                        "s_load_dword %0, " b ", 0x300\n"
+DEV const TopoLaunch& topo_kernarg() {
+    return *reinterpret_cast<const TopoLaunch*>((const char*)__builtin_amdgcn_kernarg_segment_ptr());
+}
+DEV void topo_kernarg_touch() {
+    constexpr int N = DRGNN_KA_LINES(0, (int)sizeof(TopoLaunch));
+    static_assert(N >= 13 && N <= 26, "two runs of thirteen lines cover the block");
+    const char* b0 = (const char*)__builtin_amdgcn_kernarg_segment_ptr();
+    const char* b1 = b0 + 64 * (N - 13);
+    int t;
+    asm volatile(DRGNN_KA_13L("%1") DRGNN_KA_13L("%2") "s_waitcnt lgkmcnt(0)" : "=&s"(t) : "s"(b0), "s"(b1) : "memory");
+}
 template <bool LDS>
-__global__ void __launch_bounds__(DRGNN_NTHREADS) k_topo(TopoLaunch L) {
+__global__ void __launch_bounds__(DRGNN_NTHREADS) k_topo(TopoLaunch L_by_value) {
     extern __shared__ __attribute__((aligned(16))) int smem_i[];
     PHASE_BEGIN();
-    kernarg_touch_lines<DRGNN_KA_LINES(0, (int)sizeof(TopoLaunch))>(0);
+    const TopoLaunch& L = topo_kernarg();
+    topo_kernarg_touch();
     topo_block<LDS>(L, blockIdx.x, smem_i);
 }
 #ifdef DRGNN_KERNELS_MAIN
@@ -656,9 +689,10 @@
     net_block<KIND, BWD, LDS>(L, blockIdx.x, smem_f);
 }
 template <int KIND, bool BWD>
-__global__ void __launch_bounds__(DRGNN_NTHREADS) k_net_co_topo(CoLaunch C) {
+__global__ void __launch_bounds__(DRGNN_NTHREADS) k_net_co_topo(CoLaunch C_by_value) {
     extern __shared__ __attribute__((aligned(16))) float smem_c[];
     PHASE_BEGIN();
+    const CoLaunch& C = *reinterpret_cast<const CoLaunch*>((const char*)__builtin_amdgcn_kernarg_segment_ptr());
     if ((int)blockIdx.x < C.n_net) net_block<KIND, BWD, true>(C.net, blockIdx.x, smem_c);
     else topo_block<true>(C.topo, (int)blockIdx.x - C.n_net, (int*)smem_c);
 }
@@ -666,34 +700,20 @@
     return *reinterpret_cast<const StepCoLaunch*>((const char*)__builtin_amdgcn_kernarg_segment_ptr());
 }
 DEV void co_kernarg_touch() {
-    constexpr int first = (int)offsetof(StepCoLaunch, topo), end = (int)sizeof(StepCoLaunch);
-    constexpr int N0 = 13, N1 = DRGNN_KA_LINES(first, end);
+    constexpr int end = (int)(offsetof(StepCoLaunch, topo) + offsetof(TopoLaunch, dims));
     static_assert(offsetof(StepLaunch, dims) + sizeof(int) >= 0x2c0 && sizeof(StepLaunch) >= 0x340, "the touched lines lie inside the step arguments");
-    static_assert(N1 >= 1 && N1 <= 13, "one asm statement covers 13 lines per part");
+    static_assert(offsetof(StepCoLaunch, n_net) >= ((end - 1) & ~63) - 12 * 64 && ((end - 1) >> 6) >= 25, "thirteen lines cover n_net and the builder's fixed part");
+    static_assert(sizeof(StepCoLaunch) + 64 <= 4096, "kernel arguments (the ensemble / cohort kernels append a few words)");
     const char* b0 = (const char*)__builtin_amdgcn_kernarg_segment_ptr();
-    const char* b1 = b0 + (first & ~63);
+    const char* b1 = b0 + (((end - 1) & ~63) - 12 * 64);
     int t;
-#define DRGNN_KA_OFF(k, N) "i"(64 * ((k) < N ? (k) : N - 1))
-#define DRGNN_KA_13(b) "s_load_dword %0, " b ", %3\n s_load_dword %0, " b ", %4\n s_load_dword %0, " b ", %5\n s_load_dword %0, " b ", %6\n" \
-                       "s_load_dword %0, " b ", %7\n s_load_dword %0, " b ", %8\n s_load_dword %0, " b ", %9\n s_load_dword %0, " b ", %10\n" \
-                       "s_load_dword %0, " b ", %11\n s_load_dword %0, " b ", %12\n s_load_dword %0, " b ", %13\n s_load_dword %0, " b ", %14\n" \
-                       "s_load_dword %0, " b ", %15\n"
-    asm volatile(DRGNN_KA_13("%1")
-                 "s_load_dword %0, %2, %16\n s_load_dword %0, %2, %17\n s_load_dword %0, %2, %18\n s_load_dword %0, %2, %19\n"
-                 "s_load_dword %0, %2, %20\n s_load_dword %0, %2, %21\n s_load_dword %0, %2, %22\n s_load_dword %0, %2, %23\n"
-                 "s_load_dword %0, %2, %24\n s_load_dword %0, %2, %25\n s_load_dword %0, %2, %26\n s_load_dword %0, %2, %27\n"
-                 "s_load_dword %0, %2, %28\n s_waitcnt lgkmcnt(0)"
-                 : "=&s"(t)
-                 : "s"(b0), "s"(b1),
-                   DRGNN_KA_OFF(0, N0), DRGNN_KA_OFF(1, N0), DRGNN_KA_OFF(2, N0), DRGNN_KA_OFF(3, N0), DRGNN_KA_OFF(4, N0), DRGNN_KA_OFF(5, N0),
-                   DRGNN_KA_OFF(6, N0), DRGNN_KA_OFF(7, N0), DRGNN_KA_OFF(8, N0), DRGNN_KA_OFF(9, N0), DRGNN_KA_OFF(10, N0), DRGNN_KA_OFF(11, N0),
-                   DRGNN_KA_OFF(12, N0),
-                   DRGNN_KA_OFF(0, N1), DRGNN_KA_OFF(1, N1), DRGNN_KA_OFF(2, N1), DRGNN_KA_OFF(3, N1), DRGNN_KA_OFF(4, N1), DRGNN_KA_OFF(5, N1),
-                   DRGNN_KA_OFF(6, N1), DRGNN_KA_OFF(7, N1), DRGNN_KA_OFF(8, N1), DRGNN_KA_OFF(9, N1), DRGNN_KA_OFF(10, N1), DRGNN_KA_OFF(11, N1),
-                   DRGNN_KA_OFF(12, N1)
-                 : "memory");
-#undef DRGNN_KA_13
-#undef DRGNN_KA_OFF
+#ifdef DRGNN_AB_TOUCH_DIMS
+    const char* b2 = b0 + (((int)sizeof(StepCoLaunch) - 1) & ~63) - 12 * 64;
+    asm volatile(DRGNN_KA_13L("%1") DRGNN_KA_13L("%2") DRGNN_KA_13L("%3") "s_waitcnt lgkmcnt(0)"
+                 : "=&s"(t) : "s"(b0), "s"(b1), "s"(b2) : "memory");
+#else
+    asm volatile(DRGNN_KA_13L("%1") DRGNN_KA_13L("%2") "s_waitcnt lgkmcnt(0)" : "=&s"(t) : "s"(b0), "s"(b1) : "memory");
+#endif
 }
 #ifdef DRGNN_TOPO_FIRST
 #define STEP_CO_ROLES(C)                                                       \
diff --git a/deeprank-gnn_amd/csrc/drgnn_topology.h b/deeprank-gnn_amd/csrc/drgnn_topology.h
--- a/deeprank-gnn_amd/csrc/drgnn_topology.h
+++ b/deeprank-gnn_amd/csrc/drgnn_topology.h
@@ -387,14 +387,14 @@
     const int64_t* row; const int64_t* col; const float* attr; const int64_t* cl0; const int64_t* cl1;
     long long shift; long long x_row;
 };
-DEV TopoSrc topo_src(const TopoArgs& a, int g, int n0, int e0) {
+DEV TopoSrc topo_src(const TopoArgs& a, int g, int n0, int e0, int c1b) {
     TopoSrc t;
     if (a.set_ids == nullptr) {
         t.row = a.edge_index + e0;
         t.col = a.edge_index + a.n_edges + e0;
         t.attr = a.edge_attr ? a.edge_attr + e0 : nullptr;
         t.cl0 = a.cluster0 ? a.cluster0 + n0 : nullptr;
-        t.cl1 = (a.cluster1 && a.c1_ptr) ? a.cluster1 + a.c1_ptr[g] : nullptr;
+        t.cl1 = (a.cluster1 && a.c1_ptr) ? a.cluster1 + c1b : nullptr;
         t.shift = n0;
         t.x_row = n0;
     } else {
@@ -509,23 +509,56 @@
 #define TOPO_ROLE_EDGES 1
 #define TOPO_ROLE_MEMBERS 2
 
-DEV void topo_stage_edges(const TopoView& tv, const TopoSrc& src, int g, int N, int E, bool has_w, TopoScratch& s) {
-    const int64_t* src_row = src.row;
-    const int64_t* src_col = src.col;
+DEV void topo_stage_edge(const TopoView& tv, int g, int Nm1, int e, long long r, long long c, TopoScratch& s) {
+    if (r < 0 || r > Nm1 || c < 0 || c > Nm1) {
+        topo_flag(tv, DRGNN_S_EDGE_RANGE, g);
+        r = (r < 0 || r > Nm1) ? 0 : r;
+        c = (c < 0 || c > Nm1) ? 0 : c;
+    }
+    s.er[e] = (int)r;
+    s.ec[e] = (int)c;
+}
+#ifdef DRGNN_EMU
+struct TopoEdgeRegs { int dummy; };
+DEV void topo_edges_load(TopoEdgeRegs&, const TopoSrc&, int, bool) {}
+DEV void topo_stage_edges(const TopoView& tv, const TopoSrc& src, int g, int N, int E, bool has_w, TopoScratch& s, const TopoEdgeRegs&) {
+    const long long shift = src.shift;
+    FOR_TID(e, E) {
+        topo_stage_edge(tv, g, N - 1, e, (long long)src.row[e] - shift, (long long)src.col[e] - shift, s);
+        if (has_w) s.w0[e] = src.attr[e];
+    }
+}
+#else
+#define TOPO_EDGE_REGS 2
+struct TopoEdgeRegs { long long r[TOPO_EDGE_REGS], c[TOPO_EDGE_REGS]; float w[TOPO_EDGE_REGS]; };
+DEV void topo_edges_load(TopoEdgeRegs& q, const TopoSrc& src, int E, bool has_w) {
+#pragma unroll
+    for (int j = 0; j < TOPO_EDGE_REGS; ++j) {
+        const int e = threadIdx.x + j * DRGNN_NTHREADS;
+        q.r[j] = 0; q.c[j] = 0; q.w[j] = 0.0f;
+        if (e < E) {
+            q.r[j] = (long long)src.row[e]; q.c[j] = (long long)src.col[e];
+            if (has_w) q.w[j] = src.attr[e];
+        }
+    }
+}
+DEV void topo_stage_edges(const TopoView& tv, const TopoSrc& src, int g, int N, int E, bool has_w, TopoScratch& s, const TopoEdgeRegs& q) {
     const long long shift = src.shift;
     const int Nm1 = N - 1;
-    FOR_TID(e, E) {
-        long long r = (long long)src_row[e] - shift, c = (long long)src_col[e] - shift;
-        if (r < 0 || r > Nm1 || c < 0 || c > Nm1) {
-            topo_flag(tv, DRGNN_S_EDGE_RANGE, g);
-            r = (r < 0 || r > Nm1) ? 0 : r;
-            c = (c < 0 || c > Nm1) ? 0 : c;
-        }
-        s.er[e] = (int)r;
-        s.ec[e] = (int)c;
+#pragma unroll
+    for (int j = 0; j < TOPO_EDGE_REGS; ++j) {
+        const int e = threadIdx.x + j * DRGNN_NTHREADS;
+        if (e < E) {
+            topo_stage_edge(tv, g, Nm1, e, q.r[j] - shift, q.c[j] - shift, s);
+            if (has_w) s.w0[e] = q.w[j];
+        }
+    }
+    _Pragma("nounroll") for (int e = threadIdx.x + TOPO_EDGE_REGS * DRGNN_NTHREADS; e < E; e += DRGNN_NTHREADS) {
+        topo_stage_edge(tv, g, Nm1, e, (long long)src.row[e] - shift, (long long)src.col[e] - shift, s);
         if (has_w) s.w0[e] = src.attr[e];
     }
 }
+#endif
 
 DEV void topo_csr0(const TopoView& tv, int g, int n0, int e0, int N, int E, bool has_w, TopoScratch& s) {
     const int rowbase = n0 + g;
@@ -768,7 +801,7 @@
     return C;
 }
 DEV void topo_clusters1(const TopoView& tv, const TopoArgs& a, int g, int n0, int N, int C, const TopoSrc& src, TopoScratch& s,
-                        int sidx) {
+                        int sidx, int c1_len) {
     if (a.cluster1 == nullptr || a.c1_ptr == nullptr) return;
     const bool hier = (a.flags & DRGNN_TOPO_HIER) != 0;
     FOR_TID(v, s.capF) { s.fl[v] = 0; }
@@ -776,8 +809,6 @@
         FOR_TID(i, N) { s.t5[i] = s.cl[i]; }
         topo_hier_init(C, s);
     }
-    const int b = a.c1_ptr[g];
-    const int c1_len = a.c1_ptr[g + 1] - b;
     wg_rank_prepare(src.cl1, imin(C, imax(c1_len, 0)), s);
     BARRIER();
     topo_graph_level1(tv, a, g, n0, C, src.cl1, c1_len, s, sidx, true, hier ? s.t5 : nullptr, N, true);
@@ -1221,8 +1252,8 @@
 }
 
 template <int WEIGHTS = -1>
-DEV void topo_graph(const TopoView& tv, const TopoArgs& a, int g, int n0, int n1, int e0, int e1,
-                    TopoScratch& s, int role = TOPO_ROLE_ALL) {
+DEV void topo_graph(const TopoView& tv, const TopoArgs& a, int g, int n0, int n1, int e0, int e1, int c1b, int c1e,
+                    TopoScratch& s, int role, bool preclear) {
     const int N = n1 - n0;
     int E = e1 - e0;
     const int sidx = (role == TOPO_ROLE_MEMBERS) ? a.n_graphs + g : g;
@@ -1231,15 +1262,14 @@
         E = 0;
     }
     PHASE_MARK();
-    const TopoSrc src = topo_src(a, g, n0, e0);
+    const TopoSrc src = topo_src(a, g, n0, e0, c1b);
     const bool has_w = (WEIGHTS != 0) && (a.edge_attr != nullptr) && (tv.w0 != nullptr);
     const bool structure = (role != TOPO_ROLE_EDGES);
     const bool pool = (role != TOPO_ROLE_MEMBERS);
-    if (structure) topo_gather_rows(a, src, g, n0, N);
 
     const bool lean = (a.flags & DRGNN_TOPO_LEAN) != 0 && (a.flags & DRGNN_TOPO_HIER) != 0 && a.cluster0 != nullptr &&
                       a.cluster1 != nullptr && a.c1_ptr != nullptr;
-    const int c1_len = lean ? a.c1_ptr[g + 1] - a.c1_ptr[g] : 0;
+    const int c1_len = lean ? c1e - c1b : 0;
     const int nc1 = imin(N, imax(c1_len, 0));
     const bool run_rows = lean && structure;
     const bool run_clusters = lean && pool;
@@ -1257,7 +1287,12 @@
         if ((int)threadIdx.x < nc1) pre1 = (long long)src.cl1[threadIdx.x];
     }
 #endif
-    topo_stage_edges(tv, src, sidx, N, E, has_w, s);
+    TopoEdgeRegs ereg;
+    topo_edges_load(ereg, src, E, has_w);
+    if (preclear) topo_lean_preclear(N, s, structure, pool);
+    BARRIER();
+    if (structure) topo_gather_rows(a, src, g, n0, N);
+    topo_stage_edges(tv, src, sidx, N, E, has_w, s, ereg);
     topo_tile_store(treg, tile, N);
     topo_touch_done(touch);
     bool rows_done = false, need_c1 = false;
@@ -1298,12 +1333,12 @@
     }
     if (role == TOPO_ROLE_MEMBERS) {
         const int C = topo_clusters0(tv, g, n0, N, src, s, sidx, false);
-        topo_clusters1(tv, a, g, n0, N, C, src, s, sidx);
+        topo_clusters1(tv, a, g, n0, N, C, src, s, sidx, c1e - c1b);
         return;
     }
     const bool members0 = !(lean && role == TOPO_ROLE_EDGES);
     const int C = topo_clusters0(tv, g, n0, N, src, s, sidx, members0, true);
     BARRIER();
     topo_pool(tv, g, n0, e0, E, C, has_w, s);
-    if (role == TOPO_ROLE_ALL || need_c1) topo_clusters1(tv, a, g, n0, N, C, src, s, sidx);
-}
+    if (role == TOPO_ROLE_ALL || need_c1) topo_clusters1(tv, a, g, n0, N, C, src, s, sidx, c1e - c1b);
+}
diff --git a/deeprank-gnn_amd/data.py b/deeprank-gnn_amd/data.py
--- a/deeprank-gnn_amd/data.py
+++ b/deeprank-gnn_amd/data.py
@@ -156,6 +156,7 @@
         if all(torch.is_tensor(c) for c in c1):
             lens = [int(c.numel()) for c in c1]
             d["_c1_ptr"] = ptr(lens)
+            d["_host_c1_ptr"] = d["_c1_ptr"].numpy().copy()
             d["_max_c0"] = max(lens) if lens else 0
 
 
diff --git a/deeprank-gnn_amd/topology.py b/deeprank-gnn_amd/topology.py
--- a/deeprank-gnn_amd/topology.py
+++ b/deeprank-gnn_amd/topology.py
@@ -24,7 +24,7 @@
         self.max_nodes = 0
         self.max_edges = 0
         self.max_c0 = 0
-        self.host_node_ptr = self.host_edge_ptr = None
+        self.host_node_ptr = self.host_edge_ptr = self.host_c1_ptr = None
         self.has_level1 = False
         self.flags = _lib.TOPO_HIER
         self.x = None
@@ -100,7 +100,11 @@
                 node_ptr, edge_ptr = dev_ptr[0], dev_ptr[1]
                 if cluster1 is not None and int(counts[2].sum()) == cluster1.numel():
                     c1_ptr = dev_ptr[2]
+                    topo.host_c1_ptr = ptr[2].numpy()
                 topo.host_node_ptr, topo.host_edge_ptr = ptr[0].numpy(), ptr[1].numpy()
+        elif node_ptr is not None and edge_ptr is not None:
+            topo.host_node_ptr, topo.host_edge_ptr = d.get("_host_node_ptr"), d.get("_host_edge_ptr")
+            topo.host_c1_ptr = d.get("_host_c1_ptr") if c1_ptr is not None else None
         topo.max_nodes, topo.max_edges = max_nodes, max_edges
         topo.max_c0 = max_c0
         scratch = None
@@ -126,7 +130,7 @@
                 topo.check()
         return topo
 
-    def request(self, flags=None):
+    def request(self, flags=None, host_tables=True):
         edge_index, edge_attr, batch, cluster0, cluster1, node_ptr, edge_ptr, c1_ptr, scratch = self._inputs
         r = _lib.TopologyRequest()
         p = _lib._ptr
@@ -148,7 +152,39 @@
             self._tiles_x_version = self.x._version
         self.flags = int(r.flags)
         self._finalized = False
+        tables = self.host_tables() if host_tables else None
+        if tables is not None:
+            r.set_host_tables(*tables)
         return r
+
+    def host_tables(self):
+        memo = self.__dict__.get("_host_tables_memo")
+        if memo is None:
+            memo = self.__dict__["_host_tables_memo"] = (self._host_tables_checked(),)
+        return memo[0]
+
+    def _host_tables_checked(self):
+        cluster1, node_ptr, edge_ptr, c1_ptr = self._inputs[4], self._inputs[5], self._inputs[6], self._inputs[7]
+        hn, he, hc = self.host_node_ptr, self.host_edge_ptr, self.host_c1_ptr
+        B = self.n_graphs
+        if hn is None or he is None or node_ptr is None or edge_ptr is None or not (1 <= B <= _lib.TOPO_TABLES_MAX):
+            return None
+        import numpy as np
+        want_c1 = cluster1 is not None and c1_ptr is not None
+        hn, he = np.ascontiguousarray(hn, dtype=np.int32), np.ascontiguousarray(he, dtype=np.int32)
+        hc = None if hc is None else np.ascontiguousarray(hc, dtype=np.int32)
+        totals = [(hn, self.n_nodes, self.max_nodes), (he, self.n_edges, max(self.max_edges, 1))]
+        if want_c1:
+            if hc is None:
+                return None
+            totals.append((hc, cluster1.numel(), None))
+        for t, total, bound in totals:
+            if len(t) != B + 1 or int(t[0]) != 0 or int(t[-1]) != total:
+                return None
+            lens = t[1:] - t[:-1]
+            if int(lens.min()) < 0 or (bound is not None and self.max_nodes > 0 and int(lens.max()) > bound):
+                return None
+        return hn, he, (hc if want_c1 else None)
 
     def full_flags(self):
         own = self.tiles is not None and not getattr(self, "_tiles_separately", False)
diff --git a/include/drgnn.h b/include/drgnn.h
--- a/include/drgnn.h
+++ b/include/drgnn.h
@@ -187,6 +187,12 @@
 #define DRGNN_TOPO_HIER 1
 #define DRGNN_TOPO_LEAN 2
 #define DRGNN_TOPO_TILES 4
+#define DRGNN_TOPO_HOST_TABLES 8
+#define DRGNN_TOPO_TABLES_MAX 64
+typedef struct drgnn_topology_request_tables {
+    drgnn_topology_request request;
+    const int32_t* host_node_ptr; const int32_t* host_edge_ptr; const int32_t* host_c1_ptr;
+} drgnn_topology_request_tables;
 int64_t drgnn_topology_tiles_elems(int64_t n_nodes, int32_t n_feat);
 int32_t drgnn_topology_tiles_ok(int32_t max_nodes, int32_t max_edges, int32_t n_feat);
 int drgnn_topology_tiles(const int32_t* ws_i32, const float* ws_f32, int64_t n_nodes, int64_t n_edges, int64_t n_graphs,
```

Result: no change. 3.754 million graphs/s (-0.6%).
